# katehai/m-cedm

Measured on AMD Instinct MI355X. Metric: denoised_states_per_sec_18step_edm_heun, higher is better.
Workload: dtype f32; 1 GPU; SWE-periodic 128x128, EDM U-Net ch=128 ch_mult=[1,1,1,1] attn@16^2 (BASELINE config 3); states_per_gpu=32, global_batch=32, H=128, W=128, sampler=EDM Heun, 18 steps, 35 NFE/state, S_churn=0, w=0, fp64 state / fp32 net, parallelism=batch-sharded x1, no data-path collective, launch=one HIP graph per sampler call

## Files before the change

include/mcedm_hip.h:

```cpp
#ifndef MCEDM_HIP_H_
#define MCEDM_HIP_H_

#include <stddef.h>
#include <stdint.h>

#ifdef __cplusplus
extern "C" {
#endif

#define MCEDM_ABI_VERSION 4
#define MCEDM_REDUCE_SCRATCH_BYTES (4096 * 8 + 64)
#define MCEDM_MAX_LEVELS 8

typedef enum {
  MCEDM_OK = 0,
  MCEDM_ERR_INVALID = -1,
  MCEDM_ERR_UNSUPPORTED = -2,
  MCEDM_ERR_WORKSPACE = -3,
  MCEDM_ERR_HIP = -4
} mcedm_status;

#define MCEDM_DX_NONE 0
#define MCEDM_DX_CAT 1
#define MCEDM_DX_ENC 2
typedef struct {
  int32_t in_channels;
  int32_t cond_channels;
  int32_t out_channels;
  int32_t ch;
  int32_t n_levels;
  int32_t ch_mult[MCEDM_MAX_LEVELS];
  int32_t num_res_blocks;
  int32_t resolution;
  int32_t n_attn_resolutions;
  int32_t attn_resolutions[MCEDM_MAX_LEVELS];
  int32_t channels_per_head;
  float eps;
  int32_t dx_channels;
  int32_t dx_mode;
} mcedm_unet_desc;

typedef struct {
  int32_t timesteps;
  double sigma_min, sigma_max, rho;
  double S_churn, S_min, S_max, S_noise;
  double w;
  double sigma_data;
  double net_sigma_min, net_sigma_max;
} mcedm_sampler_desc;

typedef struct mcedm_plan mcedm_plan;

int mcedm_version(void);
const char* mcedm_last_error(void);

int mcedm_unet_plan_create(const mcedm_unet_desc* desc, mcedm_plan** out);
void mcedm_unet_plan_destroy(mcedm_plan* plan);

#define MCEDM_VARIANT_CONV_WINO 0
#define MCEDM_VARIANT_CONV_WINO1 1
#define MCEDM_VARIANT_CONV_RESIDENT 2
#define MCEDM_VARIANT_CONV8 3
#define MCEDM_VARIANT_ATTN_FUSED 4
#define MCEDM_VARIANT_WGRAD_WINO 5
#define MCEDM_VARIANT_CONV1X1_REG 6
#define MCEDM_VARIANT_CONV_WINO_FOLD 7
#define MCEDM_VARIANT_CONV_WINO_UPZ 8
int mcedm_unet_plan_set_variant(mcedm_plan* plan, int which, int value);

int mcedm_unet_param_count(const mcedm_plan* plan);
int mcedm_unet_param_info(const mcedm_plan* plan, int index, const char** name, int64_t* numel,
                          int32_t* ndim, int64_t shape[4]);

int mcedm_unet_packed_bytes(const mcedm_plan* plan, size_t* bytes);
int mcedm_unet_pack_weights(const mcedm_plan* plan, const float* const* params, void* packed, void* stream);

int mcedm_unet_workspace_bytes(const mcedm_plan* plan, int B, int H, int W, int training, size_t* bytes);

int mcedm_unet_forward(const mcedm_plan* plan, const void* packed, const float* x, const float* cond,
                       const float* x_scale, const float* noise_labels, int n_noise, float* out,
                       void* workspace, size_t workspace_bytes, int B, int H, int W, int training,
                       void* stream);

int mcedm_edm_denoise(const mcedm_plan* plan, const void* packed, const float* x, const float* sigma,
                      int n_sigma, const float* cond, float* D_out, float* F_out, void* workspace,
                      size_t workspace_bytes, int B, int H, int W, int training, double sigma_data,
                      void* stream);

int mcedm_sampler_workspace_bytes(const mcedm_plan* plan, int B, int H, int W, size_t* bytes);
int mcedm_heun_sample(const mcedm_plan* plan, const void* packed, const mcedm_sampler_desc* sp,
                      const float* cond, const float* mask, const float* init_noise,
                      const double* step_noise, double* out, int return_last, void* workspace,
                      size_t workspace_bytes, int B, int H, int W, void* stream);

int mcedm_heun_sample_rng(const mcedm_plan* plan, const void* packed, const mcedm_sampler_desc* sp, const float* cond,
                          const float* mask, const float* init_noise, const uint64_t* rng_seed, double* out, int return_last,
                          void* workspace, size_t workspace_bytes, int B, int H, int W, void* stream);
typedef struct {
  int32_t system;
  float half_dt, dx;
  float two_dx;
  float sub_h, div_h, sub_u, div_u;
  double weight;
} mcedm_guidance_desc;
int mcedm_heun_sample_guided(const mcedm_plan* plan, const void* packed, const mcedm_sampler_desc* sp,
                             const mcedm_guidance_desc* gd, const float* cond, const float* mask,
                             const float* init_noise, const double* step_noise, double* out, int return_last,
                             void* workspace, size_t workspace_bytes, int B, int H, int W, void* stream);
int mcedm_heun_sample_guided_rng(const mcedm_plan* plan, const void* packed, const mcedm_sampler_desc* sp,
                                 const mcedm_guidance_desc* gd, const float* cond, const float* mask, const float* init_noise,
                                 const uint64_t* rng_seed, double* out, int return_last, void* workspace, size_t workspace_bytes,
                                 int B, int H, int W, void* stream);
int mcedm_unet_forward_dx(const mcedm_plan* plan, const void* packed, const float* x, const float* dx, const float* cond,
                          const float* x_scale, const float* noise_labels, int n_noise, float* out, void* workspace,
                          size_t workspace_bytes, int B, int H, int W, int training, void* stream);
int mcedm_edm_denoise_dx(const mcedm_plan* plan, const void* packed, const float* x, const float* dx, const float* sigma,
                         int n_sigma, const float* cond, float* D_out, float* F_out, void* workspace,
                         size_t workspace_bytes, int B, int H, int W, int training, double sigma_data, void* stream);
int mcedm_edm_denoise_backward_dx(const mcedm_plan* plan, const void* packed, const float* const* params, const float* x,
                                  const float* dx, const float* sigma, int n_sigma, const float* cond, const float* dD,
// ... 56 lines not shown
                                 void* stream);

typedef struct {
  int32_t timesteps;
  int32_t cond_channels;
  const double* t_steps;
  const double* t_hat;
  const float* c_noise;
  double S_noise;
  double w;
} mcedm_vp_sampler_desc;
int mcedm_vp_sampler_workspace_bytes(const mcedm_plan* plan, int B, int H, int W, size_t* bytes);
int mcedm_vp_heun_sample(const mcedm_plan* plan, const void* packed, const mcedm_vp_sampler_desc* sp, const float* cond,
                         const float* init_noise, const double* step_noise, double* out, int return_last, void* workspace,
                         size_t workspace_bytes, int B, int H, int W, void* stream);
int mcedm_vp_heun_sample_rng(const mcedm_plan* plan, const void* packed, const mcedm_vp_sampler_desc* sp, const float* cond,
                             const float* init_noise, const uint64_t* rng_seed, double* out, int return_last, void* workspace,
                             size_t workspace_bytes, int B, int H, int W, void* stream);

typedef struct mcedm_cond_ddim_desc {
  int32_t timesteps, skip_type;
  double eta, w;
  int32_t cond_channels, self_cond, num_diffusion_timesteps;
  const float* alphas_cumprod_ext;
} mcedm_cond_ddim_desc;
int mcedm_cond_ddim_workspace_bytes(const mcedm_plan* plan, int B, int H, int W, size_t* bytes);
int mcedm_cond_ddim_sample(const mcedm_plan* plan, const void* packed, const mcedm_cond_ddim_desc* sp, const float* cond,
                           const float* init_noise, const float* eta_noise, float* xs_out, float* x0_out, int return_last,
                           void* workspace, size_t workspace_bytes, int B, int H, int W, void* stream);
int mcedm_cond_ddim_sample_rng(const mcedm_plan* plan, const void* packed, const mcedm_cond_ddim_desc* sp, const float* cond,
                               const float* init_noise, const uint64_t* rng_seed, float* xs_out, float* x0_out, int return_last,
                               void* workspace, size_t workspace_bytes, int B, int H, int W, void* stream);


typedef struct { float mean, scale, offset, pad; } mcedm_coef;

size_t mcedm_op_conv_packed_floats(int Cout, int Cin, int k);
int mcedm_op_pack_conv(const float* w, const float* b, int Cout, int Cin, int k, int qkv_heads, int dgrad,
                       float* wpk, float* bias_pk, void* stream);
int mcedm_op_gn_coef(const float* xa, const float* xb, int Ca, int Cb, int B, int HW, const float* gamma,
                     const float* beta, const float* film, int film_batch, int film_stride, float eps,
                     mcedm_coef* coef_out, float* stats_out, void* stream);
int mcedm_op_conv(const float* xa, const float* xb, int Ca, int Cb, const mcedm_coef* coef, int coef_batch, int act,
                  int resample, int Hs, int Ws, int H, int W, const float* wpk, const float* bias_pk,
                  const float* res, int res_mode, float* out, int Cout, int B, int k, void* stream);
size_t mcedm_op_conv_wino_packed_floats(int Cout, int Cin);
int mcedm_op_pack_conv_wino(const float* w, int Cout, int Cin, float* wino, void* stream);
int mcedm_op_conv_wino(const float* xa, const float* xb, int Ca, int Cb, const mcedm_coef* coef, int coef_batch, int act,
                       int resample, int H, int W, const float* wino, const float* bias, const float* res, int res_mode,
                       float* out, int Cout, int B, void* stream);
int mcedm_op_conv_wino_sums(const float* xa, const float* xb, int Ca, int Cb, const mcedm_coef* coef, int coef_batch, int act,
                            int resample, int H, int W, const float* wino, const float* bias, const float* res, int res_mode,
                            float* out, float* gsum, int Cout, int B, void* stream);
int mcedm_op_conv_bias_batch(const float* xa, const float* xb, int Ca, int Cb, const mcedm_coef* coef, int coef_batch, int act,
                             int resample, int Hs, int Ws, int H, int W, const float* wpk, const float* bias_pk, int bias_batch,
                             const float* res, int res_mode, float* out, int Cout, int B, int k, void* stream);
int mcedm_op_conv_wino_sums_bias_batch(const float* xa, const float* xb, int Ca, int Cb, const mcedm_coef* coef, int coef_batch,
                                       int act, int resample, int H, int W, const float* wino, const float* bias, int bias_batch,
                                       const float* res, int res_mode, float* out, float* gsum, int Cout, int B, void* stream);
int mcedm_op_pack_conv_wino_dgrad(const float* w, int Cout, int Cin, float* wino, void* stream);
int mcedm_op_embedding(const float* labels, int n, int ch, const float* w0, const float* b0, const float* w1,
                       const float* b1, const float* waff, const float* baff, int rows, float* freqs_scratch,
                       float* emb_out, float* film_out, void* stream);
int mcedm_op_attention(const float* qkv, float* out, int B, int heads, int T, void* stream);
int mcedm_op_attn_block64(const float* y, const float* gamma, const float* beta, float eps, const float* wq_pk,
                          const float* bq_pk, const float* wp_pk, const float* bp_pk, float* z, float* gsum, int B, void* stream);
size_t mcedm_op_wgrad_scratch_floats(int Cout, int Cin, int k, int B, int H, int W);
int mcedm_op_conv_wgrad(const float* dy, const float* xa, const float* xb, int Ca, int Cb, const mcedm_coef* coef,
                        int coef_batch, int act, int resample, int Hs, int Ws, int H, int W, int Cout, int B, int k,
                        int qkv_heads, float* scratch, float* dw, float* db, void* stream);
int mcedm_op_gn_bwd(const float* dact, int resample, const float* xa, const float* xb, int Ca, int Cb, int Hs, int Ws,
                    int B, const mcedm_coef* coef, const float* stats, const float* gamma, const float* beta,
                    const float* film, int film_batch, int film_stride, int act, float* dxa, float* dxb, int accumulate,
                    const float* add, int add_mode, float* ab, float* dgamma, float* dbeta, float* dfilm,
                    int dfilm_stride, void* stream);
#define MCEDM_GN_SYNC_WORDS 130
int mcedm_op_gn_bwd_sync(const float* dact, int resample, const float* xa, const float* xb, int Ca, int Cb, int Hs, int Ws,
                         int B, const mcedm_coef* coef, const float* stats, const float* gamma, const float* beta,
                         const float* film, int film_batch, int film_stride, int act, float* dxa, float* dxb, int accumulate,
                         const float* add, int add_mode, float* ab, float* dgamma, float* dbeta, float* dfilm,
                         int dfilm_stride, unsigned int* sync, void* stream);
int mcedm_op_attention_bwd(const float* qkv, const float* a, const float* da, float* dqkv, float* lse_scratch, int B,
                           int heads, int T, void* stream);
int mcedm_op_ddim_cond_step(const float* xt, const float* F, const float* Fu, const float* noise, double w, float s0, float s1,
                            float sa_next, float c1, float c2, float* xt_next, float* condp, float* condp_u, int cond_channels,
                            int plan_cond_channels, int B, int C, int H, int W, float* xs, int T_xs, int t_xs, float* x0s,
                            int T_x0, int t_x0, void* stream);
int mcedm_op_ddim_cond_step_rng(const float* xt, const float* F, const float* Fu, const uint64_t* rng_seed, uint64_t draw, double w,
                                float s0, float s1, float sa_next, float c1, float c2, float* xt_next, float* condp, float* condp_u,
                                int cond_channels, int plan_cond_channels, int B, int C, int H, int W, float* xs, int T_xs,
                                int t_xs, float* x0s, int T_x0, int t_x0, void* stream);
int mcedm_op_set_conv_tile(int mt, int ph, int pw);
int mcedm_op_set_conv8(int enable);
int mcedm_op_set_conv_resident(int enable);
int mcedm_op_set_conv_wino(int enable);
int mcedm_op_set_conv_wino1(int enable);
int mcedm_op_set_wgrad_wino(int enable);
int mcedm_op_set_conv1x1_reg(int enable);
int mcedm_op_set_conv_wino_fold(int enable);
int mcedm_op_set_conv_wino_upz(int enable);
int mcedm_op_pack_conv_frag(const float* w, int Cout, int Cin, float* wfrag, void* stream);
int mcedm_op_conv_skip(const float* x, int Cin, const mcedm_coef* coef, int act, int H, int W, const float* wpk, const float* wino,
                       const float* bias, const float* res, const float* sk_xa, const float* sk_xb, int sk_Ca, int sk_Cb,
                       const float* sk_wpk, const float* sk_wfrag, const float* sk_bias, float* out, float* gsum, int Cout, int B,
                       void* stream);
int mcedm_op_conv_sums(const float* xa, const float* xb, int Ca, int Cb, const mcedm_coef* coef, int coef_batch, int act, int resample,
                       int Hs, int Ws, int H, int W, const float* wpk, const float* wino, const float* bias_pk, int bias_batch,
                       const float* res, int res_mode, float* out, int Cout, int B, int k, float* gsum, int gsum_rc, int* tiling_out,
                       void* stream);
int mcedm_op_gn_coef_from_sums(const float* suma, const float* sumb, const int* tiling_a, const int* tiling_b, int Ca, int Cb, int B, int H,
                               int W, int groups, const float* gamma, const float* beta, const float* film, int film_batch,
                               int film_stride, float eps, mcedm_coef* coef_out, float* stats_out, void* stream);
int mcedm_op_conv_gn(const float* xa, const float* xb, int Ca, int Cb, const float* suma, const float* sumb, const int* tiling_a,
                     const int* tiling_b, int groups, const float* gamma, const float* beta, const float* film, int film_batch,
                     int film_stride, float eps, int act, int resample, int Hs, int Ws, int H, int W, const float* wpk, const float* wino,
                     const float* bias_pk, const float* res, int res_mode, float* out, int Cout, int B, int k, void* stream);
int mcedm_op_set_attn_fused(int enable);
int mcedm_op_set_conv_debug(unsigned long long* buf);

typedef struct {
  int32_t in_channels;
  int32_t out_channels;
  int32_t ch;
  int32_t n_levels;
  int32_t ch_mult[MCEDM_MAX_LEVELS];
  int32_t num_res_blocks;
  int32_t resolution;
  int32_t n_attn_resolutions;
  int32_t attn_resolutions[MCEDM_MAX_LEVELS];
  int32_t self_cond;
  float eps;
} mcedm_ddpm_desc;

typedef struct {
  int32_t timesteps;
  double sigma_min, sigma_max, rho;
  double S_churn, S_min, S_max, S_noise;
  double w;
  int32_t n_repeat;
  int32_t n_time_h, n_time_u;
  int32_t h_ch, u_ch;
  int32_t num_diffusion_timesteps;
  const float* edm_steps;
  const float* alphas_cumprod_ext;
} mcedm_repaint_desc;

typedef struct mcedm_ddpm_plan mcedm_ddpm_plan;
int mcedm_ddpm_plan_create(const mcedm_ddpm_desc* desc, mcedm_ddpm_plan** out);
void mcedm_ddpm_plan_destroy(mcedm_ddpm_plan* plan);
int mcedm_ddpm_plan_set_variant(mcedm_ddpm_plan* plan, int which, int value);
int mcedm_ddpm_param_count(const mcedm_ddpm_plan* plan);
int mcedm_ddpm_param_info(const mcedm_ddpm_plan* plan, int index, const char** name, int64_t* numel, int32_t* ndim,
                          int64_t shape[4]);
// ... 100 lines not shown
```

m-cedm_amd/csrc/backward.hip:

```cpp
#include <algorithm>
#include <cmath>
#include <vector>

#include "bwd.hpp"
#include "plan.hpp"

namespace mcedm {

static inline int grid_for(size_t n) {
  size_t b = (n + 255) / 256;
  return (int)(b < 2048 ? (b ? b : 1) : 2048);
}

__global__ void scale_by_cout_kernel(const float* __restrict__ dD, const float* __restrict__ coefs4, int n_sigma,
                                     size_t per_sample, size_t total, float* __restrict__ dF) {
  for (size_t i = blockIdx.x * (size_t)blockDim.x + threadIdx.x; i < total; i += (size_t)gridDim.x * blockDim.x)
    dF[i] = dD[i] * coefs4[4 * (n_sigma == 1 ? 0 : i / per_sample) + 1];
}

__device__ __forceinline__ float silu_b(float v) { return v / (1.0f + expf(-v)); }
__device__ __forceinline__ float dsilu_b(float v) { const float s = 1.0f / (1.0f + expf(-v)); return s * (1.0f + v * (1.0f - s)); }

__global__ __launch_bounds__(256) void emb_save_kernel(const float* __restrict__ labels, const float* __restrict__ freqs,
                                                       const float* __restrict__ w0, const float* __restrict__ b0,
// ... 89 lines not shown
  S.xact = take(max_dact * 4);
  S.ab = take((size_t)B * max_c * 2 * 4);
  S.wg = take(max_wg * 4);
  S.dfilm = take((size_t)B * P.film_rows * 4);
  S.lse = take(max_lse * 4);
  S.gF = take((size_t)B * P.desc.out_channels * H * W * 4);
  S.pe = take((size_t)B * ch * 4); S.u1 = take((size_t)B * ch * 4); S.u2 = take((size_t)B * ch * 4);
  S.t1 = take((size_t)B * ch * 4); S.t2 = take((size_t)B * ch * 4); S.t3 = take((size_t)B * ch * 4);
  S.emb = take((size_t)B * ch * 4);
  S.sync_bytes = gn_bwd_sync_words(B, 32) * sizeof(unsigned);
  S.sync = take(S.sync_bytes);
  S.total = cur;
  return S;
}

size_t backward_scratch_bytes(const mcedm_plan& P, const Layout& L, int B, int H, int W) {
  return make_scratch(P, L, B, H, W).total;
}

struct Ctx;
static GnBwdArgs with_sync(const Ctx& c, GnBwdArgs g);

struct Ctx {
  const AdmNet& net;
  const mcedm_plan& P;
  const Layout& L;
  const BwdScratch& S;
  char* scr;
  const float* pk;
  float* const* grads;
  int B, n_noise;
  hipStream_t s;
  std::vector<char> have;
  const float* emb = nullptr;
  int n_buckets = 0;
  const int32_t* bucket_first = nullptr;
  void* const* bucket_events = nullptr;

  Ctx(const AdmNet& n, const BwdScratch& scratch, float* const* g)
      : net(n), P(*n.plan), L(n.L), S(scratch), scr(n.act + n.L.total_bytes), pk(n.pk), grads(g), B(n.B), n_noise(n.n_noise),
        s(n.s), have(n.L.t.size(), 0) {}
  float* T(int id) const { return net.T(id); }
  Coef* CF(int id) const { return net.CF(id); }
  float* G(int id) const { return id < 0 ? nullptr : reinterpret_cast<float*>(scr + S.g[id]); }
  float* X(size_t off) const { return reinterpret_cast<float*>(scr + off); }
};
static GnBwdArgs with_sync(const Ctx& c, GnBwdArgs g) { g.sync = reinterpret_cast<unsigned*>(c.X(c.S.sync)); return g; }

static int dgrad(const Ctx& c, const ConvP& cv, const float* dy, int H, int W, float* out) {
  ConvArgs a{};
  a.xa = dy; a.Ca = cv.cout;
  a.Hs = H; a.Ws = W; a.H = H; a.W = W;
  a.wpk = c.pk + cv.wpk_dgrad;
  a.wino = cv.wino_dgrad != NONE ? c.pk + cv.wino_dgrad : nullptr;
  a.out = out; a.Cout = cv.cin; a.B = c.B;
  return launch_conv(a, cv.taps, c.s);
}

static int norm_param_grads(const Ctx& c, const NormP& nm, const float* film, int film_stride, float* dfilm) {
  return launch_gn_param_grads(c.X(c.S.ab), c.pk + nm.gamma, c.pk + nm.beta, film, c.net.coef_batch(), film_stride,
                               c.B, nm.C, c.grads[nm.w], c.grads[nm.b], dfilm, c.P.film_rows, c.s);
}

static int block_backward(Ctx& c, const BlockP& b, const BlockLayout& bl) {
  int rc;
  const int B = c.B, H = bl.H, W = bl.W;
  const float* xa = c.T(bl.xa);
  const float* xb = c.T(bl.xb);
  const int Ca = c.L.t[bl.xa].C, Cb = bl.xb >= 0 ? c.L.t[bl.xb].C : 0;
  const int rs = b.up ? RS_UP : (b.down ? RS_DOWN : RS_NONE);
  float* dact = c.X(c.S.dact);
  float* wg = c.X(c.S.wg);
  const float* dy = c.G(bl.out);
  if (b.attn) {
    const float* dz = c.G(bl.z);
    WgradArgs wp{dz, c.T(bl.a), nullptr, b.cout, 0, nullptr, 0, 0, RS_NONE, H, W, H, W, b.cout, B, wg, nullptr};
    if ((rc = launch_wgrad(wp, 1, c.grads[b.proj.w], c.grads[b.proj.b], 0, c.X(c.S.xact), c.s))) return rc;
    if ((rc = dgrad(c, b.proj, dz, H, W, c.G(bl.a)))) return rc;
    if ((rc = launch_attention_bwd(c.T(bl.qkv), c.T(bl.a), c.G(bl.a), c.G(bl.qkv), c.X(c.S.lse), B, b.heads, H * W, c.s))) return rc;
    if ((rc = dgrad(c, b.qkv, c.G(bl.qkv), H, W, dact))) return rc;
    GnBwdArgs g2{dact, RS_NONE, c.T(bl.y), nullptr, b.cout, 0, H, W, B, b.norm2.groups, c.CF(bl.coef2), c.T(bl.stats2),
                 c.pk + b.norm2.gamma, nullptr, 0, 0, 0, c.G(bl.y), nullptr, 0, dz, 1, b.cout, c.X(c.S.ab), c.X(c.S.xact)};
    if ((rc = launch_gn_bwd(with_sync(c, g2), c.s))) return rc;
    if ((rc = norm_param_grads(c, b.norm2, nullptr, 0, nullptr))) return rc;
    WgradArgs wq{c.G(bl.qkv), c.T(bl.y), nullptr, b.cout, 0, c.CF(bl.coef2), 1, 0, RS_NONE, H, W, H, W, 3 * b.cout, B, wg, nullptr};
    if ((rc = launch_wgrad(wq, 1, c.grads[b.qkv.w], c.grads[b.qkv.b], b.heads, c.X(c.S.xact), c.s, true))) return rc;
    dy = c.G(bl.y);
  }
  if ((rc = dgrad(c, b.conv1, dy, H, W, dact))) return rc;
  const float* film = c.net.film() + b.film_row0;
  GnBwdArgs g1{dact, RS_NONE, c.T(bl.h), nullptr, b.cout, 0, H, W, B, b.norm1.groups, c.CF(bl.coef1), c.T(bl.stats1),
               c.pk + b.norm1.gamma, film, c.net.coef_batch(), c.P.film_rows, 1, c.G(bl.h), nullptr, 0, nullptr, 0, 0,
               c.X(c.S.ab), c.X(c.S.xact)};
  if ((rc = launch_gn_bwd(with_sync(c, g1), c.s))) return rc;
  if ((rc = norm_param_grads(c, b.norm1, film, c.P.film_rows, c.X(c.S.dfilm) + b.film_row0))) return rc;
  WgradArgs w1{dy, c.T(bl.h), nullptr, b.cout, 0, c.CF(bl.coef1), 1, 1, RS_NONE, H, W, H, W, b.cout, B, wg, nullptr};
  if ((rc = launch_wgrad(w1, 9, c.grads[b.conv1.w], c.grads[b.conv1.b], 0, c.X(c.S.xact), c.s, true))) return rc;
  const float* add = dy;
  int add_mode = 1;
  if (b.skip_kernel == 1) {
    if (rs != RS_NONE) { set_error("backward: resampling 1x1 skip conv is outside the hot path (%s)", b.key.c_str()); return MCEDM_ERR_UNSUPPORTED; }
    WgradArgs wsk{dy, xa, xb, Ca, Cb, nullptr, 0, 0, RS_NONE, H, W, H, W, b.cout, B, wg, nullptr};
    if ((rc = launch_wgrad(wsk, 1, c.grads[b.skip.w], c.grads[b.skip.b], 0, c.X(c.S.xact), c.s))) return rc;
    if ((rc = dgrad(c, b.skip, dy, H, W, c.X(c.S.dskip)))) return rc;
    add = c.X(c.S.dskip);
  } else if (b.skip_kernel == 0) {
    add_mode = 2;
// ... 248 lines not shown
```

m-cedm_amd/csrc/common.hpp:

```cpp
#pragma once
#include <hip/hip_runtime.h>
#include <cstdarg>
#include <cstddef>
#include <cstdint>
#include <cstdio>

#include "mcedm_hip.h"

namespace mcedm {

void set_error(const char* fmt, ...);

#define MCEDM_HIP_TRY(expr)                                                                   \
  do {                                                                                        \
    hipError_t e__ = (expr);                                                                  \
    if (e__ != hipSuccess) {                                                                  \
      ::mcedm::set_error("%s failed: %s (%s:%d)", #expr, hipGetErrorString(e__), __FILE__, __LINE__); \
      return MCEDM_ERR_HIP;                                                                   \
    }                                                                                         \
  } while (0)

#define MCEDM_LAUNCH_CHECK(what)                                                               \
  do {                                                                                        \
    hipError_t e__ = hipGetLastError();                                                       \
    if (e__ != hipSuccess) {                                                                  \
      ::mcedm::set_error("launch of %s failed: %s", what, hipGetErrorString(e__));            \
      return MCEDM_ERR_HIP;                                                                   \
    }                                                                                         \
  } while (0)

#define MCEDM_REQUIRE(cond, ...)                                                              \
  do {                                                                                        \
    if (!(cond)) {                                                                            \
      ::mcedm::set_error(__VA_ARGS__);                                                        \
      return MCEDM_ERR_INVALID;                                                               \
    }                                                                                         \
  } while (0)

enum KernelVariant { KV_CONV_WINO = 0, KV_CONV_WINO1 = 1, KV_CONV_RESIDENT = 2, KV_CONV8 = 3, KV_ATTN_FUSED = 4, KV_WGRAD_WINO = 5,
                     KV_CONV1X1_REG = 6, KV_CONV_WINO_FOLD = 7, KV_CONV_WINO_UPZ = 8, KV_COUNT = 9 };
struct KernelVariants { int v[KV_COUNT] = {-1, -1, -1, -1, -1, -1, -1, -1, -1}; };
const KernelVariants* current_variants();
struct VariantScope {
  const KernelVariants* prev;
  explicit VariantScope(const KernelVariants* kv);
  ~VariantScope();
};
static inline int variant_choice(int which, int global, int env_default) {
  const KernelVariants* kv = current_variants();
  if (kv && kv->v[which] >= 0) return kv->v[which];
  return global >= 0 ? global : env_default;
}

typedef float f32x16 __attribute__((ext_vector_type(16)));
typedef float f32x4 __attribute__((ext_vector_type(4)));
typedef float f32x2 __attribute__((ext_vector_type(2)));

static inline int ceil_div(int a, int b) { return (a + b - 1) / b; }
#ifdef __HIPCC__
__device__ __forceinline__ void xcd_group_map(int map, int& bx, int& by) {
  const int nx = gridDim.x, ny = gridDim.y;
  bx = blockIdx.x; by = blockIdx.y;
  if (!map || (ny & 7) != 0) return;
  const int lin = bx + by * nx;
  const int c = lin & 7, i = lin >> 3;
  by = (i / nx) * 8 + c;
  bx = i - (i / nx) * nx;
}
#endif

static inline size_t align_up(size_t v, size_t a) { return (v + a - 1) / a * a; }

struct __attribute__((aligned(16))) Coef {
  float mean, scale, offset, pad;
};

enum Resample { RS_NONE = 0, RS_UP = 1, RS_DOWN = 2, RS_S2 = 3 };

struct SumTiles {
  int tiles = 0;
  int tiles_x = 0;
  int ph = 0, pw = 0;
  int rc = 4;
};
__host__ __device__ static inline int sum_tile_count(const SumTiles& g, int t, int H, int W) {
  const int ty = t / g.tiles_x, tx = t - ty * g.tiles_x;
  const int h = H - ty * g.ph < g.ph ? H - ty * g.ph : g.ph;
  const int w = W - tx * g.pw < g.pw ? W - tx * g.pw : g.pw;
  return g.rc * h * w;
}

struct GnArgs {
  const float* xa; const float* xb; int Ca, Cb;
  int HW, B, groups;
// ... 7 lines not shown
  const float* suma; const float* sumb;
  SumTiles ta, tb;
  int W;
};
int launch_gn_coef_from_sums(const GnArgs& a, hipStream_t stream);
int launch_gn_coef(const GnArgs& a, hipStream_t stream);
bool gn_sums_usable(const GnArgs& a);

struct ConvArgs {
  const float* xa;
  const float* xb;
  int Ca, Cb;
  const Coef* coef;
  int coef_batch;
  int act;
  int resample;
  int Hs, Ws;
  int H, W;
  const float* wpk;
  const float* wino;
  const float* bias;
  const float* res;
  int res_mode;
  int bias_batch;
  float* out;
  int Cout;
  int B;
  float* gsum;
  int gsum_rc;
  SumTiles* gsum_tiles;
  const float* sk_xa; const float* sk_xb; int sk_Ca, sk_Cb;
  const float* sk_wpk; const float* sk_bias;
  GnArgs gn; int gn_on;
  int coef_rows;
  unsigned long long* dbg;
  const float* sk_wfrag;
};
static_assert(sizeof(ConvArgs) % 8 == 0 && offsetof(ConvArgs, bias_batch) + sizeof(int) == offsetof(ConvArgs, out),
              "bias_batch fills the padding in front of `out`: no member moves and the struct does not grow");

int launch_conv(const ConvArgs& a, int taps, hipStream_t stream);
size_t conv_wino_packed_floats(int Cout, int Cin);
int launch_pack_conv_wino(const float* w, float* dst, int Cout, int Cin, int transpose_flip, hipStream_t stream);
bool conv_wino_applicable(const ConvArgs& a, int taps);
bool conv_wino_shape_ok(int Cout, int Cin, int H, int W);
bool conv_wino_fold_shape_ok(int Cout, int sk_Ca, int sk_Cb, int H, int W);
void set_conv_wino_fold(int enable);
void set_conv_wino_upz(int enable);
size_t conv_frag_packed_floats(int Cout, int Cin);
int launch_pack_conv_frag(const float* w, float* dst, int Cout, int Cin, hipStream_t stream);
void set_conv_wino(int enable);
bool conv_wino_preferred(const ConvArgs& a);
int launch_conv_wino(const ConvArgs& a, hipStream_t stream);
static inline int cout_padded(int Cout) { return (Cout + 31) / 32 * 32; }
int conv_resolve_identity(ConvArgs& a);
unsigned long long* conv_debug_buffer();
int try_launch_conv_resident(const ConvArgs& a, int taps, hipStream_t stream);
int try_launch_conv1x1_reg(const ConvArgs& a, int taps, hipStream_t stream);
void set_conv1x1_reg(int enable);
void set_conv_resident(int enable);
static inline int conv_max_tiles(int H, int W) { return ((H + 3) / 4) * ((W + 7) / 8); }
void set_conv_tile_override(int mt, int ph, int pw);
void set_conv8(int enable);
void set_conv_debug(unsigned long long* buf);
int conv_mt_for(int Cout);
int conv_kc_for(int taps);
size_t conv_packed_floats(int Cout, int Cin, int taps);
int launch_pack_conv(const float* w, float* dst, int Cout, int Cin, int taps, int qkv_heads, int transpose_flip,
                     hipStream_t stream);
int launch_pack_bias(const float* b, float* dst, int Cout, int qkv_heads, hipStream_t stream);



struct EmbArgs {
  const float* labels; int n;
  int ch;
  const float* freqs;
  const float* w0; const float* b0; const float* w1; const float* b1;
  const float* waff; const float* baff; int rows;
  float* emb;
  float* film;
};
int launch_embedding(const EmbArgs& a, hipStream_t stream);

int launch_attention(const float* qkv, float* out, int B, int heads, int T, hipStream_t stream);
bool attn_block_fused_applicable(int C, int heads, int H, int W, int groups);
int launch_attn_block64(const float* y, float* z, const float* gamma, const float* beta, float eps, int groups, const float* wq,
                        const float* bq, const float* wp, const float* bp, float* gsum, SumTiles* gsum_tiles, int B,
                        hipStream_t stream);
void set_attn_fused(int enable);

}
```

m-cedm_amd/csrc/conv_mfma.hip:

```cpp
#include <atomic>
#include <cstdlib>

#include "common.hpp"
#include "conv_tile.hpp"
#include "pack.hpp"
#include "prof.hpp"

namespace mcedm {

__device__ Coef k_identity_coef = {0.f, 1.f, 0.f, 0.f};


template <class C>
__device__ __forceinline__ void conv_skip_phase(const ConvArgs& p, const TileGeom<C, RS_NONE>& G, float* xl, float* wl,
                                                f32x16 (&acc)[C::TM][C::TN], int n, int m0, int coutp, int aoff,
                                                const int (&boff)[C::TN], int tid, int wave) {
  static_assert(C::TAPS == 9, "the folded projection rides on a 3x3 conv");
  constexpr int SUB = TileGeom<C, RS_NONE>::SUB;
  constexpr int KS = 8;
  constexpr int V4 = C::MT / 4;
  constexpr int NV4 = KS * V4;
  static_assert(NV4 <= C::NT && C::KC == KS, "one float4 of the skip slab per thread");
  const int Cin = p.sk_Ca + p.sk_Cb;
  const int iters = (Cin + KS - 1) / KS;
// ... 734 lines not shown
  const long long want = 512;
  if ((long long)a.H * a.W <= 256 || a.W < 12) {
    if (coutp % 64 == 0) return launch_cfg<ConvCfg<64, 8, 8, 2, 2, TAPS, KC, 256, SMALL_CPI>>(a, stream);
    return launch_cfg<ConvCfg<32, 8, 8, 1, 2, TAPS, KC, 256, SMALL_CPI>>(a, stream);
  }
  if (TAPS == 9 && a.W >= 24 && (long long)a.H * a.W <= 1024) {
    if (coutp % 128 == 0 && blocks_for(128, 8, 16) >= want) return launch_cfg<ConvCfg<128, 8, 16, 1, 4, TAPS, KC>>(a, stream);
    if (coutp % 64 == 0) return launch_cfg<ConvCfg<64, 8, 16, 1, 4, TAPS, KC, 256, MID_CPI>>(a, stream);
    return launch_cfg<ConvCfg<32, 8, 32, 1, 4, TAPS, KC>>(a, stream);
  }
  if (a.W >= 24) {
    static int conv8_env = -1;
    if (conv8_env < 0) { const char* e = getenv("MCEDM_CONV8"); conv8_env = e ? atoi(e) : 0; }
    if (variant_choice(KV_CONV8, g_conv8, conv8_env) && !a.sk_wpk && a.gsum_rc != 2 && TAPS == 9 && a.resample == RS_NONE && coutp % 128 == 0 && a.Ca + a.Cb <= 2048 &&
        blocks_for(128, 16, 32) >= 224)
      return launch_conv8(a, stream);
    if (coutp % 128 == 0 && blocks_for(128, 8, 32) >= want) return launch_cfg<ConvCfg<128, 8, 32, 1, 4, TAPS, KC>>(a, stream);
    if (coutp % 64 == 0 && blocks_for(64, 8, 32) >= want) return launch_cfg<ConvCfg<64, 8, 32, 1, 4, TAPS, KC>>(a, stream);
    return launch_cfg<ConvCfg<32, 8, 32, 1, 4, TAPS, KC>>(a, stream);
  }
  if (coutp % 128 == 0 && blocks_for(128, 16, 16) >= want) return launch_cfg<ConvCfg<128, 16, 16, 1, 4, TAPS, KC>>(a, stream);
  if (coutp % 64 == 0 && blocks_for(64, 16, 16) >= want) return launch_cfg<ConvCfg<64, 16, 16, 1, 4, TAPS, KC>>(a, stream);
  return launch_cfg<ConvCfg<32, 16, 16, 1, 4, TAPS, KC>>(a, stream);
#endif
}

int launch_conv(const ConvArgs& a, int taps, hipStream_t stream) {
  MCEDM_REQUIRE(taps == 9 || taps == 1, "conv: taps must be 9 or 1 (got %d)", taps);
  MCEDM_REQUIRE(a.B > 0 && a.H > 0 && a.W > 0 && a.Cout > 0 && a.Ca + a.Cb > 0, "conv: empty shape");
  MCEDM_REQUIRE(a.out && a.wpk, "conv: null output / weights");
  if (a.resample == RS_UP) MCEDM_REQUIRE(a.Hs * 2 == a.H && a.Ws * 2 == a.W, "conv: up-resample needs H = 2*Hs");
  else if (a.resample == RS_DOWN) MCEDM_REQUIRE(a.Hs == a.H * 2 && a.Ws == a.W * 2, "conv: down-resample needs Hs = 2*H");
  else if (a.resample == RS_S2) MCEDM_REQUIRE(taps == 9 && a.Hs == a.H * 2 && a.Ws == a.W * 2 && !a.res,
                                              "conv: the stride-2 conv is 3x3 on an even-sized source, without residual");
  else MCEDM_REQUIRE(a.Hs == a.H && a.Ws == a.W, "conv: source size mismatch");
  if (a.res && a.res_mode == RS_UP) MCEDM_REQUIRE(a.H % 2 == 0 && a.W % 2 == 0, "conv: up residual needs even size");
  if (a.sk_wpk) MCEDM_REQUIRE(taps == 9 && a.resample == RS_NONE && a.sk_Ca + a.sk_Cb > 0 && (a.sk_xa || a.sk_xb) && a.Cout > 4,
                              "conv: a folded 1x1 projection rides on an un-resampled 3x3 conv with more than 4 output channels");
  MCEDM_REQUIRE(a.bias_batch == 0 || (a.bias && a.bias_batch >= a.Cout && (long long)a.B * a.bias_batch < (1ll << 31) && taps == 9 &&
                                      a.resample == RS_NONE && a.Cout > 4),
                "conv: a bias row per sample (bias_batch=%d) goes with an un-resampled 3x3 conv of more than 4 output channels", a.bias_batch);
  MCEDM_REQUIRE((unsigned long long)a.Hs * a.Ws * 4ull < (1ull << 32) &&
                (unsigned long long)cout_padded(a.Cout) * (a.Ca + a.Cb + 16) * taps * 4ull < (1ull << 32),
                "conv: plane or weight table exceeds the 4 GiB buffer range");
  if (a.res) {
    const unsigned long long rpix = a.res_mode == RS_DOWN ? 4ull * a.H * a.W : a.res_mode == RS_UP ? (a.H / 2ull) * (a.W / 2ull)
                                                                                                    : 1ull * a.H * a.W;
    MCEDM_REQUIRE(rpix * a.Cout * 4ull < (1ull << 32), "conv: one sample of the residual exceeds the 4 GiB buffer range");
  }
  if (taps == 9 && a.Cout <= 4 && a.resample == RS_NONE && !a.res && !a.gsum && !g_force_mt && (long long)a.H * a.W >= 4096)
    return launch_small_cout(a, stream);
  if (a.resample == RS_S2) return dispatch_s2(a, stream);
  if (!g_force_mt && taps == 9 && a.wino && (a.bias_batch == 0 || a.act) && conv_wino_preferred(a) && conv_wino_applicable(a, taps)) return launch_conv_wino(a, stream);
  if (!g_force_mt && taps == 1) {
    const int rc = try_launch_conv1x1_reg(a, taps, stream);
    if (rc != -1) return rc;
  }
  if (!g_force_mt) {
    const int rc = try_launch_conv_resident(a, taps, stream);
    if (rc != -1) return rc;
  }
  return taps == 9 ? dispatch<9, 8>(a, stream) : dispatch<1, 16>(a, stream);
}

}
```

m-cedm_amd/csrc/conv_resident.hip:

```cpp
#include <atomic>
#include <algorithm>
#include <cstdint>
#include <cstdlib>
#include <type_traits>

#include "common.hpp"
#include "conv_tile.hpp"
#include "prof.hpp"

namespace mcedm {

__device__ __forceinline__ int opaque(int v) { asm volatile("" : "+v"(v)); return v; }

static constexpr int SKC = 16;

template <int MT_, int PH_, int PW_, int WM_, int WN_, int TAPS_, int KC_, int KS_ = 1, int DB_ = 0>
struct ResCfg {
  static constexpr int MT = MT_, PH = PH_, PW = PW_, WM = WM_, WN = WN_, TAPS = TAPS_, KC = KC_, KS = KS_;
  static constexpr bool DB = DB_ != 0;
  static constexpr int CPI = 1, KCI = KC_, NT = 256;
  static constexpr int HALO = (TAPS == 9) ? 1 : 0;
  static constexpr int XL0 = HALO ? 3 : 0;
  static constexpr int XM = HALO ? 4 : 0;
  static constexpr int PITCH = HALO ? PW + 8 : PW;
// ... 405 lines not shown
      }
    }
  }

  if (p.dbg && tid == 0) { p.dbg[blockIdx.x * 16 + 2] = __builtin_amdgcn_s_memrealtime(); p.dbg[blockIdx.x * 16 + 6] = __builtin_amdgcn_s_memtime(); }
  float* red = wl;
  if constexpr (C::KS > 1) {
    float* part = xl;
    constexpr int PER_WAVE = C::TM * C::TN * 16 * 64;
    if (ks > 0) {
      float* dst = part + ((ks - 1) * (C::WM * C::WN) + wm * C::WN + wn) * PER_WAVE + lane;
#pragma unroll
      for (int i = 0; i < C::TM; ++i)
#pragma unroll
        for (int j = 0; j < C::TN; ++j)
#pragma unroll
          for (int r = 0; r < 16; ++r) dst[((i * C::TN + j) * 16 + r) * 64] = acc[i][j][r];
    }
    __syncthreads();
    if (ks == 0) {
      for (int g = 1; g < C::KS; ++g) {
        const float* src = part + ((g - 1) * (C::WM * C::WN) + wm * C::WN + wn) * PER_WAVE + lane;
#pragma unroll
        for (int i = 0; i < C::TM; ++i)
#pragma unroll
          for (int j = 0; j < C::TN; ++j)
#pragma unroll
            for (int r = 0; r < 16; ++r) acc[i][j][r] += src[((i * C::TN + j) * 16 + r) * 64];
      }
    }
  }
  if (ks == 0) conv_epilogue_any<C>(p, acc, n, m0, y0, x0, wm, wn, lane, red);
  if (p.dbg && tid == 0) {
    asm volatile("s_waitcnt vmcnt(0)" ::: "memory");
    p.dbg[blockIdx.x * 16 + 3] = __builtin_amdgcn_s_memrealtime();
    unsigned hwid, xcc;
    asm volatile("s_getreg_b32 %0, hwreg(HW_REG_HW_ID)" : "=s"(hwid));
    asm volatile("s_getreg_b32 %0, hwreg(HW_REG_XCC_ID)" : "=s"(xcc));
    p.dbg[blockIdx.x * 16 + 4] = ((unsigned long long)xcc << 32) | hwid;
  }
  if (p.gsum) {
    __syncthreads();
    conv_stats_store<C, C::WN>(p, red, n, m0, ty * tiles_x + tx, tiles_x * tiles_y, tid);
  }
}

static int g_resident = -1;
void set_conv_resident(int enable) { g_resident = enable; }
static int resident_level() {
  static int env = -1;
  if (env < 0) { const char* e = getenv("MCEDM_CONV_RESIDENT"); env = e ? atoi(e) : 1; }
  return variant_choice(KV_CONV_RESIDENT, g_resident, env);
}

static constexpr int LDS_MAX = 160 * 1024;
static int big_level() {
  static int env = -1;
  if (env < 0) { const char* e = getenv("MCEDM_RES_BIG"); env = e ? atoi(e) : 1; }
  return env;
}
static int db_level() {
  static int env = -1;
  if (env < 0) { const char* e = getenv("MCEDM_RES_DB"); env = e ? atoi(e) : 0; }
  return env;
}
static int big128_level() {
  static int env = -1;
  if (env < 0) { const char* e = getenv("MCEDM_RES_BIG128"); env = e ? atoi(e) : 0; }
  return env;
}
static int big_pass() {
  static int env = -1;
  if (env < 0) { const char* e = getenv("MCEDM_RES_BIG_PASS"); env = (e && atoi(e) >= 8) ? atoi(e) / 8 * 8 : 1 << 20; }
  return env;
}

struct ResidentPlan { int pass_c = 0, nslab = 0, wide = 0; size_t lds = 0; };

template <class C, bool SPLIT>
static size_t resident_lds_bytes(const ConvArgs& a, int pass_c, int nslab) {
  return sizeof(float) * ((size_t)nslab * SlabGeom<C, SPLIT>::SL + (size_t)((C::BIG || C::DB) ? 2 : 1) * pass_c * C::PLANE) + sizeof(Coef) * (size_t)(a.Ca + a.Cb);
}

template <class C, bool SPLIT>
static ResidentPlan resident_plan(const ConvArgs& a, size_t budget, int min_pass) {
  constexpr int LPQ = C::PH * (C::PW / 4);
  constexpr int CPS = C::BIG ? 1 : C::NT / C::PLANE, CPD = C::BIG ? 1 : C::NT / C::NPIX, CPQ = LPQ > 64 ? 1 : 64 / LPQ;
  ResidentPlan r;
  const int Cin = a.Ca + a.Cb, Csk = a.sk_wpk ? a.sk_Ca + a.sk_Cb : 0;
  if (!a.xa || a.Ca <= 0 || (a.Cb > 0 && !a.xb)) return r;
  if (Csk && (!a.sk_xa || a.sk_Ca <= 0 || (a.sk_Cb > 0 && !a.sk_xb) || Csk % SKC)) return r;
  auto al16 = [](const void* q) { return (reinterpret_cast<uintptr_t>(q) & 15u) == 0; };
  r.wide = a.resample == RS_NONE && a.Ws % 4 == 0 && a.W % 4 == 0 && al16(a.xa) && al16(a.xb) && a.Ca % C::CPW == 0 && Cin % C::CPW == 0 &&
           (!Csk || (al16(a.sk_xa) && al16(a.sk_xb) && a.sk_Ca % CPQ == 0));
  if (!r.wide && (C::BIG || a.Ca % CPS || Cin % CPS || (Csk && a.sk_Ca % CPD))) { r.wide = 0; return r; }
  const int need = std::max(ceil_div(Cin, C::KC) * C::KC, Csk);
  constexpr int G = C::BIG ? C::KC : (C::KS * C::KC > 16 ? C::KS * C::KC : 16);
  static_assert(!C::BIG || 2 * C::KC * C::PLANE >= SKC * C::NPIX, "projection chunk fits the two pass buffers");
  const int all = ceil_div(need, G) * G;
  for (int nslab = 3; nslab >= 2; --nslab) {
    const size_t fixed = resident_lds_bytes<C, SPLIT>(a, 0, nslab);
    if (fixed >= budget) continue;
    int pc = (int)((budget - fixed) / (sizeof(float) * C::PLANE * ((C::BIG || C::DB) ? 2 : 1))) / G * G;
    if (pc > all) pc = all;
    if (pc >= std::min(min_pass, all)) { r.pass_c = pc; r.nslab = nslab; r.lds = resident_lds_bytes<C, SPLIT>(a, pc, nslab); return r; }
  }
// ... 127 lines not shown
```

m-cedm_amd/csrc/conv_wino.hip:

```cpp
#include <atomic>
#include <cstdlib>

#include "conv_wino.hpp"
#include "pack.hpp"
#include "prof.hpp"

namespace mcedm {

__global__ void wino_pack_kernel(const float* __restrict__ w, float* __restrict__ dst, int Cout, int Cin, int coutp, int nch,
                                 int tflip) {
  const int idx = blockIdx.x * blockDim.x + threadIdx.x;
  if (idx >= coutp * nch * WKC) return;
  wino_pack_elem(w, dst, idx, Cout, Cin, coutp, tflip);
}

__global__ void conv_frag_pack_kernel(const float* __restrict__ w, float* __restrict__ dst, int Cout, int Cin, int coutp, int cinp) {
  const int idx = blockIdx.x * blockDim.x + threadIdx.x;
  if (idx >= coutp * cinp) return;
  dst[idx] = frag_pack_value(w, idx, Cout, Cin, coutp);
}

template <class C, bool = C::SKIP>
struct SkipFold {};
template <class C>
// ... 60 lines not shown
#pragma unroll
    for (int r = 0; r < 16; ++r) v0[r] = keep[0][r] + xch[(pw * 16 + r) * 64 + lane];
    f32x4 bq[4];
#pragma unroll
    for (int jj = 0; jj < 4; ++jj) bq[jj] = *reinterpret_cast<const f32x4*>(rd + 4 * jj);
    for (int s = 0; s < nsk; ++s) {
      f32x4 bqn[4], san[2];
      wreq(s + 1 < nsk ? s + 1 : s, san);
      commit((s + 1) & 1);
      sld = req(s + 2 < nsk ? s + 2 : nsk - 1);
#pragma unroll
      for (int j = 0; j < 4; ++j)
#pragma unroll
        for (int e = 0; e < 2; ++e) rv[e] = __builtin_amdgcn_mfma_f32_32x32x2f32(sa[j >> 2][j & 3], bq[j >> 1][2 * (j & 1) + e], rv[e], 0, 0, 0);
      __syncthreads();
      const float* b = rd + ((s + 1) & 1) * SKBUF;
#pragma unroll
      for (int jj = 0; jj < 4; ++jj) bqn[jj] = *reinterpret_cast<const f32x4*>(b + 4 * jj);
      if (s == 0) {
#pragma unroll
        for (int r = 0; r < 16; ++r) xch[(wave * 16 + r) * 64 + lane] = send[1][r];
      }
      if (s == 1) {
#pragma unroll
        for (int r = 0; r < 16; ++r) v1[r] = keep[1][r] + xch[(pw * 16 + r) * 64 + lane];
      }
#pragma unroll
      for (int j = 4; j < 8; ++j)
#pragma unroll
        for (int e = 0; e < 2; ++e) rv[e] = __builtin_amdgcn_mfma_f32_32x32x2f32(sa[j >> 2][j & 3], bq[j >> 1][2 * (j & 1) + e], rv[e], 0, 0, 0);
#pragma unroll
      for (int jj = 0; jj < 4; ++jj) bq[jj] = bqn[jj];
      sa[0] = san[0];
      sa[1] = san[1];
    }
#pragma unroll
    for (int r = 0; r < 16; ++r) {
      const float bs = skb[(r & 3) + 8 * (r >> 2)];
      v0[r] = v0[r] + (rv[0][r] + bs);
      v1[r] = v1[r] + (rv[1][r] + bs);
    }
  }
};

template <class C, bool UP, bool ACT = true, class... Tag>
__global__ __launch_bounds__(C::NT, C::MB == 4 ? 1 : 2) void conv_wino_kernel(const ConvArgs p, int tiles_x, int tiles_img, int nch, int mblocks,
                                                                          int per, int mode) {
  constexpr int WSC = C::SC, VBUF = C::VBUF, RBUF = C::RBUF, MB = C::MB;
  constexpr bool SKIP = C::SKIP;
  constexpr bool UPZ = WinoUpTraits<Tag...>::UPZ;
  constexpr bool UPS = WinoUpTraits<Tag...>::UPS;
  static_assert(!UPS || UPZ, "source-resolution staging is part of the zero-position variant");
  static_assert(!UPZ || (UP && !SKIP), "the zero positions belong to the up-sampled input");
  extern __shared__ float lds[];
  const int Cin = p.Ca + p.Cb;
  float* const vbuf = lds;
  float* const rbuf = lds + 2 * VBUF;
  Coef* const cfl = reinterpret_cast<Coef*>(lds + C::LDS_ROWS_OFF);
  float* const xch = lds + C::LDS_ROWS_OFF + 4 * Cin;
  float* const red = xch + C::XCH_FLOATS;
  float* const bias_l = red + 2 * (C::MT / 2) * 3;
  float* const skb_l = bias_l + C::MT;
  float* const skbuf = skb_l + C::MT;
  const int tid = threadIdx.x, lane = tid & 63;
  const int wave = __builtin_amdgcn_readfirstlane(tid >> 6);
  const int mb = wave % MB, hf = wave / MB;
  if (p.dbg && tid == 0) { p.dbg[blockIdx.x * 16 + 0] = __builtin_amdgcn_s_memrealtime(); p.dbg[blockIdx.x * 16 + 4] = per; }
  int gt0 = blockIdx.x * per, tstep = 1;
  int n = gt0 / tiles_img, tile0 = gt0 % tiles_img;
  if (mode & 256) {
    const int nwg = gridDim.x, wps = tiles_img / per;
    const int lid = (nwg % 8 == 0) ? (int)(blockIdx.x % 8) * (nwg / 8) + (int)(blockIdx.x / 8) : (int)blockIdx.x;
    n = lid / wps; tile0 = lid % wps; tstep = wps;
  }
  const int m0 = blockIdx.y * C::MT;
  const size_t HW = (size_t)p.H * p.W, HWs = (size_t)p.Hs * p.Ws;
  const int nst = (nch + WSC - 1) / WSC;
  const int G = per * nst;

  constexpr int NR = UPS ? 1 : UP ? RSUB : 4, NG = UPS ? 1 : UP ? RSUB : 1;
  unsigned roff[NG], rkeepL[NG], rkeepC[NG];
  int lofs[4];
  if (!UP) {
    const int r = lane / 6, qd = lane % 6;
#pragma unroll
    for (int e = 0; e < 4; ++e) {
      const int col = 4 * qd + e - 3;
      lofs[e] = (lane < 60 && col >= 0 && col < RPITCH) ? r * RPITCH + col : RROWS * RPITCH + lane % (RPLANE - RROWS * RPITCH);
    }
  }
  auto set_geom = [&](int tile) {
    const int y0 = (tile / tiles_x) * WPH, x0 = (tile % tiles_x) * WPW;
    if (UPS) {
      const int r = lane / UCOLS, c = lane - r * UCOLS;
      const int y = (y0 >> 1) - 1 + r, x = (x0 >> 1) - 1 + c;
      const bool inb = lane < UROWS * UCOLS && (unsigned)y < (unsigned)p.Hs && (unsigned)x < (unsigned)p.Ws;
      rkeepL[0] = inb ? 0xffffffffu : 0u;
      roff[0] = !inb ? 0u : 4u * (unsigned)(y * p.Ws + x);
    } else if (UP) {
#pragma unroll
      for (int i = 0; i < NG; ++i) {
        const int e = lane + 64 * i;
        const int r = e / RPITCH, c = e - r * RPITCH;
        const int y = y0 - 1 + r, x = x0 - 1 + c;
        const bool inb = e < RROWS * RPITCH && (unsigned)y < (unsigned)p.H && (unsigned)x < (unsigned)p.W;
        rkeepL[i] = inb ? 0xffffffffu : 0u;
        roff[i] = !inb ? 0u : 4u * (unsigned)((y >> 1) * p.Ws + (x >> 1));
      }
    } else {
      const int y = y0 - 1 + lane / 6, x = x0 - 4 + 4 * (lane % 6);
      const bool inb = lane < 60 && (unsigned)y < (unsigned)p.H && x >= 0 && x < p.W;
      rkeepL[0] = inb ? 0xffffffffu : 0u;
      roff[0] = inb ? 4u * (unsigned)(y * p.W + x) : 0u;
    }
  };
  float raw[WSC][C::CPW][NR];
  int ld_st = 0, ld_tile = tile0, cm_st = 0;
  set_geom(tile0);
  auto raw_load1 = [&](int sc) {
#pragma unroll
    for (int cw = 0; cw < C::CPW; ++cw) {
      const int ci = (ld_st * WSC + sc) * WKC + wave * C::CPW + cw;
      const bool in_a = ci < p.Ca;
      const float* src = in_a ? p.xa : p.xb;
      const int cc = in_a ? ci : ci - p.Ca, CC = in_a ? p.Ca : p.Cb;
      const bool ok = ci < Cin && src != nullptr;
      const float* plane = ok ? src + ((size_t)n * CC + cc) * HWs : (p.xa ? p.xa : p.xb);
      if (UP) {
// ... 92 lines not shown
      for (int ti = 0; ti < C::TI; ++ti) {
        float t[2][3];
#pragma unroll
        for (int c = 0; c < 3; ++c) {
          t[0][c] = tu[sc][ti][0][c] - tu[sc][ti][2][c];
          t[1][c] = tu[sc][ti][2][c] + tsgn * tu[sc][ti][1][c];
        }
#pragma unroll
        for (int x = 0; x < 2; ++x) {
          if (x == 0 && hf != 0) continue;
          float* o = vb + sc * 16 * VPOS + tr_dst + MB * ti * WTX * 4 + 4 * x * VPOS;
          o[0 * VPOS] = t[x][0] - t[x][1];
          o[1 * VPOS] = t[x][1] + 1.f * t[x][1];
          o[3 * VPOS] = t[x][1] - t[x][2];
        }
      }
      return;
    }
#pragma unroll
    for (int ti = 0; ti < C::TI; ++ti) {
      f32x2 t[2][2];
#pragma unroll
      for (int j = 0; j < 2; ++j) {
        t[0][j] = td[sc][ti][0][j] - td[sc][ti][2][j];
        t[1][j] = td[sc][ti][2][j] + tsgn * td[sc][ti][1][j];
      }
#pragma unroll
      for (int x = 0; x < 2; ++x) {
        const f32x2 o03 = t[x][0] - t[x][1];
        const f32x2 c11 = {t[x][0].y, t[x][0].y}, c22 = {t[x][1].x, t[x][1].x};
        const f32x2 o12 = c11 + tpm * c22;
        float* o = vb + sc * 16 * VPOS + tr_dst + MB * ti * WTX * 4 + 4 * x * VPOS;
        o[0 * VPOS] = o03.x;
        o[1 * VPOS] = o12.x;
        if constexpr (!UPZ) o[2 * VPOS] = o12.y;
        o[3 * VPOS] = o03.y;
      }
    }
  };
  auto transform_read = [&](const float* rb) { for (int sc = 0; sc < WSC; ++sc) transform_read1(sc, rb); };
  auto transform_finish = [&](float* vb) { for (int sc = 0; sc < WSC; ++sc) transform_finish1(sc, vb); };

  stage_coef_rows<C::NT>(p, n, cfl, tid);
  if (tid < C::MT) bias_l[tid] = p.bias ? p.bias[(WinoUpTraits<Tag...>::BROWS ? n * p.bias_batch : 0) + m0 + tid] : 0.f;
  if constexpr (SKIP) { if (tid < C::MT) skb_l[tid] = p.sk_bias ? p.sk_bias[m0 + tid] : 0.f; }
  raw_load();
  __syncthreads();
  for (int sc = 0; sc < WSC; ++sc) raw_commit1(sc, rbuf);
  commit_done();
  if (G > 1) { raw_load(); for (int sc = 0; sc < WSC; ++sc) raw_commit1(sc, rbuf + RBUF); commit_done(); }
  if (G > 2) raw_load();
  const size_t ustride = (size_t)mblocks * 16 * 64;
  constexpr int PHF = UPZ ? 12 : 8;
  const f32x4* up = reinterpret_cast<const f32x4*>(p.wino) + ((size_t)(m0 / 32 + mb) * 16 + PHF * hf) * 64 + lane;
  f32x4 ua[8];
  if constexpr (UPZ) {
    const f32x4 zero4 = {0.f, 0.f, 0.f, 0.f};
    ua[0] = up[0 * 64]; ua[1] = up[1 * 64]; ua[3] = up[3 * 64];
    ua[4] = zero4; ua[5] = zero4; ua[7] = zero4;
    if (hf == 0) { ua[4] = up[4 * 64]; ua[5] = up[5 * 64]; ua[7] = up[7 * 64]; }
  } else {
#pragma unroll
    for (int q = 0; q < 8; ++q) ua[q] = up[q * 64];
  }
  __syncthreads();
  transform_read(rbuf);
  transform_finish(vbuf);
  f32x16 acc[8];
  auto init_acc = [&]() {
    const f32x16 zero16 = {0.f, 0.f, 0.f, 0.f, 0.f, 0.f, 0.f, 0.f, 0.f, 0.f, 0.f, 0.f, 0.f, 0.f, 0.f, 0.f};
    float z = 0.f;
#pragma unroll
    for (int q = 0; q < 8; ++q) {
      asm volatile("" : "+v"(z));
      acc[q] = __builtin_amdgcn_mfma_f32_32x32x2f32(z, z, zero16, 0, 0, 0);
    }
    if (hf == 0) {
#pragma unroll
      for (int r = 0; r < 16; ++r) acc[5][r] = bias_l[32 * mb + 4 * (lane >> 5) + (r & 3) + 8 * (r >> 2)];
    }
  };
  __syncthreads();
  init_acc();

  const int vrd = (PHF * hf) * VPOS + (lane >> 5) * VH1 + (lane & 31) * 4;
  if (p.dbg && tid == 0) { p.dbg[blockIdx.x * 16 + 1] = __builtin_amdgcn_s_memrealtime(); p.dbg[blockIdx.x * 16 + 5] = __builtin_amdgcn_s_memtime(); }
#ifdef MCEDM_WINO_TIMELINE
  unsigned long long ph[5] = {0, 0, 0, 0, 0}, tlast = __builtin_amdgcn_s_memtime();
#define WINO_STAMP(i) { const unsigned long long t_ = __builtin_amdgcn_s_memtime(); ph[i] += t_ - tlast; tlast = t_; }
  unsigned long long sl[8] = {0, 0, 0, 0, 0, 0, 0, 0}, slast = 0;
#define WINO_SLOT(i) { const unsigned long long t_ = __builtin_amdgcn_s_memtime(); sl[(i) & 7] += t_ - slast; slast = t_; }
#define WINO_SLOT0 { slast = __builtin_amdgcn_s_memtime(); }
  unsigned long long ep[6] = {0, 0, 0, 0, 0, 0}, elast = 0;
#define WINO_EP(i) { __builtin_amdgcn_sched_barrier(0); const unsigned long long t_ = __builtin_amdgcn_s_memtime(); if (i) ep[(i) - 1] += t_ - elast; elast = t_; __builtin_amdgcn_sched_barrier(0); }
  const bool no_u = mode & 2;
#else
#define WINO_STAMP(i)
#define WINO_SLOT(i)
#define WINO_SLOT0
#define WINO_EP(i)
  constexpr bool no_u = false;
#endif
  auto side_slice_upz = [&](int slot, int cur) {
    if (WSC == 2) {
      if (slot == 0) transform_read1(0, rbuf + (cur ^ 1) * RBUF);
      if (slot == 1) raw_commit1(0, rbuf + cur * RBUF);
      if (slot == 2) { transform_finish1(0, vbuf + (cur ^ 1) * VBUF); raw_load1(0); }
      if (slot == 3) transform_read1(WSC - 1, rbuf + (cur ^ 1) * RBUF);
      if (slot == 4) { raw_commit1(WSC - 1, rbuf + cur * RBUF); commit_done(); }
      if (slot == 5) { transform_finish1(WSC - 1, vbuf + (cur ^ 1) * VBUF); raw_load1(WSC - 1); raw_load_done(); }
    } else {
      if (slot == 0) transform_read(rbuf + (cur ^ 1) * RBUF);
      if (slot == 1) { raw_commit1(0, rbuf + cur * RBUF); commit_done(); }
      if (slot == 2) { transform_finish1(0, vbuf + (cur ^ 1) * VBUF); raw_load1(0); raw_load_done(); }
    }
  };
  auto side_slice = [&](int slot, int g, int cur) {
    if (WSC == 2) {
      if (slot == 0) transform_read1(0, rbuf + (cur ^ 1) * RBUF);
      if (slot == 1) raw_commit1(0, rbuf + cur * RBUF);
      if (slot == 2) { transform_finish1(0, vbuf + (cur ^ 1) * VBUF); raw_load1(0); }
      if (slot == 3) transform_read1(WSC - 1, rbuf + (cur ^ 1) * RBUF);
      if (slot == 4) { raw_commit1(WSC - 1, rbuf + cur * RBUF); commit_done(); }
      if (slot == 5) { transform_finish1(WSC - 1, vbuf + (cur ^ 1) * VBUF); raw_load1(WSC - 1); raw_load_done(); }
    } else {
      if (slot == 0) transform_read(rbuf + (cur ^ 1) * RBUF);
      if (slot == 1) { raw_commit1(0, rbuf + cur * RBUF); commit_done(); }
      if (slot == 2) { raw_load1(0); raw_load_done(); }
      if (slot == 3) transform_finish1(0, vbuf + (cur ^ 1) * VBUF);
    }
  };
  (void)mode;
  int st = 0, tile = tile0;
  for (int g = 0; g < G; ++g) {
    const int cur = g & 1;
    WINO_STAMP(0)
    WINO_SLOT0
#pragma unroll
    for (int sc = 0; sc < WSC; ++sc) {
      const int c = st * WSC + sc;
      const f32x4* un = up + (size_t)(c + 1 < nch ? c + 1 : 0) * ustride;
      const float* vb = vbuf + cur * VBUF + sc * 16 * VPOS + vrd;
      if constexpr (UPZ) {
        constexpr int CQ[3] = {0, 1, 3};
        f32x4 bq[3];
        bq[0] = *reinterpret_cast<const f32x4*>(vb);
        bq[1] = *reinterpret_cast<const f32x4*>(vb + VPOS);
        __builtin_amdgcn_sched_group_barrier(0x100, 2, 0);
#pragma unroll
        for (int i = 0; i < 3; ++i) {
          if (i == 0) bq[2] = *reinterpret_cast<const f32x4*>(vb + 3 * VPOS);
#pragma unroll
          for (int s = 0; s < 4; ++s) acc[CQ[i]] = __builtin_amdgcn_mfma_f32_32x32x2f32(ua[CQ[i]][s], bq[i][s], acc[CQ[i]], 0, 0, 0);
          if (!no_u) ua[CQ[i]] = un[CQ[i] * 64];
          side_slice_upz(sc * 3 + i, cur);
          if (i == 0) __builtin_amdgcn_sched_group_barrier(0x100, 1, 0);
#pragma unroll
          for (int k = 0; k < 4; ++k) {
            __builtin_amdgcn_sched_group_barrier(0x008, 1, 0);
            __builtin_amdgcn_sched_group_barrier(0x486, 2 * WINO_IL_K, 0);
          }
          __builtin_amdgcn_sched_group_barrier(0x020, 4, 0);
          __builtin_amdgcn_sched_barrier(0);
          if (sc * 3 + i == (WSC == 2 ? 5 : 2)) raw_load_next();
          __builtin_amdgcn_sched_barrier(0);
        }
        if (hf == 0) {
          constexpr int HQ[3] = {4, 5, 7};
          f32x4 bh[3];
#pragma unroll
          for (int i = 0; i < 3; ++i) bh[i] = *reinterpret_cast<const f32x4*>(vb + HQ[i] * VPOS);
#pragma unroll
          for (int i = 0; i < 3; ++i) {
#pragma unroll
            for (int s = 0; s < 4; ++s) acc[HQ[i]] = __builtin_amdgcn_mfma_f32_32x32x2f32(ua[HQ[i]][s], bh[i][s], acc[HQ[i]], 0, 0, 0);
            if (!no_u) ua[HQ[i]] = un[HQ[i] * 64];
          }
        }
        __builtin_amdgcn_sched_barrier(0);
      } else {
      f32x4 b4[2][2];
      b4[0][0] = *reinterpret_cast<const f32x4*>(vb);
      b4[0][1] = *reinterpret_cast<const f32x4*>(vb + VPOS);
      __builtin_amdgcn_sched_group_barrier(0x100, 2, 0);
#pragma unroll
      for (int qp = 0; qp < 4; ++qp) {
        const int cb = qp & 1;
        if (qp < 3) {
          b4[cb ^ 1][0] = *reinterpret_cast<const f32x4*>(vb + (2 * qp + 2) * VPOS);
          b4[cb ^ 1][1] = *reinterpret_cast<const f32x4*>(vb + (2 * qp + 3) * VPOS);
        }
#pragma unroll
        for (int s = 0; s < 4; ++s) {
          acc[2 * qp] = __builtin_amdgcn_mfma_f32_32x32x2f32(ua[2 * qp][s], b4[cb][0][s], acc[2 * qp], 0, 0, 0);
          acc[2 * qp + 1] = __builtin_amdgcn_mfma_f32_32x32x2f32(ua[2 * qp + 1][s], b4[cb][1][s], acc[2 * qp + 1], 0, 0, 0);
        }
        if (!no_u) {
          ua[2 * qp] = un[(2 * qp) * 64];
          ua[2 * qp + 1] = un[(2 * qp + 1) * 64];
        }
        side_slice(sc * 4 + qp, g, cur);
        if (qp < 3) __builtin_amdgcn_sched_group_barrier(0x100, 2, 0);
#pragma unroll
        for (int i = 0; i < 8; ++i) {
          __builtin_amdgcn_sched_group_barrier(0x008, 1, 0);
          __builtin_amdgcn_sched_group_barrier(0x486, WINO_IL_K, 0);
        }
        __builtin_amdgcn_sched_group_barrier(0x020, 4, 0);
        __builtin_amdgcn_sched_barrier(0);
        if (sc * 4 + qp == (WSC == 2 ? 5 : 2)) raw_load_next();
        __builtin_amdgcn_sched_barrier(0);
        WINO_SLOT(sc * 4 + qp + (WSC == 1 ? 0 : 0))
      }
      }
    }
    WINO_STAMP(1)
    __syncthreads();
    WINO_STAMP(2)
    if (++st < nst) continue;
    st = 0;

    WINO_EP(0)
    const int y0 = (tile / tiles_x) * WPH, x0 = (tile % tiles_x) * WPW;
    const int pt = lane & 31;
    const int oy = y0 + 2 * (pt >> 3) + hf, ox = x0 + 2 * (pt & 7);
    const int cbase = m0 + 32 * mb + 4 * (lane >> 5);
    const size_t splane = (size_t)p.Cout * HW;
    const __amdgpu_buffer_rsrc_t rs_out = make_rsrc(p.out + (size_t)n * splane, 4u * (unsigned)splane);
    const size_t rplane = p.res_mode == RS_UP ? splane >> 2 : p.res_mode == RS_DOWN ? splane << 2 : splane;
    const __amdgpu_buffer_rsrc_t rs_res = make_rsrc(p.res ? p.res + (size_t)n * rplane : nullptr, p.res ? 4u * (unsigned)rplane : 0u);
    const unsigned HWu = (unsigned)HW;
    const unsigned voff = 4u * ((unsigned)cbase * HWu + (unsigned)oy * p.W + ox);
    const unsigned rvoff = 4u * ((unsigned)cbase * (HWu >> 2) + (unsigned)(oy >> 1) * (p.W >> 1) + (ox >> 1));
    f32x16 keep[2], send[2];
    float v0[16], v1[16];
    SkipFold<C> sk;
    if constexpr (SKIP) sk.begin(p, skbuf, n, m0 / 32 + mb, mblocks, y0, x0, tid, lane, hf);
#pragma unroll
    for (int j = 0; j < 2; ++j) {
      const f32x16 t0 = j == 0 ? acc[0] + acc[1] + acc[2] : acc[1] - acc[2] - acc[3];
      const f32x16 t1 = j == 0 ? acc[4] + acc[5] + acc[6] : acc[5] - acc[6] - acc[7];
      if (hf == 0)  { keep[j] = t0 + t1; send[j] = t1; }
      else if (UPZ) { keep[j] = -t1 - t0; send[j] = t1; }
      else          { keep[j] = -t0 - t1; send[j] = t0; }
      __builtin_amdgcn_sched_barrier(0);
    }
    __builtin_amdgcn_sched_barrier(0);
    if constexpr (SKIP) {
      WINO_EP(1)
      sk.run(xch, skb_l + 32 * mb + 4 * (lane >> 5), wave, wave ^ MB, lane, keep, send, v0, v1);
      WINO_EP(2)
    } else {
    float2 rv[16];
    if (p.res && p.res_mode == RS_DOWN) {
      const unsigned dvoff = 4u * ((unsigned)cbase * (HWu << 2) + (unsigned)(2 * oy) * (unsigned)(2 * p.W) + (unsigned)(2 * ox));
#pragma unroll
      for (int r0 = 0; r0 < 16; r0 += 4) {
        f32x4 ta[4], tb[4];
#pragma unroll
        for (int k = 0; k < 4; ++k) {
          const unsigned so = 4u * (unsigned)(((r0 + k) & 3) + 8 * ((r0 + k) >> 2)) * (HWu << 2);
          ta[k] = __builtin_bit_cast(f32x4, __builtin_amdgcn_raw_buffer_load_b128(rs_res, dvoff, so, 0));
          tb[k] = __builtin_bit_cast(f32x4, __builtin_amdgcn_raw_buffer_load_b128(rs_res, dvoff + 8u * (unsigned)p.W, so, 0));
        }
#pragma unroll
        for (int k = 0; k < 4; ++k)
          rv[r0 + k] = make_float2(0.25f * ((ta[k][0] + ta[k][1]) + (tb[k][0] + tb[k][1])), 0.25f * ((ta[k][2] + ta[k][3]) + (tb[k][2] + tb[k][3])));
      }
    } else {
#pragma unroll
      for (int r = 0; r < 16; ++r) {
        const int dr = (r & 3) + 8 * (r >> 2);
        if (p.res && p.res_mode == RS_UP) {
          const float q = __builtin_bit_cast(float, __builtin_amdgcn_raw_buffer_load_b32(rs_res, rvoff, 4u * (unsigned)dr * (HWu >> 2), 0));
// ... 52 lines not shown
            for (int e = 0; e < 2; ++e) {
              float* slot = red + (hf * (C::MT / 2) + 2 * quad + e) * 3;
              slot[0] = cnt; slot[1] = a[e]; slot[2] = b[e];
            }
          } else {
            float* slot = red + (hf * (C::MT / 4) + quad) * 3;
            slot[0] = cnt; slot[1] = a[0] + a[1]; slot[2] = b[0] + b[1];
          }
        }
      }
      __syncthreads();
      conv_stats_store<C, 2>(p, red, n, m0, tile, tiles_img, tid);
    }
    WINO_EP(4)
    __builtin_amdgcn_sched_barrier(0);
    init_acc();
    tile += tstep;
    WINO_EP(5)
    WINO_STAMP(3)
  }
  if (p.dbg && tid == 0) {
    asm volatile("s_waitcnt vmcnt(0)" ::: "memory");
    p.dbg[blockIdx.x * 16 + 2] = __builtin_amdgcn_s_memrealtime(); p.dbg[blockIdx.x * 16 + 6] = __builtin_amdgcn_s_memtime();
    p.dbg[blockIdx.x * 16 + 3] = __builtin_amdgcn_s_memrealtime();
  }
#ifdef MCEDM_WINO_TIMELINE
  if (p.dbg && tid == 0) for (int i = 0; i < 5; ++i) p.dbg[blockIdx.x * 16 + 8 + i] = ph[i];
  if (p.dbg && tid == 0 && (mode & 16)) for (int i = 0; i < 8; ++i) p.dbg[blockIdx.x * 16 + 8 + i] = sl[i];
  if (p.dbg && tid == 0 && (mode & 32)) for (int i = 0; i < 6; ++i) p.dbg[blockIdx.x * 16 + 8 + i] = ep[i];
  if (p.dbg && tid == 64 * MB && !(mode & 48)) { p.dbg[blockIdx.x * 16 + 13] = ph[1]; p.dbg[blockIdx.x * 16 + 14] = ph[2]; p.dbg[blockIdx.x * 16 + 15] = ph[3]; p.dbg[blockIdx.x * 16 + 7] = ph[0]; }
#endif
}

static int g_wino = -1;
void set_conv_wino(int enable) { g_wino = enable; }
static int wino_env() {
  static int env = -1;
  if (env < 0) { const char* e = getenv("MCEDM_WINOGRAD"); env = e ? atoi(e) : 1; }
  return variant_choice(KV_CONV_WINO, g_wino, env);
}
static int g_wino_fold = -1;
void set_conv_wino_fold(int enable) { g_wino_fold = enable; }
static int wino_fold_env() {
  static int env = -1;
  if (env < 0) { const char* e = getenv("MCEDM_WINO_FOLD"); env = e ? atoi(e) : 1; }
  return variant_choice(KV_CONV_WINO_FOLD, g_wino_fold, env);
}
static int g_wino_upz = -1;
void set_conv_wino_upz(int enable) { g_wino_upz = enable; }
static int wino_upz_env() {
  static int env = -1;
  if (env < 0) { const char* e = getenv("MCEDM_WINO_UPZ"); env = e ? atoi(e) : 1; }
  return variant_choice(KV_CONV_WINO_UPZ, g_wino_upz, env);
}
static int wino_mode_env() {
  static int env = -1;
  if (env < 0) {
    const char* e = getenv("MCEDM_WINO_MODE");
    const char* m = getenv("MCEDM_WINO_MAP");
    env = ((e ? atoi(e) : 0) & ~256) | ((m ? atoi(m) : 1) ? 256 : 0);
  }
  return env;
}

static int wino_min_hw_env() {
  static int env = -1;
  if (env < 0) { const char* e = getenv("MCEDM_WINO_MIN_HW"); env = e ? atoi(e) : 1024; }
  return env;
}

size_t conv_frag_packed_floats(int Cout, int Cin) { return (size_t)cout_padded(Cout) * (size_t)ceil_div(Cin, 8) * 8; }

int launch_pack_conv_frag(const float* w, float* dst, int Cout, int Cin, hipStream_t stream) {
  MCEDM_REQUIRE(w && dst && Cout > 0 && Cin > 0, "pack_conv_frag: bad arguments");
  const int coutp = cout_padded(Cout), cinp = ceil_div(Cin, 8) * 8;
  hipLaunchKernelGGL(conv_frag_pack_kernel, dim3(ceil_div(coutp * cinp, 256)), dim3(256), 0, stream, w, dst, Cout, Cin, coutp, cinp);
  MCEDM_LAUNCH_CHECK("conv_frag_pack_kernel");
  return MCEDM_OK;
}

size_t conv_wino_packed_floats(int Cout, int Cin) { return (size_t)16 * cout_padded(Cout) * (size_t)ceil_div(Cin, WKC) * WKC; }

int launch_pack_conv_wino(const float* w, float* dst, int Cout, int Cin, int transpose_flip, hipStream_t stream) {
  MCEDM_REQUIRE(w && dst && Cout > 0 && Cin > 0, "pack_conv_wino: bad arguments");
  const int coutp = cout_padded(Cout), nch = ceil_div(Cin, WKC);
  hipLaunchKernelGGL(wino_pack_kernel, dim3(ceil_div(coutp * nch * WKC, 256)), dim3(256), 0, stream, w, dst, Cout, Cin, coutp, nch,
                     transpose_flip);
  MCEDM_LAUNCH_CHECK("wino_pack_kernel");
  return MCEDM_OK;
}

static bool conv_wino_fold_ok(const ConvArgs& a) {
  const int Csk = a.sk_Ca + a.sk_Cb;
  const unsigned long long HW = (unsigned long long)a.H * a.W;
  return wino_fold_env() != 0 && a.sk_wfrag && a.resample == RS_NONE && !a.res && a.act && a.Cout % 128 == 0 && a.sk_xa && a.sk_Ca > 0 &&
         a.sk_Cb >= 0 && (a.sk_Cb > 0) == (a.sk_xb != nullptr) && a.sk_Ca % 16 == 0 && a.sk_Cb % 16 == 0 && Csk >= 32 && Csk <= 256 &&
         (((size_t)a.sk_xa | (size_t)a.sk_xb | (size_t)a.sk_wfrag) & 15) == 0 && HW * 4ull * (unsigned long long)a.sk_Ca < (1ull << 32) &&
         HW * 4ull * (unsigned long long)a.sk_Cb < (1ull << 32);
}
bool conv_wino_fold_shape_ok(int Cout, int sk_Ca, int sk_Cb, int H, int W) {
  const int Csk = sk_Ca + sk_Cb;
  return wino_fold_env() != 0 && conv_wino_shape_ok(Cout, Cout, H, W) && Cout % 128 == 0 && sk_Ca > 0 && sk_Ca % 16 == 0 && sk_Cb % 16 == 0 &&
         Csk >= 32 && Csk <= 256 && (unsigned long long)H * W * 4ull * (unsigned long long)(sk_Ca > sk_Cb ? sk_Ca : sk_Cb) < (1ull << 32);
}

bool conv_wino_applicable(const ConvArgs& a, int taps) {
// ... 57 lines not shown
                               noact ? "false" : "true", a.bias_batch ? ", WinoBiasRows" : upz == 2 ? ", WinoUp<false>" : upz ? ", WinoUp<true>" : "");
  const double px = (double)a.B * a.H * a.W;
  const double skc = C::SKIP ? (double)(a.sk_Ca + a.sk_Cb) : 0.0;
  ProfScope ps(name, 2.0 * px * a.Cout * ((double)Cin * 9 + skc),
               4.0 * ((double)a.B * Cin * a.Hs * a.Ws + px * (a.Cout * (a.res ? 2 : 1) + skc) + (double)a.Cout * (Cin * 9 + skc)), stream);
  if constexpr (C::SKIP)
    hipLaunchKernelGGL((conv_wino_kernel<C, false>), dim3((unsigned)(total / per), a.Cout / C::MT), dim3(C::NT), lds_bytes, stream, a, tiles_x,
                       tiles_img, nch, cout_padded(a.Cout) / 32, per, wino_mode_env());
  else if (a.bias_batch)
    hipLaunchKernelGGL((conv_wino_kernel<C, false, true, WinoBiasRows>), dim3((unsigned)(total / per), a.Cout / C::MT), dim3(C::NT), lds_bytes, stream, a, tiles_x,
                       tiles_img, nch, cout_padded(a.Cout) / 32, per, wino_mode_env());
  else if (upz == 2)
    hipLaunchKernelGGL((conv_wino_kernel<C, true, true, WinoUp<false>>), dim3((unsigned)(total / per), a.Cout / C::MT), dim3(C::NT), lds_bytes, stream, a, tiles_x,
                       tiles_img, nch, cout_padded(a.Cout) / 32, per, wino_mode_env());
  else if (upz)
    hipLaunchKernelGGL((conv_wino_kernel<C, true, true, WinoUp<true>>), dim3((unsigned)(total / per), a.Cout / C::MT), dim3(C::NT), lds_bytes, stream, a, tiles_x,
                       tiles_img, nch, cout_padded(a.Cout) / 32, per, wino_mode_env());
  else if (a.resample == RS_UP)
    hipLaunchKernelGGL((conv_wino_kernel<C, true>), dim3((unsigned)(total / per), a.Cout / C::MT), dim3(C::NT), lds_bytes, stream, a, tiles_x,
                       tiles_img, nch, cout_padded(a.Cout) / 32, per, wino_mode_env());
  else if (noact)
    hipLaunchKernelGGL((conv_wino_kernel<C, false, false>), dim3((unsigned)(total / per), a.Cout / C::MT), dim3(C::NT), lds_bytes, stream, a, tiles_x,
                       tiles_img, nch, cout_padded(a.Cout) / 32, per, wino_mode_env());
  else
    hipLaunchKernelGGL((conv_wino_kernel<C, false>), dim3((unsigned)(total / per), a.Cout / C::MT), dim3(C::NT), lds_bytes, stream, a, tiles_x,
                       tiles_img, nch, cout_padded(a.Cout) / 32, per, wino_mode_env());
  MCEDM_LAUNCH_CHECK("conv_wino_kernel");
  if (a.gsum_tiles) *a.gsum_tiles = SumTiles{tiles_img, tiles_x, WPH, WPW, a.gsum_rc == 2 ? 2 : 4};
  return MCEDM_OK;
}

int launch_conv_wino(const ConvArgs& a_in, hipStream_t stream) {
  ConvArgs a = a_in;
  a.dbg = conv_debug_buffer();
  MCEDM_REQUIRE(conv_wino_applicable(a, 9), "conv_wino: shape not served by the Winograd kernel");
  MCEDM_REQUIRE(a.out && a.B > 0 && (a.resample == RS_UP ? (a.Hs * 2 == a.H && a.Ws * 2 == a.W) : (a.Hs == a.H && a.Ws == a.W)),
                "conv_wino: bad arguments");
  MCEDM_REQUIRE((unsigned long long)a.H * a.W * 4ull * a.Cout * (a.res && a.res_mode == RS_DOWN ? 4 : 1) < (1ull << 32),
                "conv_wino: one sample of the output / residual exceeds the 4 GiB buffer range");
  { const int rc = conv_resolve_identity(a); if (rc != MCEDM_OK) return rc; }
  if (a.sk_wpk) return launch_wino_cfg<WinoSkipCfg<4>>(a, stream);
  if (a.Cout % 128 == 0 && !a.bias_batch) {
    const int rc = try_launch_conv_wino1(a, stream);
    if (rc != -1) return rc;
  }
  return a.Cout % 128 == 0 ? launch_wino_cfg<WinoCfg<4>>(a, stream) : launch_wino_cfg<WinoCfg<2>>(a, stream);
}

bool conv_wino_shape_ok(int Cout, int Cin, int H, int W) {
  return wino_env() != 0 && Cout % 64 == 0 && Cin % WKC == 0 && H % WPH == 0 && W % WPW == 0 && (long long)H * W >= wino_min_hw_env();
}
bool conv_wino_preferred(const ConvArgs& a) { return wino_env() != 0 && (long long)a.H * a.W >= wino_min_hw_env(); }

}
```

m-cedm_amd/csrc/conv_wino.hpp:

```cpp
#pragma once
#include "conv_tile.hpp"

namespace mcedm {

constexpr int WPH = 8, WPW = 16;
constexpr int WTX = WPW / 2, WTY = WPH / 2;
constexpr int WKC = 8;
static_assert(WTX * WTY == 32, "one MFMA N block of patches per workgroup");
template <int MB_>
struct WinoCfg {
  static constexpr int MB = MB_, NT = 128 * MB_, NW = 2 * MB_, MT = 32 * MB_;
  static constexpr int SC = MB_ == 4 ? 2 : 1;
  static constexpr int CPW = WKC / NW;
  static constexpr int TI = 4 / MB_;
  static constexpr int VBUF = SC * 16 * 288, RBUF = SC * WKC * 196;
  static constexpr int LDS_ROWS_OFF = 2 * VBUF + 2 * RBUF;
  static constexpr int XCH_FLOATS = NW * 16 * 64;
  static constexpr int RED_FLOATS = 2 * (MT / 2) * 3 + MT;
  static constexpr bool SKIP = false;
  static_assert(MB_ == 4 || MB_ == 2, "128 or 64 output channels per workgroup");
  static_assert(LDS_ROWS_OFF % 4 == 0, "LDS layout");
};
template <int MB_>
struct WinoSkipCfg : WinoCfg<MB_> {
  static constexpr bool SKIP = true;
  static constexpr int SKS = 16, SKPITCH = 36, SKBUF = 64 * SKPITCH;
  static constexpr int SK_FLOATS = WinoCfg<MB_>::MT + 2 * SKBUF;
  static_assert(MB_ == 4, "the fold is built for the 128-channel workgroup (512 threads = 16 channels x 32 quads per stage)");
};
template <bool SRC>
struct WinoUp {};
template <class... Tag>
struct WinoUpTraits { static constexpr bool UPZ = false, UPS = false, BROWS = false; static_assert(sizeof...(Tag) == 0, "one tag at most: WinoUp<SRC> or WinoBiasRows"); };
template <bool SRC>
struct WinoUpTraits<WinoUp<SRC>> { static constexpr bool UPZ = true, UPS = SRC, BROWS = false; };
struct WinoBiasRows {};
template <>
struct WinoUpTraits<WinoBiasRows> { static constexpr bool UPZ = false, UPS = false, BROWS = true; };
constexpr int UROWS = WPH / 2 + 2, UCOLS = WPW / 2 + 2;
constexpr int UPLANE = 68;
static_assert(UPLANE >= 64 && UPLANE % 32 == 4 && UPLANE <= 196, "LDS layout");
constexpr int RROWS = WPH + 2, RPITCH = WPW + 2;
constexpr int RPLANE = 196;
constexpr int RSUB = (RROWS * RPITCH + 63) / 64;
constexpr int WINO_IL_K = 5;
constexpr int VH1 = 144, VPOS = 288;
static_assert(RPLANE % 32 == 4 && VH1 % 32 == 16 && VH1 >= 128 && VPOS >= VH1 + 128 && RPLANE >= RROWS * RPITCH && RPLANE % 2 == 0 && VPOS % 4 == 0 && VH1 % 4 == 0, "LDS layout");



int try_launch_conv_wino1(const ConvArgs& a, hipStream_t stream);
void set_conv_wino1(int enable);
int wino_tiles_per_wg(long long total, int tiles_img, int slots);

}
```

m-cedm_amd/csrc/ddpm.hip:

```cpp
#include <cmath>
#include <cstring>
#include <string>
#include <vector>

#include "heun.hpp"
#include "prof.hpp"

namespace mcedm {

struct DConv { int w = -1, b = -1; int cin = 0, cout = 0, taps = 0; size_t wpk = NONE, bias = NONE, wino = NONE; };
struct DNorm { int w = -1, b = -1; int C = 0; size_t gamma = NONE, beta = NONE; };
struct DRes {
  std::string key;
  int cin = 0, cout = 0;
  DNorm n1, n2;
  DConv c1, c2, sc;
  bool has_sc = false;
  int tw = -1, tb = -1;
  int brow = 0;
};
struct DAttn {
  std::string key;
  int C = 0;
  DNorm n;
// ... 505 lines not shown
  Pool pool;
  std::vector<DT> t;
  int bias_batch = 0;

  int act(int C, int H, int W, bool with_sums) {
    DT d; d.C = C; d.H = H; d.W = W;
    d.bytes = (size_t)B * C * H * W * sizeof(float);
    d.off = pool.alloc(d.bytes);
    d.rc = with_sums ? record_width(C) : 0;
    if (d.rc) {
      d.sums_bytes = (size_t)B * conv_max_tiles(H, W) * ceil_div(C, d.rc) * 2 * sizeof(float);
      d.sums = pool.alloc(d.sums_bytes);
    }
    t.push_back(d);
    return (int)t.size() - 1;
  }
  int raw(size_t bytes) { DT d; d.bytes = bytes; d.off = pool.alloc(bytes); t.push_back(d); return (int)t.size() - 1; }
  void release(int id) {
    if (id < 0) return;
    pool.release(t[id].off, t[id].bytes);
    if (t[id].sums != NONE) pool.release(t[id].sums, t[id].sums_bytes);
  }
  float* ptr(int id) const { return id < 0 ? nullptr : reinterpret_cast<float*>(base + t[id].off); }
  float* sums(int id) const { return (id < 0 || t[id].sums == NONE) ? nullptr : reinterpret_cast<float*>(base + t[id].sums); }
};

static int gn_into(DExec& E, const DNorm& n, int xa, int xb, ConvArgs& c, int* table_id) {
  const DT& A = E.t[xa];
  const int Ca = A.C, Cb = xb >= 0 ? E.t[xb].C : 0;
  GnArgs g{E.ptr(xa), E.ptr(xb), Ca, Cb, A.H * A.W, E.B, 32, E.pk + n.gamma, E.pk + n.beta, nullptr, 0, 0, E.P.desc.eps,
           nullptr, nullptr, E.sums(xa), E.sums(xb), A.st, xb >= 0 ? E.t[xb].st : SumTiles{}, A.W};
  *table_id = -1;
  c.act = 1; c.coef_batch = 1;
  const int cpg = (Ca + Cb) / 32, ra = A.rc, rb = xb >= 0 ? E.t[xb].rc : A.rc;
  const bool usable = (Ca + Cb) % 32 == 0 && ra > 0 && rb > 0 && cpg % ra == 0 && cpg % rb == 0 && Ca % ra == 0 && Ca % rb == 0;
  if (usable) {
    if (!E.dry && !gn_sums_usable(g)) { set_error("ddpm forward: statistics table of a %d-channel input is unusable", Ca + Cb); return MCEDM_ERR_INVALID; }
    c.gn = g; c.gn_on = 1; c.coef = nullptr;
    return MCEDM_OK;
  }
  *table_id = E.raw((size_t)E.B * (Ca + Cb) * sizeof(Coef));
  g.coef = reinterpret_cast<Coef*>(E.ptr(*table_id));
  c.coef = g.coef;
  return E.dry ? MCEDM_OK : launch_gn_coef(g, E.s);
}

static void src_of(const DExec& E, ConvArgs& c, int xa, int xb) {
  c.xa = E.ptr(xa); c.Ca = E.t[xa].C;
  c.xb = E.ptr(xb); c.Cb = xb >= 0 ? E.t[xb].C : 0;
  c.Hs = E.t[xa].H; c.Ws = E.t[xa].W; c.H = c.Hs; c.W = c.Ws;
}
static void dst_of(DExec& E, ConvArgs& c, int out, const DConv& cv, const float* bias, bool stats) {
  c.wpk = E.pk + cv.wpk; c.bias = bias ? bias : E.pk + cv.bias;
  c.wino = cv.wino != NONE ? E.pk + cv.wino : nullptr;
  c.out = E.ptr(out); c.Cout = cv.cout; c.B = E.B;
  if (stats && E.t[out].rc) { c.gsum = E.sums(out); c.gsum_rc = E.t[out].rc; c.gsum_tiles = &E.t[out].st; }
}
static int run_conv(DExec& E, ConvArgs& c, int taps, int out) {
  if (E.dry) { if (c.gsum_tiles) *c.gsum_tiles = SumTiles{1, 1, 8, 8, c.gsum_rc == 2 ? 2 : 4}; (void)out; return MCEDM_OK; }
  return launch_conv(c, taps, E.s);
}

static int res_block(DExec& E, const DRes& r, int xa, int xb, const float* bias_table, int* out_id) {
  const int bias_batch = E.bias_batch;
  int rc, tab;
  const int H = E.t[xa].H, W = E.t[xa].W;
  const int h = E.act(r.cout, H, W, true);
  ConvArgs c1{};
  src_of(E, c1, xa, xb);
  if ((rc = gn_into(E, r.n1, xa, xb, c1, &tab))) return rc;
  dst_of(E, c1, h, r.c1, bias_table + r.brow, true);
  c1.bias_batch = bias_batch;
  if ((rc = run_conv(E, c1, 9, h))) return rc;
  E.release(tab);
  const int y = E.act(r.cout, H, W, true);
  ConvArgs c2{};
  src_of(E, c2, h, -1);
  if ((rc = gn_into(E, r.n2, h, -1, c2, &tab))) return rc;
  dst_of(E, c2, y, r.c2, nullptr, true);
  int scid = -1;
  if (r.has_sc && r.c2.wino != NONE && conv_wino_shape_ok(r.cout, r.cout, H, W)) {
    scid = E.act(r.cout, H, W, false);
    ConvArgs cs{};
    src_of(E, cs, xa, xb);
    dst_of(E, cs, scid, r.sc, nullptr, false);
    if ((rc = run_conv(E, cs, 1, scid))) return rc;
    c2.res = E.ptr(scid); c2.res_mode = RS_NONE;
  } else if (r.has_sc) {
    c2.sk_xa = E.ptr(xa); c2.sk_Ca = E.t[xa].C;
    c2.sk_xb = E.ptr(xb); c2.sk_Cb = xb >= 0 ? E.t[xb].C : 0;
    c2.sk_wpk = E.pk + r.sc.wpk; c2.sk_bias = E.pk + r.sc.bias;
  } else {
    c2.res = E.ptr(xa); c2.res_mode = RS_NONE;
  }
  if ((rc = run_conv(E, c2, 9, y))) return rc;
  E.release(tab);
  E.release(h);
  if (scid >= 0) E.release(scid);
  *out_id = y;
  return MCEDM_OK;
}

static int attn_block(DExec& E, const DAttn& a, int x, int* out_id) {
  int rc, tab;
  const int H = E.t[x].H, W = E.t[x].W;
  const int qkv = E.act(3 * a.C, H, W, false);
  ConvArgs cq{};
// ... 851 lines not shown
```

m-cedm_amd/csrc/ops_api.hip:

```cpp
#include "common.hpp"
#include "conv_wino.hpp"
#include "bwd.hpp"
#include "edm.hpp"

using namespace mcedm;

static_assert(sizeof(mcedm_coef) == sizeof(Coef), "mcedm_coef must mirror Coef");

extern "C" size_t mcedm_op_conv_packed_floats(int Cout, int Cin, int k) {
  if (Cout <= 0 || Cin <= 0 || (k != 1 && k != 3)) return 0;
  return conv_packed_floats(Cout, Cin, k * k);
}

extern "C" int mcedm_op_pack_conv(const float* w, const float* b, int Cout, int Cin, int k, int qkv_heads, int dgrad,
                                  float* wpk, float* bias_pk, void* stream) {
  MCEDM_REQUIRE(w && wpk, "op_pack_conv: null pointer");
  MCEDM_REQUIRE(Cout > 0 && Cin > 0 && (k == 1 || k == 3), "op_pack_conv: bad shape");
  MCEDM_REQUIRE(qkv_heads == 0 || (Cout % (3 * qkv_heads) == 0 && !dgrad), "op_pack_conv: bad qkv_heads");
  int rc = dgrad ? launch_pack_conv(w, wpk, Cin, Cout, k * k, 0, 1, (hipStream_t)stream)
                 : launch_pack_conv(w, wpk, Cout, Cin, k * k, qkv_heads, 0, (hipStream_t)stream);
  if (rc) return rc;
  if (b && bias_pk) rc = launch_pack_bias(b, bias_pk, Cout, qkv_heads, (hipStream_t)stream);
  return rc;
}
// ... 44 lines not shown
  return launch_pack_conv_wino(w, wino, Cout, Cin, 0, (hipStream_t)stream);
}

extern "C" int mcedm_op_pack_conv_wino_dgrad(const float* w, int Cout, int Cin, float* wino, void* stream) {
  return launch_pack_conv_wino(w, wino, Cin, Cout, 1, (hipStream_t)stream);
}

extern "C" int mcedm_op_conv_wino(const float* xa, const float* xb, int Ca, int Cb, const mcedm_coef* coef, int coef_batch,
                                  int act, int resample, int H, int W, const float* wino, const float* bias, const float* res,
                                  int res_mode, float* out, int Cout, int B, void* stream) {
  MCEDM_REQUIRE((resample == RS_NONE || resample == RS_UP) && (res_mode == RS_NONE || res_mode == RS_UP || res_mode == RS_DOWN),
                "op_conv_wino: resample must be 0 (none) or 1 (nearest-2x up), res_mode 0, 1 or 2 (2x2-mean down)");
  ConvArgs a{};
  a.xa = xa; a.xb = xb; a.Ca = Ca; a.Cb = Cb;
  a.coef = reinterpret_cast<const Coef*>(coef); a.coef_batch = coef_batch; a.act = act;
  a.resample = resample; a.H = H; a.W = W;
  a.Hs = resample == RS_UP ? H / 2 : H; a.Ws = resample == RS_UP ? W / 2 : W;
  a.wino = wino; a.bias = bias; a.res = res; a.res_mode = res_mode;
  a.out = out; a.Cout = Cout; a.B = B;
  MCEDM_REQUIRE(conv_wino_applicable(a, 9), "op_conv_wino: needs Cout %% 64 == 0, H %% 8 == 0, W %% 16 == 0, Cin %% 8 == 0 and 16-byte aligned inputs / weight table");
  return launch_conv_wino(a, (hipStream_t)stream);
}

static int op_conv_wino_sums(const float* xa, const float* xb, int Ca, int Cb, const mcedm_coef* coef, int coef_batch, int act,
                             int resample, int H, int W, const float* wino, const float* bias, int bias_batch, const float* res,
                             int res_mode, float* out, float* gsum, int Cout, int B, void* stream) {
  MCEDM_REQUIRE((resample == RS_NONE || resample == RS_UP) && (res_mode == RS_NONE || res_mode == RS_UP || res_mode == RS_DOWN),
                "op_conv_wino_sums: resample must be 0 (none) or 1 (nearest-2x up), res_mode 0, 1 or 2 (2x2-mean down)");
  MCEDM_REQUIRE(gsum, "op_conv_wino_sums: gsum is null");
  ConvArgs a{};
  a.xa = xa; a.xb = xb; a.Ca = Ca; a.Cb = Cb;
  a.coef = reinterpret_cast<const Coef*>(coef); a.coef_batch = coef_batch; a.act = act;
  a.resample = resample; a.H = H; a.W = W;
  a.Hs = resample == RS_UP ? H / 2 : H; a.Ws = resample == RS_UP ? W / 2 : W;
  a.wino = wino; a.bias = bias; a.res = res; a.res_mode = res_mode;
  SumTiles st;
  a.out = out; a.Cout = Cout; a.B = B; a.gsum = gsum; a.gsum_tiles = &st;
  MCEDM_REQUIRE(bias_batch == 0 || (bias && bias_batch >= Cout), "op_conv_wino_sums: bias_batch %d needs a bias of B rows of at least Cout floats", bias_batch);
  a.bias_batch = bias_batch;
  MCEDM_REQUIRE(conv_wino_applicable(a, 9), "op_conv_wino_sums: needs Cout %% 64 == 0, H %% 8 == 0, W %% 16 == 0, Cin %% 8 == 0 and 16-byte aligned inputs / weight table");
  return launch_conv_wino(a, (hipStream_t)stream);
}
extern "C" int mcedm_op_conv_wino_sums(const float* xa, const float* xb, int Ca, int Cb, const mcedm_coef* coef, int coef_batch,
                                       int act, int resample, int H, int W, const float* wino, const float* bias, const float* res,
                                       int res_mode, float* out, float* gsum, int Cout, int B, void* stream) {
  return op_conv_wino_sums(xa, xb, Ca, Cb, coef, coef_batch, act, resample, H, W, wino, bias, 0, res, res_mode, out, gsum, Cout, B, stream);
}
extern "C" int mcedm_op_conv_wino_sums_bias_batch(const float* xa, const float* xb, int Ca, int Cb, const mcedm_coef* coef,
                                                  int coef_batch, int act, int resample, int H, int W, const float* wino,
                                                  const float* bias, int bias_batch, const float* res, int res_mode, float* out,
                                                  float* gsum, int Cout, int B, void* stream) {
  return op_conv_wino_sums(xa, xb, Ca, Cb, coef, coef_batch, act, resample, H, W, wino, bias, bias_batch, res, res_mode, out, gsum, Cout, B,
                           stream);
}

extern "C" int mcedm_op_pack_conv_frag(const float* w, int Cout, int Cin, float* wfrag, void* stream) {
  return launch_pack_conv_frag(w, wfrag, Cout, Cin, (hipStream_t)stream);
}

extern "C" int mcedm_op_conv_skip(const float* x, int Cin, const mcedm_coef* coef, int act, int H, int W, const float* wpk, const float* wino,
                                  const float* bias, const float* res, const float* sk_xa, const float* sk_xb, int sk_Ca, int sk_Cb,
                                  const float* sk_wpk, const float* sk_wfrag, const float* sk_bias, float* out, float* gsum, int Cout,
                                  int B, void* stream) {
  MCEDM_REQUIRE(x && out && wpk && Cin > 0 && Cout > 0 && B > 0 && H > 0 && W > 0, "op_conv_skip: bad arguments");
  MCEDM_REQUIRE(!(res && sk_wpk), "op_conv_skip: a residual or a folded projection, not both");
  ConvArgs a{};
  a.xa = x; a.Ca = Cin;
  a.coef = reinterpret_cast<const Coef*>(coef); a.coef_batch = 1; a.act = act;
  a.resample = RS_NONE; a.Hs = H; a.Ws = W; a.H = H; a.W = W;
  a.wpk = wpk; a.wino = wino; a.bias = bias; a.res = res; a.res_mode = RS_NONE;
  a.sk_xa = sk_xa; a.sk_xb = sk_xb; a.sk_Ca = sk_Ca; a.sk_Cb = sk_Cb; a.sk_wpk = sk_wpk; a.sk_wfrag = sk_wfrag; a.sk_bias = sk_bias;
  SumTiles st;
  a.out = out; a.Cout = Cout; a.B = B; a.gsum = gsum; a.gsum_tiles = gsum ? &st : nullptr;
  return launch_conv(a, 9, (hipStream_t)stream);
}

static void tiling_to_ints(const SumTiles& t, int* o) { o[0] = t.tiles; o[1] = t.tiles_x; o[2] = t.ph; o[3] = t.pw; o[4] = t.rc; }
static SumTiles tiling_from_ints(const int* t) { return t ? SumTiles{t[0], t[1], t[2], t[3], t[4]} : SumTiles{}; }

static int op_conv_chain(const char* who, const float* xa, const float* xb, int Ca, int Cb, const mcedm_coef* coef, int coef_batch,
                         const GnArgs* gn, int act, int resample, int Hs, int Ws, int H, int W, const float* wpk, const float* wino,
                         const float* bias_pk, int bias_batch, const float* res, int res_mode, float* out, int Cout, int B, int k,
                         float* gsum, int gsum_rc, int* tiling_out, void* stream) {
  MCEDM_REQUIRE(k == 1 || k == 3, "%s: k must be 1 or 3", who);
  MCEDM_REQUIRE(resample >= 0 && resample <= 3 && res_mode >= 0 && res_mode <= 2, "%s: bad resample mode", who);
  MCEDM_REQUIRE(bias_batch >= 0, "%s: bias_batch %d < 0", who, bias_batch);
  ConvArgs a{};
  a.xa = xa; a.xb = xb; a.Ca = Ca; a.Cb = Cb;
  a.coef = reinterpret_cast<const Coef*>(coef); a.coef_batch = coef_batch; a.act = act;
  a.resample = resample; a.Hs = Hs; a.Ws = Ws; a.H = H; a.W = W;
  a.wpk = wpk; a.wino = wino; a.bias = bias_pk; a.res = res; a.res_mode = res_mode;
  a.out = out; a.Cout = Cout; a.B = B; a.bias_batch = bias_batch;
  SumTiles st;
  if (gsum) { a.gsum = gsum; a.gsum_rc = gsum_rc; a.gsum_tiles = &st; }
  if (gn) { a.gn = *gn; a.gn_on = 1; a.coef = nullptr; a.coef_batch = 1; }
  const int rc = launch_conv(a, k * k, (hipStream_t)stream);
  if (rc) return rc;
  if (gsum) {
    MCEDM_REQUIRE(st.tiles > 0 && st.rc == (gsum_rc == 2 ? 2 : 4), "%s: the launcher wrote no tiling, or records of %d channels where %d were asked for",
                  who, st.rc, gsum_rc == 2 ? 2 : 4);
    tiling_to_ints(st, tiling_out);
  }
  return MCEDM_OK;
}

extern "C" int mcedm_op_conv_sums(const float* xa, const float* xb, int Ca, int Cb, const mcedm_coef* coef, int coef_batch, int act,
// ... 117 lines not shown
              stats, gamma, film, film_batch, film_stride, act, dxa, dxb, accumulate, add, add_mode, C, ab};
  a.sync = sync;
  int rc = launch_gn_bwd(a, (hipStream_t)stream);
  if (rc) return rc;
  return launch_gn_param_grads(ab, gamma, beta, film, film_batch, film_stride, B, C, dgamma, dbeta, dfilm, dfilm_stride,
                               (hipStream_t)stream);
}

extern "C" int mcedm_op_gn_bwd(const float* dact, int resample, const float* xa, const float* xb, int Ca, int Cb, int Hs,
                               int Ws, int B, const mcedm_coef* coef, const float* stats, const float* gamma,
                               const float* beta, const float* film, int film_batch, int film_stride, int act,
                               float* dxa, float* dxb, int accumulate, const float* add, int add_mode, float* ab,
                               float* dgamma, float* dbeta, float* dfilm, int dfilm_stride, void* stream) {
  return op_gn_bwd_impl(dact, resample, xa, xb, Ca, Cb, Hs, Ws, B, coef, stats, gamma, beta, film, film_batch, film_stride, act, dxa, dxb,
                        accumulate, add, add_mode, ab, dgamma, dbeta, dfilm, dfilm_stride, nullptr, stream);
}

extern "C" int mcedm_op_gn_bwd_sync(const float* dact, int resample, const float* xa, const float* xb, int Ca, int Cb, int Hs,
                                    int Ws, int B, const mcedm_coef* coef, const float* stats, const float* gamma,
                                    const float* beta, const float* film, int film_batch, int film_stride, int act,
                                    float* dxa, float* dxb, int accumulate, const float* add, int add_mode, float* ab,
                                    float* dgamma, float* dbeta, float* dfilm, int dfilm_stride, unsigned int* sync, void* stream) {
  return op_gn_bwd_impl(dact, resample, xa, xb, Ca, Cb, Hs, Ws, B, coef, stats, gamma, beta, film, film_batch, film_stride, act, dxa, dxb,
                        accumulate, add, add_mode, ab, dgamma, dbeta, dfilm, dfilm_stride, sync, stream);
}

extern "C" int mcedm_op_attention_bwd(const float* qkv, const float* a, const float* da, float* dqkv, float* lse_scratch,
                                      int B, int heads, int T, void* stream) {
  return launch_attention_bwd(qkv, a, da, dqkv, lse_scratch, B, heads, T, (hipStream_t)stream);
}

extern "C" int mcedm_op_set_conv8(int enable) {
  set_conv8(enable);
  return MCEDM_OK;
}

extern "C" int mcedm_op_set_conv_wino(int enable) {
  set_conv_wino(enable);
  return MCEDM_OK;
}

extern "C" int mcedm_op_set_conv_wino1(int enable) {
  set_conv_wino1(enable);
  return MCEDM_OK;
}

extern "C" int mcedm_op_set_conv_wino_fold(int enable) {
  set_conv_wino_fold(enable);
  return MCEDM_OK;
}

extern "C" int mcedm_op_set_conv_wino_upz(int enable) {
  set_conv_wino_upz(enable);
  return MCEDM_OK;
}

extern "C" int mcedm_op_set_conv1x1_reg(int enable) {
  set_conv1x1_reg(enable);
  return MCEDM_OK;
}

extern "C" int mcedm_op_set_wgrad_wino(int enable) {
  set_wgrad_wino(enable);
  return MCEDM_OK;
}

extern "C" int mcedm_op_set_conv_resident(int enable) {
  set_conv_resident(enable);
  return MCEDM_OK;
}

extern "C" int mcedm_op_set_attn_fused(int enable) {
  set_attn_fused(enable);
  return MCEDM_OK;
}

extern "C" int mcedm_op_set_conv_debug(unsigned long long* buf) {
  set_conv_debug(buf);
  return MCEDM_OK;
}

static int op_ddim_cond_step(const float* xt, const float* F, const float* Fu, const float* noise, const uint64_t* rng_seed,
                             uint64_t draw, double w, float s0, float s1, float sa_next, float c1, float c2, float* xt_next,
                             float* condp, float* condp_u, int cond_channels, int plan_cond_channels, int B, int C, int H, int W,
                             float* xs, int T_xs, int t_xs, float* x0s, int T_x0, int t_x0, void* stream) {
  MCEDM_REQUIRE(xt && F && xt_next, "op_ddim_cond_step: null pointer");
  MCEDM_REQUIRE(B > 0 && C > 0 && H > 0 && W > 0, "op_ddim_cond_step: empty shape");
  MCEDM_REQUIRE(!condp_u || condp, "op_ddim_cond_step: the twin goes with cond'");
  MCEDM_REQUIRE(!condp || (cond_channels >= 0 && cond_channels + C <= plan_cond_channels),
                "op_ddim_cond_step: channels [%d, %d) outside cond' (%d channels)", cond_channels, cond_channels + C, plan_cond_channels);
  MCEDM_REQUIRE((!xs || (t_xs >= 0 && t_xs < T_xs)) && (!x0s || (t_x0 >= 0 && t_x0 < T_x0)), "op_ddim_cond_step: slot outside the trajectory");
  DdimCondStep k{};
  k.xt = xt; k.F = F; k.Fu = Fu; k.noise = noise;
  k.seed = reinterpret_cast<const unsigned long long*>(rng_seed); k.draw = draw;
  k.w1 = (float)(w + 1.0); k.w = (float)w; k.s0 = s0; k.s1 = s1; k.sa = sa_next; k.c1 = c1; k.c2 = c2;
  k.xt_next = xt_next; k.sc = condp; k.sc_u = condp_u;
  k.C = C; k.Cp = plan_cond_channels; k.sc_off = cond_channels; k.hw = (size_t)H * W; k.n = (size_t)B * C * k.hw;
  k.xs = xs; k.x0s = x0s; k.T_xs = T_xs; k.t_xs = t_xs; k.T_x0 = T_x0; k.t_x0 = t_x0;
  return launch_ddim_cond_step(k, (hipStream_t)stream);
}
extern "C" int mcedm_op_ddim_cond_step(const float* xt, const float* F, const float* Fu, const float* noise, double w, float s0,
                                       float s1, float sa_next, float c1, float c2, float* xt_next, float* condp, float* condp_u,
                                       int cond_channels, int plan_cond_channels, int B, int C, int H, int W, float* xs,
                                       int T_xs, int t_xs, float* x0s, int T_x0, int t_x0, void* stream) {
  return op_ddim_cond_step(xt, F, Fu, noise, nullptr, 0, w, s0, s1, sa_next, c1, c2, xt_next, condp, condp_u, cond_channels,
                           plan_cond_channels, B, C, H, W, xs, T_xs, t_xs, x0s, T_x0, t_x0, stream);
// ... 11 lines not shown
```

m-cedm_amd/csrc/plan.hip:

```cpp
#include <algorithm>
#include <cmath>
#include <cstring>

#include "edm.hpp"
#include "pack.hpp"
#include "plan.hpp"
#include "prof.hpp"
#include "bwd.hpp"

namespace mcedm {

static thread_local char g_err[1024] = "";

void set_error(const char* fmt, ...) {
  va_list ap;
  va_start(ap, fmt);
  vsnprintf(g_err, sizeof(g_err), fmt, ap);
  va_end(ap);
}

static NormP make_norm(mcedm_plan& P, const std::string& key, int C) {
  NormP n;
  n.C = C;
  n.groups = std::min(32, C / 4);
  n.w = add_param(P.params, key + ".weight", {C});
  n.b = add_param(P.params, key + ".bias", {C});
  return n;
}

static ConvP make_conv(mcedm_plan& P, const std::string& key, int cin, int cout, int k, int qkv_heads = 0) {
  ConvP c;
  c.cin = cin; c.cout = cout; c.taps = k * k; c.qkv_heads = qkv_heads;
  c.w = add_param(P.params, key + ".weight", {cout, cin, k, k});
  c.b = add_param(P.params, key + ".bias", {cout});
  return c;
}

static BlockP make_block(mcedm_plan& P, const std::string& key, int cin, int cout, bool up, bool down, bool attn) {
  const int emb = P.desc.ch;
  BlockP b;
  b.key = key; b.cin = cin; b.cout = cout; b.up = up; b.down = down;
  b.heads = attn ? cout / P.desc.channels_per_head : 0;
  b.attn = b.heads > 0;
  b.norm0 = make_norm(P, key + ".norm0", cin);
  b.conv0 = make_conv(P, key + ".conv0", cin, cout, 3);
  b.aff_w = add_param(P.params, key + ".affine.weight", {2 * cout, emb});
  b.aff_b = add_param(P.params, key + ".affine.bias", {2 * cout});
  b.norm1 = make_norm(P, key + ".norm1", cout);
  b.conv1 = make_conv(P, key + ".conv1", cout, cout, 3);
  b.skip_kernel = -1;
  if (cout != cin || up || down) {
    b.skip_kernel = (cout != cin) ? 1 : 0;
    if (b.skip_kernel == 1) b.skip = make_conv(P, key + ".skip", cin, cout, 1);
  }
  if (b.attn) {
    b.norm2 = make_norm(P, key + ".norm2", cout);
    b.qkv = make_conv(P, key + ".qkv", cout, 3 * cout, 1, b.heads);
    b.proj = make_conv(P, key + ".proj", cout, cout, 1);
  }
  return b;
}

static void place_conv(Taker& t, ConvP& c, bool dgrad) {
  c.wpk = t.take(conv_packed_floats(c.cout, c.cin, c.taps));
  c.bias = t.take((size_t)(c.cout + 31) / 32 * 32);
  if (dgrad) c.wpk_dgrad = t.take(conv_packed_floats(c.cin, c.cout, c.taps));
  if (c.taps == 9 && c.qkv_heads == 0) {
    if (c.cout % 64 == 0 && c.cin % 8 == 0) c.wino = t.take(conv_wino_packed_floats(c.cout, c.cin));
    if (dgrad && c.cin % 64 == 0 && c.cout % 8 == 0) c.wino_dgrad = t.take(conv_wino_packed_floats(c.cin, c.cout));
  }
}
static void place_skip_frag(Taker& t, ConvP& c) {
  if (c.taps == 1 && c.cout % 128 == 0 && c.cin % 16 == 0 && c.cin >= 32 && c.cin <= 256) c.wfrag = t.take(conv_frag_packed_floats(c.cout, c.cin));
}
static void place_norm(Taker& t, NormP& n) { n.gamma = t.take(n.C); n.beta = t.take(n.C); }

}

using namespace mcedm;

extern "C" int mcedm_version(void) { return MCEDM_ABI_VERSION; }

extern "C" int mcedm_unet_plan_set_variant(mcedm_plan* plan, int which, int value) {
  return plan_set_variant(plan, "plan_set_variant", which, value);
}
extern "C" const char* mcedm_last_error(void) { return g_err; }

extern "C" int mcedm_unet_plan_create(const mcedm_unet_desc* d, mcedm_plan** out) {
  MCEDM_REQUIRE(d && out, "plan_create: null argument");
  MCEDM_REQUIRE(d->n_levels >= 1 && d->n_levels <= MCEDM_MAX_LEVELS, "plan_create: n_levels=%d out of range", d->n_levels);
  MCEDM_REQUIRE(d->n_attn_resolutions >= 0 && d->n_attn_resolutions <= MCEDM_MAX_LEVELS, "plan_create: bad n_attn_resolutions");
  MCEDM_REQUIRE(d->in_channels > 0 && d->out_channels > 0 && d->cond_channels >= 0, "plan_create: bad channel counts");
  MCEDM_REQUIRE(d->ch > 0 && d->ch % 8 == 0, "plan_create: ch=%d must be a positive multiple of 8", d->ch);
  MCEDM_REQUIRE(d->num_res_blocks >= 1, "plan_create: num_res_blocks must be >= 1");
  if (d->channels_per_head != 64) {
    set_error("plan_create: channels_per_head=%d unsupported (the hot path uses 64, adm_blocks.py:223)", d->channels_per_head);
    return MCEDM_ERR_UNSUPPORTED;
  }
  for (int l = 0; l < d->n_levels; ++l) {
    const int c = d->ch * d->ch_mult[l];
    MCEDM_REQUIRE(d->ch_mult[l] >= 1 && c % 8 == 0, "plan_create: level %d width %d must be a multiple of 8", l, c);
  }
  MCEDM_REQUIRE(d->dx_mode == MCEDM_DX_NONE || d->dx_mode == MCEDM_DX_CAT || d->dx_mode == MCEDM_DX_ENC, "plan_create: dx_mode=%d", d->dx_mode);
  MCEDM_REQUIRE((d->dx_mode == MCEDM_DX_NONE) == (d->dx_channels == 0) && d->dx_channels >= 0,
                "plan_create: dx_channels=%d does not go with dx_mode=%d", d->dx_channels, d->dx_mode);
  mcedm_plan* Pp = new mcedm_plan();
  mcedm_plan& P = *Pp;
  P.desc = *d;
  P.levels_div = 1 << (d->n_levels - 1);
  const int ch = d->ch;
  auto key = [&](const char* side, int res, const std::string& tail) {
    return std::string(side) + "." + std::to_string(res) + "x" + std::to_string(res) + "_" + tail;
  };
  P.map0_w = add_param(P.params, "map_layer0.weight", {ch, ch});
  P.map0_b = add_param(P.params, "map_layer0.bias", {ch});
  P.map1_w = add_param(P.params, "map_layer1.weight", {ch, ch});
  P.map1_b = add_param(P.params, "map_layer1.bias", {ch});
  if (d->dx_mode == MCEDM_DX_ENC) {
    const int c0 = ch * d->ch_mult[0];
    P.dx_enc0 = make_conv(P, "dx_enc.0", d->dx_channels, c0, 3);
    P.dx_enc2 = make_conv(P, "dx_enc.2", c0, c0, 3);
// ... 224 lines not shown
  for (auto* v : {&P.enc, &P.dec})
    for (const BlockP& b : *v) {
      cp.add(params[b.aff_w], pk + P.waff + (size_t)b.film_row0 * ch, (size_t)2 * b.cout * ch);
      cp.add(params[b.aff_b], pk + P.baff + b.film_row0, (size_t)2 * b.cout);
      pack_norm(b.norm0, params, pk, cp);
      pack_norm(b.norm1, params, pk, cp);
      if ((rc = pack_conv(b.conv0, params, pk, cp, pp, s))) return rc;
      if ((rc = pack_conv(b.conv1, params, pk, cp, pp, s))) return rc;
      if (b.skip_kernel == 1 && (rc = pack_conv(b.skip, params, pk, cp, pp, s))) return rc;
      if (b.attn) {
        pack_norm(b.norm2, params, pk, cp);
        if ((rc = pack_conv(b.qkv, params, pk, cp, pp, s))) return rc;
        if ((rc = pack_conv(b.proj, params, pk, cp, pp, s))) return rc;
      }
    }
  pack_norm(P.out_norm, params, pk, cp);
  if ((rc = pack_conv(P.conv_out, params, pk, cp, pp, s))) return rc;
  cp.flush();
  pp.flush();
  return cp.status != MCEDM_OK ? cp.status : pp.status;
}

namespace mcedm {

struct LayoutBuilder {
  Layout& L;
  Pool pool;
  int B;
  int make(int C, int H, int W, size_t bytes) {
    TRef t;
    t.C = C; t.H = H; t.W = W; t.bytes = bytes;
    t.off = pool.alloc(bytes);
    L.t.push_back(t);
    return (int)L.t.size() - 1;
  }
  int act(int C, int H, int W) { return make(C, H, W, (size_t)B * C * H * W * sizeof(float)); }
  int coef(int C) { return make(C, 1, 1, (size_t)B * C * sizeof(Coef)); }
  int stats(int groups) { return make(groups, 1, 1, (size_t)B * groups * 2 * sizeof(float)); }
  void retain(int id) { if (id >= 0) L.t[id].ref++; }
  void release(int id) {
    if (id < 0) return;
    if (--L.t[id].ref == 0) pool.release(L.t[id].off, L.t[id].bytes);
  }
  void drop(int id) { if (id >= 0) pool.release(L.t[id].off, L.t[id].bytes); }
};

int build_layout(const mcedm_plan& P, int B, int H, int W, int training, int n_noise, Layout* out) {
  MCEDM_REQUIRE(B > 0 && H > 0 && W > 0, "layout: empty shape B=%d H=%d W=%d", B, H, W);
  MCEDM_REQUIRE(H % P.levels_div == 0 && W % P.levels_div == 0,
                "layout: H=%d W=%d must be multiples of %d (2^(levels-1))", H, W, P.levels_div);
  MCEDM_REQUIRE(n_noise == 1 || n_noise == B, "layout: n_noise=%d must be 1 or B=%d", n_noise, B);
  Layout& L = *out;
  L = Layout();
  LayoutBuilder lb{L, Pool(), B};
  lb.pool.keep_all = training != 0;
  L.film = lb.make(P.film_rows, 1, 1, (size_t)n_noise * P.film_rows * sizeof(float));
  auto sums_sz = [&](int C, int h, int w) { return align_up((size_t)B * conv_max_tiles(h, w) * ceil_div(C, 4) * 2 * sizeof(float), 256); };
  {
    size_t need = sums_sz(P.conv_in.cout, H, W);
    int h = H, w = W;
    for (auto* v : {&P.enc, &P.dec})
      for (const BlockP& b : *v) {
        if (b.up) { h *= 2; w *= 2; } else if (b.down) { h /= 2; w /= 2; }
        need += (size_t)(b.attn ? 3 : 2) * sums_sz(b.cout, h, w);
      }
    L.sums_bytes = need;
    const int id = lb.make(1, 1, 1, need);
    L.sums_base = L.t[id].off;
  }
  size_t sums_cur = L.sums_base;
  auto give_sums = [&](int id) {
    L.t[id].sums = sums_cur;
    sums_cur += sums_sz(L.t[id].C, L.t[id].H, L.t[id].W);
  };
  if (P.desc.dx_mode == MCEDM_DX_CAT) L.xdx = lb.act(P.desc.in_channels + P.desc.dx_channels, H, W);
  if (P.desc.dx_mode == MCEDM_DX_ENC) {
    L.xf = lb.act(P.conv_in.cout, H, W);
    L.d1 = lb.act(P.conv_in.cout, H, W);
    L.g1 = lb.act(P.conv_in.cout, H, W);
    L.d2 = lb.act(P.conv_in.cout, H, W);
  }
  L.t0 = lb.act(P.conv_in.cout, H, W);
  give_sums(L.t0);
  lb.drop(L.xdx); lb.drop(L.xf); lb.drop(L.d1); lb.drop(L.g1); lb.drop(L.d2);
  std::vector<int> skips;
  int cur = L.t0;
  lb.retain(cur);
  lb.retain(cur); skips.push_back(cur);

  auto do_block = [&](const BlockP& b, int xa, int xb) {
    BlockLayout bl;
    bl.xa = xa; bl.xb = xb;
    bl.Hin = L.t[xa].H; bl.Win = L.t[xa].W;
    bl.H = b.up ? bl.Hin * 2 : (b.down ? bl.Hin / 2 : bl.Hin);
    bl.W = b.up ? bl.Win * 2 : (b.down ? bl.Win / 2 : bl.Win);
    bl.coef0 = lb.coef(b.cin);
    if (training) bl.stats0 = lb.stats(b.norm0.groups);
    if (b.down) bl.xd = lb.act(b.cin, bl.H, bl.W);
    bl.h = lb.act(b.cout, bl.H, bl.W);
    give_sums(bl.h);
    lb.drop(bl.coef0); lb.drop(bl.xd);
    bl.coef1 = lb.coef(b.cout);
    if (training) bl.stats1 = lb.stats(b.norm1.groups);
    const bool wino1 = b.conv1.wino != NONE && conv_wino_shape_ok(b.cout, b.cout, bl.H, bl.W);
    const bool wfold = wino1 && !training && !b.up && !b.down && b.skip_kernel == 1 && b.skip.wfrag != NONE &&
                       conv_wino_fold_shape_ok(b.cout, L.t[xa].C, xb >= 0 ? L.t[xb].C : 0, bl.H, bl.W);
// ... 44 lines not shown
  L.coef_out = lb.coef(P.out_norm.C);
  if (training) L.stats_out = lb.stats(P.out_norm.groups);
  L.total_bytes = lb.pool.peak;
  return MCEDM_OK;
}

Header header_for(const mcedm_plan& P, int B, int H, int W) {
  Header h;
  size_t cur = 0;
  auto take = [&](size_t bytes) { size_t o = cur; cur += align_up(bytes, 256); return o; };
  const int Ct = P.desc.in_channels + P.desc.cond_channels + P.desc.dx_channels;
  h.coefs4 = take((size_t)B * 4 * sizeof(float));
  h.c_noise = take((size_t)B * sizeof(float));
  h.coef_in = take((size_t)B * Ct * sizeof(Coef));
  h.F = take((size_t)B * P.desc.out_channels * H * W * sizeof(float));
  h.Fu = take((size_t)B * P.desc.out_channels * H * W * sizeof(float));
  h.total = cur;
  return h;
}

float* AdmNet::F() const { return at<float>(ws, hd.F); }
float* AdmNet::Fu() const { return at<float>(ws, hd.Fu); }
Coef* AdmNet::coef_in() const { return at<Coef>(ws, hd.coef_in); }
float* AdmNet::c_noise() const { return at<float>(ws, hd.c_noise); }
float* AdmNet::coefs4() const { return at<float>(ws, hd.coefs4); }

void AdmNet::place(const void* packed, void* region, void* stream) {
  pk = (const float*)packed; ws = (char*)region; act = ws + hd.total; s = (hipStream_t)stream;
}

int adm_sizes(const mcedm_plan& P, int B, int H, int W, int training, int n_noise, AdmNet* net, size_t* bytes) {
  const int rc = build_layout(P, B, H, W, training, n_noise, &net->L);
  if (rc) return rc;
  net->plan = &P; net->hd = header_for(P, B, H, W);
  net->B = B; net->H = H; net->W = W; net->n_noise = n_noise;
  *bytes = net->hd.total + net->L.total_bytes;
  return MCEDM_OK;
}

static int gn_for_conv(const GnArgs& g, ConvArgs& c, bool need_table, hipStream_t s) {
  if (!need_table && g.stats == nullptr && gn_sums_usable(g)) {
    c.gn = g; c.gn_on = 1; c.coef = nullptr;
    return MCEDM_OK;
  }
  return launch_gn_coef_from_sums(g, s);
}

ConvArgs AdmNet::conv(const ConvP& cv, const float* xa, int Ca, const float* xb, int Cb, int Hs, int Ws, int H, int W, int dst,
                      std::vector<SumTiles>& st) const {
  ConvArgs c{};
  c.xa = xa; c.Ca = Ca; c.xb = xb; c.Cb = Cb;
  c.Hs = Hs; c.Ws = Ws; c.H = H; c.W = W;
  c.wpk = pk + cv.wpk; c.bias = pk + cv.bias;
  c.wino = cv.wino != NONE ? pk + cv.wino : nullptr;
  c.out = T(dst); c.Cout = cv.cout; c.B = B;
  c.gsum = SUMS(dst); c.gsum_tiles = c.gsum ? &st[dst] : nullptr;
  return c;
}

int AdmNet::run_block(const BlockP& b, const BlockLayout& bl, std::vector<SumTiles>& st) const {
  const mcedm_plan& P = *plan;
  auto TL = [&](int id) -> SumTiles { return id < 0 ? SumTiles{} : st[id]; };
  const float* xa = T(bl.xa);
  const float* xb = T(bl.xb);
  const int Ca = L.t[bl.xa].C, Cb = bl.xb >= 0 ? L.t[bl.xb].C : 0;
  const float eps = P.desc.eps;
  int rc;
  GnArgs g0{xa, xb, Ca, Cb, bl.Hin * bl.Win, B, b.norm0.groups, pk + b.norm0.gamma, pk + b.norm0.beta,
            nullptr, 0, 0, eps, CF(bl.coef0), T(bl.stats0), SUMS(bl.xa), SUMS(bl.xb), TL(bl.xa), TL(bl.xb), bl.Win};
  const int rs = b.up ? RS_UP : (b.down ? RS_DOWN : RS_NONE);
  ConvArgs c0 = conv(b.conv0, xa, Ca, xb, Cb, bl.Hin, bl.Win, bl.H, bl.W, bl.h, st);
  c0.coef = CF(bl.coef0); c0.coef_batch = 1; c0.act = 1; c0.resample = rs;
  if ((rc = gn_for_conv(g0, c0, bl.xd >= 0, s))) return rc;
  if (bl.xd >= 0) {
    WgradArgs m{};
    m.xa = xa; m.xb = xb; m.Ca = Ca; m.Cb = Cb; m.coef = c0.coef; m.coef_batch = 1; m.act = 1; m.resample = RS_DOWN;
    m.Hs = bl.Hin; m.Ws = bl.Win; m.H = bl.H; m.W = bl.W; m.B = B;
    if ((rc = launch_act_materialize(m, T(bl.xd), s))) return rc;
    c0.xa = T(bl.xd); c0.xb = nullptr; c0.Ca = Ca + Cb; c0.Cb = 0;
    c0.coef = nullptr; c0.act = 0; c0.resample = RS_NONE; c0.Hs = bl.H; c0.Ws = bl.W;
  }
  if ((rc = launch_conv(c0, 9, s))) return rc;
  GnArgs g1{T(bl.h), nullptr, b.cout, 0, bl.H * bl.W, B, b.norm1.groups, pk + b.norm1.gamma, pk + b.norm1.beta,
            film() + b.film_row0, coef_batch(), P.film_rows, eps, CF(bl.coef1), T(bl.stats1), SUMS(bl.h), nullptr, TL(bl.h), SumTiles{}, bl.W};
  const float* res = xa;
  int res_mode = RS_NONE;
  const bool fold_skip = b.skip_kernel == 1 && (bl.sk < 0 || bl.wfold);
  if (b.skip_kernel == 1 && !fold_skip) {
    ConvArgs cs = conv(b.skip, xa, Ca, xb, Cb, bl.Hin, bl.Win, bl.H, bl.W, bl.sk, st);
    cs.resample = rs;
    if ((rc = launch_conv(cs, 1, s))) return rc;
    res = T(bl.sk);
  } else if (b.skip_kernel == 0) {
    res_mode = rs;
  }
  ConvArgs c1 = conv(b.conv1, T(bl.h), b.cout, nullptr, 0, bl.H, bl.W, bl.H, bl.W, bl.y, st);
  c1.coef = CF(bl.coef1); c1.coef_batch = 1; c1.act = 1;
  c1.res = res; c1.res_mode = res_mode;
  if (fold_skip) {
    c1.res = nullptr; c1.res_mode = RS_NONE;
    c1.sk_xa = xa; c1.sk_xb = xb; c1.sk_Ca = Ca; c1.sk_Cb = Cb;
    c1.sk_wpk = pk + b.skip.wpk; c1.sk_bias = pk + b.skip.bias;
    c1.sk_wfrag = b.skip.wfrag != NONE ? pk + b.skip.wfrag : nullptr;
  }
  if ((rc = gn_for_conv(g1, c1, false, s))) return rc;
  if ((rc = launch_conv(c1, 9, s))) return rc;
  if (!b.attn) return MCEDM_OK;
// ... 171 lines not shown
```

m-cedm_amd/csrc/plan.hpp:

```cpp
#pragma once
#include <algorithm>
#include <initializer_list>
#include <string>
#include <utility>
#include <vector>

#include "common.hpp"

namespace mcedm {

constexpr size_t NONE = (size_t)-1;

struct Pool {
  std::vector<std::pair<size_t, size_t>> free_;
  size_t top = 0, peak = 0;
  bool keep_all = false;
  size_t alloc(size_t bytes) {
    bytes = align_up(bytes ? bytes : 1, 256);
    for (size_t i = 0; i < free_.size(); ++i)
      if (free_[i].second >= bytes) {
        const size_t off = free_[i].first;
        if (free_[i].second == bytes) free_.erase(free_.begin() + i);
        else { free_[i].first += bytes; free_[i].second -= bytes; }
        return off;
// ... 78 lines not shown
  int w = -1, b = -1;
  int cin = 0, cout = 0, taps = 0;
  int qkv_heads = 0;
  size_t wpk = NONE, bias = NONE;
  size_t wpk_dgrad = NONE;
  size_t wino = NONE, wino_dgrad = NONE;
  size_t wfrag = NONE;
};

struct NormP {
  int w = -1, b = -1;
  int C = 0, groups = 0;
  size_t gamma = NONE, beta = NONE;
};

struct BlockP {
  std::string key;
  int cin = 0, cout = 0;
  bool up = false, down = false, attn = false;
  int heads = 0;
  int skip_kernel = -1;
  NormP norm0, norm1, norm2;
  ConvP conv0, conv1, skip, qkv, proj;
  int aff_w = -1, aff_b = -1;
  int film_row0 = 0;
};

struct TRef {
  size_t off = NONE;
  int C = 0, H = 0, W = 0;
  size_t bytes = 0;
  size_t sums = NONE;
  int sum_tiles = 0;
  int ref = 0;
};

struct BlockLayout {
  int xa = -1, xb = -1;
  int coef0 = -1, h = -1, coef1 = -1, sk = -1, y = -1, coef2 = -1, qkv = -1, a = -1, z = -1;
  int stats0 = -1, stats1 = -1, stats2 = -1;
  int xd = -1;
  int out = -1;
  int wfold = 0;
  int Hin = 0, Win = 0, H = 0, W = 0;
};

struct Layout {
  std::vector<TRef> t;
  std::vector<BlockLayout> blocks;
  int film = -1, t0 = -1, coef_out = -1, stats_out = -1, last = -1;
  int xdx = -1, xf = -1, d1 = -1, g1 = -1, d2 = -1;
  size_t sums_base = 0, sums_bytes = 0;
  size_t total_bytes = 0;
};

}

struct mcedm_plan {
  mcedm_unet_desc desc;
  std::vector<mcedm::ParamInfo> params;
  mcedm::ConvP conv_in, conv_out;
  mcedm::ConvP dx_enc0, dx_enc2, combine;
  mcedm::NormP out_norm;
  std::vector<mcedm::BlockP> enc, dec;
  int map0_w = -1, map0_b = -1, map1_w = -1, map1_b = -1;
  size_t freqs = mcedm::NONE, w0 = mcedm::NONE, b0 = mcedm::NONE, w1 = mcedm::NONE, b1 = mcedm::NONE;
  size_t waff = mcedm::NONE, baff = mcedm::NONE;
  int film_rows = 0;
  size_t packed_floats = 0;
  int levels_div = 1;
  mcedm::KernelVariants variants;
};

namespace mcedm {
int build_layout(const mcedm_plan& P, int B, int H, int W, int training, int n_noise, Layout* out);

struct Header {
  size_t coefs4, c_noise, coef_in, F, Fu, total;
};
Header header_for(const mcedm_plan& P, int B, int H, int W);

template <class T>
static inline T* at(void* ws, size_t off) { return reinterpret_cast<T*>(reinterpret_cast<char*>(ws) + off); }

static inline int heun_check_workspace(const char* who, size_t have, size_t need) {
  if (need > have) {
    set_error("%s: workspace too small (%zu < %zu bytes)", who, have, need);
    return MCEDM_ERR_WORKSPACE;
  }
  return MCEDM_OK;
}

struct AdmIn {
  const float* x = nullptr;
  const float* dx = nullptr;
  const float* cond = nullptr;
  const Coef* coef_in = nullptr;
  const float* noise_labels = nullptr;
};

struct AdmNet {
  const mcedm_plan* plan = nullptr;
  const float* pk = nullptr;
  Layout L;
  Header hd{};
  char* ws = nullptr;
// ... 49 lines not shown
```

m-cedm_amd/lib.py:

```python
from __future__ import annotations

import ctypes as C
import os
from typing import Dict, List, Optional, Sequence

import torch

_HERE = os.path.dirname(os.path.abspath(__file__))
LIB_PATH = os.environ.get("MCEDM_LIB") or os.path.join(_HERE, "libmcedm_hip.so")
MAX_LEVELS = 8

EXPORTS = [
    "mcedm_version", "mcedm_last_error", "mcedm_unet_plan_create", "mcedm_unet_plan_destroy",
    "mcedm_unet_param_count", "mcedm_unet_param_info", "mcedm_unet_packed_bytes", "mcedm_unet_pack_weights",
    "mcedm_unet_workspace_bytes", "mcedm_unet_forward", "mcedm_edm_denoise", "mcedm_sampler_workspace_bytes",
    "mcedm_heun_sample", "mcedm_edm_t_steps", "mcedm_edm_loss", "mcedm_edm_noise_inputs",
    "mcedm_edm_denoise_backward", "mcedm_edm_denoise_backward_bucketed", "mcedm_unet_grad_buckets", "mcedm_sqnorm",
    "mcedm_adam_ema_step",
    "mcedm_swe_fv_step", "mcedm_swe_fv_residual", "mcedm_darcy_residual", "mcedm_swe_fv_guidance", "mcedm_darcy_guidance",
    "mcedm_heun_sample_guided",
    "mcedm_ddpm_plan_create", "mcedm_ddpm_plan_destroy", "mcedm_ddpm_param_count", "mcedm_ddpm_param_info",
    "mcedm_ddpm_packed_bytes", "mcedm_ddpm_pack_weights", "mcedm_ddpm_workspace_bytes", "mcedm_ddpm_forward",
    "mcedm_ddpm_denoise", "mcedm_repaint_schedule", "mcedm_repaint_workspace_bytes", "mcedm_repaint_sample",
    "mcedm_repaint_sample_rng", "mcedm_normal_fill", "mcedm_ddpm_forward_sc", "mcedm_ddim_workspace_bytes",
    "mcedm_ddim_repaint_sample", "mcedm_ddim_timesteps",
    "mcedm_unet_forward_dx", "mcedm_edm_denoise_dx", "mcedm_edm_denoise_backward_dx", "mcedm_heun_sample_dxcond",
    "mcedm_unet_plan_set_variant", "mcedm_ddpm_plan_set_variant", "mcedm_heun_sample_rng",
    "mcedm_eps_noise_inputs", "mcedm_eps_self_cond", "mcedm_eps_loss", "mcedm_unet_backward", "mcedm_unet_backward_bucketed",
    "mcedm_vp_sampler_workspace_bytes", "mcedm_vp_heun_sample", "mcedm_vp_heun_sample_rng",
    "mcedm_cond_ddim_workspace_bytes", "mcedm_cond_ddim_sample",
    "mcedm_uniform_fill", "mcedm_cond_ddim_sample_rng", "mcedm_ddim_repaint_sample_rng", "mcedm_heun_sample_guided_rng",
    "mcedm_heun_sample_dxcond_rng",
    "mcedm_ddpm_plan_create_cond", "mcedm_ddpm_cond_map", "mcedm_ddpm_forward_cond", "mcedm_ddpm_vp_sampler_workspace_bytes",
    "mcedm_ddpm_vp_heun_sample", "mcedm_ddpm_vp_heun_sample_rng", "mcedm_ddpm_cond_ddim_workspace_bytes",
    "mcedm_ddpm_cond_ddim_sample", "mcedm_ddpm_cond_ddim_sample_rng",
    "mcedm_ddpm_forward_cat", "mcedm_ddpm_edm_denoise", "mcedm_ddpm_edm_sampler_workspace_bytes", "mcedm_ddpm_edm_heun_sample",
    "mcedm_ddpm_edm_heun_sample_rng",
    "mcedm_swe_fv_unroll",
    "mcedm_ddpm_temb_row_count", "mcedm_ddpm_temb_rows", "mcedm_ddpm_workspace_bytes_t", "mcedm_ddpm_forward_t",
    "mcedm_ddpm_edm_denoise_t",
]
SAMPLER_STEMS = {
    "mcedm_heun_sample": 1, "mcedm_heun_sample_guided": 1, "mcedm_heun_sample_dxcond": 1,
    "mcedm_vp_heun_sample": 1, "mcedm_ddpm_vp_heun_sample": 1, "mcedm_cond_ddim_sample": 1, "mcedm_ddpm_cond_ddim_sample": 1,
    "mcedm_ddim_repaint_sample": 1, "mcedm_repaint_sample": 2, "mcedm_ddpm_edm_heun_sample": 1,
}
GN_SYNC_WORDS = 130
VARIANTS = {"conv_wino": 0, "conv_wino1": 1, "conv_resident": 2, "conv8": 3, "attn_fused": 4, "wgrad_wino": 5, "conv1x1_reg": 6,
            "conv_wino_fold": 7, "conv_wino_upz": 8}


class UNetDesc(C.Structure):
    _fields_ = [("in_channels", C.c_int32), ("cond_channels", C.c_int32), ("out_channels", C.c_int32),
                ("ch", C.c_int32), ("n_levels", C.c_int32), ("ch_mult", C.c_int32 * MAX_LEVELS),
                ("num_res_blocks", C.c_int32), ("resolution", C.c_int32), ("n_attn_resolutions", C.c_int32),
                ("attn_resolutions", C.c_int32 * MAX_LEVELS), ("channels_per_head", C.c_int32), ("eps", C.c_float),
                ("dx_channels", C.c_int32), ("dx_mode", C.c_int32)]


DX_NONE, DX_CAT, DX_ENC = 0, 1, 2
ABI_VERSION = 4
REDUCE_SCRATCH_BYTES = 4096 * 8 + 64
SWE_UNROLL_MAX_X = 4096


class SamplerDesc(C.Structure):
    _fields_ = [("timesteps", C.c_int32), ("sigma_min", C.c_double), ("sigma_max", C.c_double), ("rho", C.c_double),
                ("S_churn", C.c_double), ("S_min", C.c_double), ("S_max", C.c_double), ("S_noise", C.c_double),
                ("w", C.c_double), ("sigma_data", C.c_double), ("net_sigma_min", C.c_double),
                ("net_sigma_max", C.c_double)]


class GuidanceDesc(C.Structure):
    _fields_ = [("system", C.c_int32), ("half_dt", C.c_float), ("dx", C.c_float), ("two_dx", C.c_float), ("sub_h", C.c_float),
                ("div_h", C.c_float), ("sub_u", C.c_float), ("div_u", C.c_float), ("weight", C.c_double)]


class DdpmDesc(C.Structure):
    _fields_ = [("in_channels", C.c_int32), ("out_channels", C.c_int32), ("ch", C.c_int32), ("n_levels", C.c_int32),
                ("ch_mult", C.c_int32 * MAX_LEVELS), ("num_res_blocks", C.c_int32), ("resolution", C.c_int32),
                ("n_attn_resolutions", C.c_int32), ("attn_resolutions", C.c_int32 * MAX_LEVELS), ("self_cond", C.c_int32),
                ("eps", C.c_float)]


class DdpmCondDesc(C.Structure):
    _fields_ = [("cond_channels", C.c_int32), ("cat_cond", C.c_int32)]


class RepaintDesc(C.Structure):
    _fields_ = [("timesteps", C.c_int32), ("sigma_min", C.c_double), ("sigma_max", C.c_double), ("rho", C.c_double),
                ("S_churn", C.c_double), ("S_min", C.c_double), ("S_max", C.c_double), ("S_noise", C.c_double),
                ("w", C.c_double), ("n_repeat", C.c_int32), ("n_time_h", C.c_int32), ("n_time_u", C.c_int32),
                ("h_ch", C.c_int32), ("u_ch", C.c_int32), ("num_diffusion_timesteps", C.c_int32),
                ("edm_steps", C.POINTER(C.c_float)), ("alphas_cumprod_ext", C.POINTER(C.c_float))]


class DdimDesc(C.Structure):
    _fields_ = [("timesteps", C.c_int32), ("skip_type", C.c_int32), ("eta", C.c_double), ("n_repeat", C.c_int32),
                ("n_time_h", C.c_int32), ("n_time_u", C.c_int32), ("h_ch", C.c_int32), ("u_ch", C.c_int32),
                ("num_diffusion_timesteps", C.c_int32), ("self_cond", C.c_int32), ("alphas_cumprod_ext", C.POINTER(C.c_float))]


# ... 1112 lines not shown
    check(load().mcedm_darcy_residual(_ptr(pred), _ptr(out), B, S, two_dx, denom, int(clamp), _stream()), "darcy_residual")
    return out


def sqnorm(g: torch.Tensor, out: Optional[torch.Tensor] = None, scratch: Optional[torch.Tensor] = None) -> torch.Tensor:
    if out is None:
        out = torch.empty(1, dtype=torch.float64, device=g.device)
    scratch = reduce_scratch(g.device) if scratch is None else scratch
    check(load().mcedm_sqnorm(_ptr(g), g.numel(), _ptr(out, torch.float64), scratch.data_ptr(),
                              scratch.numel() * scratch.element_size(), _stream()), "sqnorm")
    return out


def adam_ema_step(param, grad, exp_avg, exp_avg_sq, ema, step, lr=2e-4, beta1=0.9, beta2=0.999, eps=1e-8,
                  weight_decay=0.0, sqnorm_t=None, max_norm=1.0, grad_scale=1.0, ema_beta=0.999):
    check(load().mcedm_adam_ema_step(_ptr(param), _ptr(grad), _ptr(exp_avg), _ptr(exp_avg_sq), _ptr(ema), param.numel(),
                                     lr, beta1, beta2, eps, weight_decay, _ptr(sqnorm_t, torch.float64), max_norm,
                                     grad_scale, ema_beta, int(step), _stream()), "adam_ema_step")


_OPS_BOUND = False


def _bind_ops():
    global _OPS_BOUND
    lib = load()
    if _OPS_BOUND:
        return lib
    vp, i32, sz = C.c_void_p, C.c_int, C.c_size_t
    lib.mcedm_op_conv_packed_floats.argtypes = [i32, i32, i32]
    lib.mcedm_op_conv_packed_floats.restype = sz
    lib.mcedm_op_pack_conv.argtypes = [vp, vp, i32, i32, i32, i32, i32, vp, vp, vp]
    lib.mcedm_op_gn_coef.argtypes = [vp, vp, i32, i32, i32, i32, vp, vp, vp, i32, i32, C.c_float, vp, vp, vp]
    lib.mcedm_op_conv.argtypes = [vp, vp, i32, i32, vp, i32, i32, i32, i32, i32, i32, i32, vp, vp, vp, i32, vp, i32,
                                  i32, i32, vp]
    lib.mcedm_op_attention.argtypes = [vp, vp, i32, i32, i32, vp]
    lib.mcedm_op_attn_block64.argtypes = [vp, vp, vp, C.c_float, vp, vp, vp, vp, vp, vp, i32, vp]
    lib.mcedm_op_embedding.argtypes = [vp, i32, i32, vp, vp, vp, vp, vp, vp, i32, vp, vp, vp, vp]
    lib.mcedm_op_wgrad_scratch_floats.argtypes = [i32, i32, i32, i32, i32, i32]
    lib.mcedm_op_wgrad_scratch_floats.restype = sz
    lib.mcedm_op_conv_wgrad.argtypes = [vp, vp, vp, i32, i32, vp, i32, i32, i32, i32, i32, i32, i32, i32, i32, i32, i32,
                                        vp, vp, vp, vp]
    lib.mcedm_op_gn_bwd.argtypes = [vp, i32, vp, vp, i32, i32, i32, i32, i32, vp, vp, vp, vp, vp, i32, i32, i32, vp, vp,
                                    i32, vp, i32, vp, vp, vp, vp, i32, vp]
    lib.mcedm_op_gn_bwd_sync.argtypes = [vp, i32, vp, vp, i32, i32, i32, i32, i32, vp, vp, vp, vp, vp, i32, i32, i32, vp, vp,
                                         i32, vp, i32, vp, vp, vp, vp, i32, vp, vp]
    lib.mcedm_op_attention_bwd.argtypes = [vp, vp, vp, vp, vp, i32, i32, i32, vp]
    lib.mcedm_op_conv_wino_packed_floats.argtypes = [i32, i32]
    lib.mcedm_op_conv_wino_packed_floats.restype = sz
    lib.mcedm_op_pack_conv_wino.argtypes = [vp, i32, i32, vp, vp]
    lib.mcedm_op_pack_conv_wino_dgrad.argtypes = [vp, i32, i32, vp, vp]
    lib.mcedm_op_conv_wino.argtypes = [vp, vp, i32, i32, vp, i32, i32, i32, i32, i32, vp, vp, vp, i32, vp, i32, i32, vp]
    lib.mcedm_op_conv_wino_sums.argtypes = [vp, vp, i32, i32, vp, i32, i32, i32, i32, i32, vp, vp, vp, i32, vp, vp, i32, i32, vp]
    lib.mcedm_op_conv_bias_batch.argtypes = [vp, vp, i32, i32, vp, i32, i32, i32, i32, i32, i32, i32, vp, vp, i32, vp, i32, vp, i32,
                                             i32, i32, vp]
    lib.mcedm_op_conv_wino_sums_bias_batch.argtypes = [vp, vp, i32, i32, vp, i32, i32, i32, i32, i32, vp, vp, i32, vp, i32, vp, vp, i32,
                                                       i32, vp]
    lib.mcedm_op_pack_conv_frag.argtypes = [vp, i32, i32, vp, vp]
    lib.mcedm_op_conv_skip.argtypes = [vp, i32, vp, i32, i32, i32, vp, vp, vp, vp, vp, vp, i32, i32, vp, vp, vp, vp, vp, i32, i32, vp]
    f32 = C.c_float
    lib.mcedm_op_conv_sums.argtypes = [vp, vp, i32, i32, vp, i32, i32, i32, i32, i32, i32, i32, vp, vp, vp, i32, vp, i32, vp, i32, i32, i32,
                                       vp, i32, vp, vp]
    lib.mcedm_op_gn_coef_from_sums.argtypes = [vp, vp, vp, vp, i32, i32, i32, i32, i32, i32, vp, vp, vp, i32, i32, f32, vp, vp, vp]
    lib.mcedm_op_conv_gn.argtypes = [vp, vp, i32, i32, vp, vp, vp, vp, i32, vp, vp, vp, i32, i32, f32, i32, i32, i32, i32, i32, i32, vp, vp,
                                     vp, vp, i32, vp, i32, i32, i32, vp]
    lib.mcedm_op_ddim_cond_step.argtypes = [vp, vp, vp, vp, C.c_double, f32, f32, f32, f32, f32, vp, vp, vp, i32, i32, i32, i32, i32,
                                            i32, vp, i32, i32, vp, i32, i32, vp]
    lib.mcedm_op_ddim_cond_step_rng.argtypes = [vp, vp, vp, vp, C.c_uint64, C.c_double, f32, f32, f32, f32, f32, vp, vp, vp, i32, i32,
                                                i32, i32, i32, i32, vp, i32, i32, vp, i32, i32, vp]
    for n in ("mcedm_op_pack_conv", "mcedm_op_gn_coef", "mcedm_op_conv", "mcedm_op_attention", "mcedm_op_embedding", "mcedm_op_conv_wgrad",
              "mcedm_op_gn_bwd", "mcedm_op_gn_bwd_sync", "mcedm_op_attention_bwd", "mcedm_op_pack_conv_wino", "mcedm_op_conv_wino",
              "mcedm_op_conv_wino_sums", "mcedm_op_pack_conv_wino_dgrad", "mcedm_op_ddim_cond_step", "mcedm_op_ddim_cond_step_rng", "mcedm_op_pack_conv_frag", "mcedm_op_conv_skip",
              "mcedm_op_attn_block64", "mcedm_op_conv_bias_batch", "mcedm_op_conv_wino_sums_bias_batch", "mcedm_op_conv_sums",
              "mcedm_op_gn_coef_from_sums", "mcedm_op_conv_gn"):
        getattr(lib, n).restype = C.c_int
    _OPS_BOUND = True
    return lib


OP_EXPORTS = ["mcedm_op_conv_packed_floats", "mcedm_op_pack_conv", "mcedm_op_gn_coef", "mcedm_op_conv",
              "mcedm_op_attention", "mcedm_op_set_conv_tile", "mcedm_prof_enable", "mcedm_prof_report",
              "mcedm_op_wgrad_scratch_floats", "mcedm_op_conv_wgrad", "mcedm_op_gn_bwd", "mcedm_op_attention_bwd",
              "mcedm_op_set_conv_debug", "mcedm_op_set_conv8", "mcedm_op_set_conv_resident", "mcedm_op_set_attn_fused", "mcedm_op_embedding",
              "mcedm_op_conv_wino_packed_floats", "mcedm_op_pack_conv_wino", "mcedm_op_conv_wino", "mcedm_op_set_conv_wino", "mcedm_op_set_conv_wino1",
              "mcedm_op_set_wgrad_wino", "mcedm_op_set_conv1x1_reg", "mcedm_op_gn_bwd_sync", "mcedm_op_pack_conv_wino_dgrad",
              "mcedm_op_ddim_cond_step", "mcedm_op_ddim_cond_step_rng", "mcedm_op_set_conv_wino_fold", "mcedm_op_set_conv_wino_upz", "mcedm_op_conv_wino_sums", "mcedm_op_pack_conv_frag", "mcedm_op_conv_skip",
              "mcedm_op_attn_block64", "mcedm_op_conv_bias_batch", "mcedm_op_conv_wino_sums_bias_batch", "mcedm_op_conv_sums",
              "mcedm_op_gn_coef_from_sums", "mcedm_op_conv_gn"]


def prof_enable(on: bool) -> None:
    lib = load()
    lib.mcedm_prof_enable.argtypes = [C.c_int]
    check(lib.mcedm_prof_enable(int(on)), "prof_enable")


def prof_report() -> list:
    import json
    lib = load()
    lib.mcedm_prof_report.argtypes = [C.c_char_p, C.c_size_t]
    buf = C.create_string_buffer(1 << 16)
    check(lib.mcedm_prof_report(buf, len(buf)), "prof_report")
    return json.loads(buf.value.decode())


def set_conv_tile(mt: int = 0, ph: int = 0, pw: int = 0) -> None:
    lib = _bind_ops()
    lib.mcedm_op_set_conv_tile.argtypes = [C.c_int, C.c_int, C.c_int]
    check(lib.mcedm_op_set_conv_tile(mt, ph, pw), "set_conv_tile")
def set_conv8(enable: int = -1) -> None:
    lib = _bind_ops()
    lib.mcedm_op_set_conv8.argtypes = [C.c_int]
    check(lib.mcedm_op_set_conv8(int(enable)), "set_conv8")


def set_conv_wino(enable: int = -1) -> None:
    lib = _bind_ops()
    lib.mcedm_op_set_conv_wino.argtypes = [C.c_int]
    check(lib.mcedm_op_set_conv_wino(int(enable)), "set_conv_wino")


def set_conv_wino1(enable: int = -1) -> None:
    lib = _bind_ops()
    lib.mcedm_op_set_conv_wino1.argtypes = [C.c_int]
    check(lib.mcedm_op_set_conv_wino1(int(enable)), "set_conv_wino1")


def set_conv1x1_reg(enable: int = -1) -> None:
    lib = _bind_ops()
    lib.mcedm_op_set_conv1x1_reg.argtypes = [C.c_int]
    check(lib.mcedm_op_set_conv1x1_reg(int(enable)), "set_conv1x1_reg")


def set_conv_wino_fold(enable: int = -1) -> None:
    lib = _bind_ops()
    lib.mcedm_op_set_conv_wino_fold.argtypes = [C.c_int]
    check(lib.mcedm_op_set_conv_wino_fold(int(enable)), "set_conv_wino_fold")


def set_conv_wino_upz(enable: int = -1) -> None:
    lib = _bind_ops()
    lib.mcedm_op_set_conv_wino_upz.argtypes = [C.c_int]
    check(lib.mcedm_op_set_conv_wino_upz(int(enable)), "set_conv_wino_upz")


def set_wgrad_wino(enable: int = -1) -> None:
    lib = _bind_ops()
    lib.mcedm_op_set_wgrad_wino.argtypes = [C.c_int]
    check(lib.mcedm_op_set_wgrad_wino(int(enable)), "set_wgrad_wino")


def set_conv_resident(enable: int = -1) -> None:
    lib = _bind_ops()
    lib.mcedm_op_set_conv_resident.argtypes = [C.c_int]
    check(lib.mcedm_op_set_conv_resident(int(enable)), "set_conv_resident")


def set_attn_fused(enable: int = -1) -> None:
    lib = _bind_ops()
    lib.mcedm_op_set_attn_fused.argtypes = [C.c_int]
    check(lib.mcedm_op_set_attn_fused(int(enable)), "set_attn_fused")


def set_conv_debug(buf: Optional[torch.Tensor] = None) -> None:
    lib = _bind_ops()
    lib.mcedm_op_set_conv_debug.argtypes = [C.c_void_p]
    if buf is not None and (not buf.is_cuda or buf.element_size() != 8 or not buf.is_contiguous() or buf.numel() % 16):
        raise ValueError("set_conv_debug: buf must be a contiguous device tensor of 64-bit words, 16 per workgroup")
    check(lib.mcedm_op_set_conv_debug(buf.data_ptr() if buf is not None else None), "set_conv_debug")


RS_NONE, RS_UP, RS_DOWN, RS_S2 = 0, 1, 2, 3


def op_pack_conv(w: torch.Tensor, b: Optional[torch.Tensor], qkv_heads: int = 0, dgrad: bool = False):
    lib = _bind_ops()
    Cout, Cin, k, _ = w.shape
    rows, cols = (Cin, Cout) if dgrad else (Cout, Cin)
    n = lib.mcedm_op_conv_packed_floats(rows, cols, k)
    wpk = torch.empty(n, dtype=torch.float32, device=w.device)
    bpk = torch.zeros((Cout + 31) // 32 * 32, dtype=torch.float32, device=w.device) if b is not None else None
    check(lib.mcedm_op_pack_conv(_ptr(w), _ptr(b), Cout, Cin, k, qkv_heads, int(dgrad), _ptr(wpk), _ptr(bpk), _stream()),
          "op_pack_conv")
    return wpk, bpk


def op_gn_coef(xa, xb, gamma, beta, film=None, film_batch=0, film_stride=0, eps=1e-5, want_stats=False):
    lib = _bind_ops()
    B, Ca = xa.shape[:2]
    Cb = xb.shape[1] if xb is not None else 0
    HW = xa[0, 0].numel()
    Ct = Ca + Cb
    coef = torch.empty((B, Ct, 4), dtype=torch.float32, device=xa.device)
    stats = torch.empty((B, min(32, Ct // 4), 2), dtype=torch.float32, device=xa.device) if want_stats else None
    check(lib.mcedm_op_gn_coef(_ptr(xa), _ptr(xb), Ca, Cb, B, HW, _ptr(gamma), _ptr(beta), _ptr(film), film_batch,
                               film_stride, eps, _ptr(coef), _ptr(stats), _stream()), "op_gn_coef")
# ... 7 lines not shown
    Cb = xb.shape[1] if xb is not None else 0
    H, W = (Hs * 2, Ws * 2) if resample == RS_UP else ((Hs // 2, Ws // 2) if resample in (RS_DOWN, RS_S2) else (Hs, Ws))
    if out is None:
        out = torch.empty((B, Cout, H, W), dtype=torch.float32, device=xa.device)
    if bias_batch:
        if bias_pk is None or bias_pk.numel() < (B - 1) * bias_batch + Cout:
            raise RuntimeError(f"op_conv: bias_batch={bias_batch} needs a bias of {B} rows")
        check(lib.mcedm_op_conv_bias_batch(_ptr(xa), _ptr(xb), Ca, Cb, _ptr(coef), coef_batch, act, resample, Hs, Ws, H, W, _ptr(wpk),
                                           _ptr(bias_pk), int(bias_batch), _ptr(res), res_mode, _ptr(out), Cout, B, k, _stream()),
              "op_conv_bias_batch")
        return out
    check(lib.mcedm_op_conv(_ptr(xa), _ptr(xb), Ca, Cb, _ptr(coef), coef_batch, act, resample, Hs, Ws, H, W, _ptr(wpk),
                            _ptr(bias_pk), _ptr(res), res_mode, _ptr(out), Cout, B, k, _stream()), "op_conv")
    return out


def op_pack_conv_wino(w: torch.Tensor, dgrad: bool = False) -> torch.Tensor:
    lib = _bind_ops()
    Cout, Cin = w.shape[:2]
    if dgrad:
        wino = torch.empty(lib.mcedm_op_conv_wino_packed_floats(Cin, Cout), dtype=torch.float32, device=w.device)
        check(lib.mcedm_op_pack_conv_wino_dgrad(_ptr(w), Cout, Cin, _ptr(wino), _stream()), "op_pack_conv_wino_dgrad")
        return wino
    wino = torch.empty(lib.mcedm_op_conv_wino_packed_floats(Cout, Cin), dtype=torch.float32, device=w.device)
    check(lib.mcedm_op_pack_conv_wino(_ptr(w), Cout, Cin, _ptr(wino), _stream()), "op_pack_conv_wino")
    return wino


def op_conv_wino(xa, xb, wino, bias, Cout, coef=None, coef_batch=1, act=0, resample=RS_NONE, res=None, res_mode=RS_NONE,
                 out=None, want_sums=False, bias_batch=0):
    lib = _bind_ops()
    B, Ca, Hs, Ws = xa.shape
    Cb = xb.shape[1] if xb is not None else 0
    H, W = (Hs * 2, Ws * 2) if resample == RS_UP else (Hs, Ws)
    if out is None:
        out = torch.empty((B, Cout, H, W), dtype=torch.float32, device=xa.device)
    if bias_batch and (not want_sums or bias is None or bias.numel() < (B - 1) * bias_batch + Cout):
        raise RuntimeError(f"op_conv_wino: bias_batch={bias_batch} goes with want_sums and a bias of {B} rows")
    if want_sums:
        gsum = torch.zeros(B * ((H + 3) // 4) * ((W + 7) // 8) * ((Cout + 3) // 4) * 2, dtype=torch.float32, device=xa.device)
        if bias_batch:
            check(lib.mcedm_op_conv_wino_sums_bias_batch(_ptr(xa), _ptr(xb), Ca, Cb, _ptr(coef), coef_batch, act, resample, H, W,
                                                         _ptr(wino), _ptr(bias), int(bias_batch), _ptr(res), res_mode, _ptr(out),
                                                         _ptr(gsum), Cout, B, _stream()), "op_conv_wino_sums_bias_batch")
            return out, gsum
        check(lib.mcedm_op_conv_wino_sums(_ptr(xa), _ptr(xb), Ca, Cb, _ptr(coef), coef_batch, act, resample, H, W, _ptr(wino),
                                          _ptr(bias), _ptr(res), res_mode, _ptr(out), _ptr(gsum), Cout, B, _stream()), "op_conv_wino_sums")
        return out, gsum
    check(lib.mcedm_op_conv_wino(_ptr(xa), _ptr(xb), Ca, Cb, _ptr(coef), coef_batch, act, resample, H, W, _ptr(wino),
                                 _ptr(bias), _ptr(res), res_mode, _ptr(out), Cout, B, _stream()), "op_conv_wino")
    return out


def op_pack_conv_frag(w: torch.Tensor) -> torch.Tensor:
    lib = _bind_ops()
    Cout, Cin = w.shape[:2]
    wfrag = torch.empty((Cout + 31) // 32 * 32 * ((Cin + 7) // 8 * 8), dtype=torch.float32, device=w.device)
    check(lib.mcedm_op_pack_conv_frag(_ptr(w), Cout, Cin, _ptr(wfrag), _stream()), "op_pack_conv_frag")
    return wfrag


def op_conv_skip(x, wpk, wino, bias, Cout, coef=None, act=1, res=None, sk_xa=None, sk_xb=None, sk_wpk=None, sk_wfrag=None,
                 sk_bias=None, want_sums=False):
    lib = _bind_ops()
    B, Cin, H, W = x.shape
    out = torch.empty((B, Cout, H, W), dtype=torch.float32, device=x.device)
    gsum = torch.zeros(B * ((H + 3) // 4) * ((W + 7) // 8) * ((Cout + 3) // 4) * 2, dtype=torch.float32, device=x.device) if want_sums else None
    check(lib.mcedm_op_conv_skip(_ptr(x), Cin, _ptr(coef), act, H, W, _ptr(wpk), _ptr(wino), _ptr(bias), _ptr(res), _ptr(sk_xa), _ptr(sk_xb),
                                 sk_xa.shape[1] if sk_xa is not None else 0, sk_xb.shape[1] if sk_xb is not None else 0, _ptr(sk_wpk),
                                 _ptr(sk_wfrag), _ptr(sk_bias), _ptr(out), _ptr(gsum), Cout, B, _stream()), "op_conv_skip")
    return (out, gsum) if want_sums else out


def _conv_hw(xa, resample):
    Hs, Ws = xa.shape[2:]
    H, W = (Hs * 2, Ws * 2) if resample == RS_UP else ((Hs // 2, Ws // 2) if resample in (RS_DOWN, RS_S2) else (Hs, Ws))
    return Hs, Ws, H, W


def _tiling_arg(t):
    return None if t is None else (C.c_int * 5)(*[int(v) for v in t])


def op_conv_sums(xa, xb, wpk, bias_pk, Cout, k, rc=4, wino=None, coef=None, coef_batch=1, act=0, resample=RS_NONE, res=None,
                 res_mode=RS_NONE, bias_batch=0):
    lib = _bind_ops()
    B, Ca = xa.shape[:2]
    Cb = xb.shape[1] if xb is not None else 0
    Hs, Ws, H, W = _conv_hw(xa, resample)
    out = torch.empty((B, Cout, H, W), dtype=torch.float32, device=xa.device)
    nrec = -(-Cout // (2 if rc == 2 else 4))
    gsum = torch.full((B * ((H + 3) // 4) * ((W + 7) // 8) * nrec * 2,), float("nan"), dtype=torch.float32, device=xa.device)
    tiling = (C.c_int * 5)()
    check(lib.mcedm_op_conv_sums(_ptr(xa), _ptr(xb), Ca, Cb, _ptr(coef), coef_batch, act, resample, Hs, Ws, H, W, _ptr(wpk), _ptr(wino),
                                 _ptr(bias_pk), int(bias_batch), _ptr(res), res_mode, _ptr(out), Cout, B, k, _ptr(gsum), int(rc), tiling,
                                 _stream()), "op_conv_sums")
    tiling = tuple(tiling)
    if tiling[0] > ((H + 3) // 4) * ((W + 7) // 8):
        raise RuntimeError(f"op_conv_sums: the launcher reports {tiling[0]} tiles, beyond the table")
    return out, gsum[:B * tiling[0] * nrec * 2].view(B, tiling[0], nrec, 2), tiling


def op_gn_coef_from_sums(suma, tiling_a, Ca, H, W, groups, gamma, beta, sumb=None, tiling_b=None, Cb=0, film=None, film_batch=0,
                         film_stride=0, eps=1e-5):
    lib = _bind_ops()
    B = suma.shape[0]
# ... 116 lines not shown
```

Baseline: 82.35 states/s.

## Add split-Cout Winograd conv variant for small low-resolution feature maps

Adds a Winograd 3x3 conv kernel variant for images below the Winograd minimum size. It splits the Winograd transform positions across waves, with each wave handling two positions for a 32-channel output block, and spreads output blocks over the grid so small images still fill the GPU. The output transform goes through an LDS dump and also does the residual add, 2x2-mean downsampled residual and group-norm partial sums. Winograd weights are now packed for Cout%32, training and dgrad paths keep the old routing, and the variant is on by default unless resident conv is chosen explicitly.

Result: faster. 83.41 states/s, median of 6 (+1.3%).

```diff
diff --git a/include/mcedm_hip.h b/include/mcedm_hip.h
--- a/include/mcedm_hip.h
+++ b/include/mcedm_hip.h
@@ -66,6 +66,7 @@
 #define MCEDM_VARIANT_CONV1X1_REG 6
 #define MCEDM_VARIANT_CONV_WINO_FOLD 7
 #define MCEDM_VARIANT_CONV_WINO_UPZ 8
+#define MCEDM_VARIANT_CONV_WINO_SPLIT 9
 int mcedm_unet_plan_set_variant(mcedm_plan* plan, int which, int value);
 
 int mcedm_unet_param_count(const mcedm_plan* plan);
@@ -228,6 +229,12 @@
 int mcedm_op_conv_wino_sums(const float* xa, const float* xb, int Ca, int Cb, const mcedm_coef* coef, int coef_batch, int act,
                             int resample, int H, int W, const float* wino, const float* bias, const float* res, int res_mode,
                             float* out, float* gsum, int Cout, int B, void* stream);
+int mcedm_op_conv_wino_split(const float* xa, const float* xb, int Ca, int Cb, const mcedm_coef* coef, int coef_batch, int act,
+                             int H, int W, const float* wino, const float* bias, const float* res, int res_mode, float* out, int Cout,
+                             int B, void* stream);
+int mcedm_op_conv_wino_split_sums(const float* xa, const float* xb, int Ca, int Cb, const mcedm_coef* coef, int coef_batch, int act,
+                                  int H, int W, const float* wino, const float* bias, const float* res, int res_mode, float* out,
+                                  float* gsum, int Cout, int B, void* stream);
 int mcedm_op_conv_bias_batch(const float* xa, const float* xb, int Ca, int Cb, const mcedm_coef* coef, int coef_batch, int act,
                              int resample, int Hs, int Ws, int H, int W, const float* wpk, const float* bias_pk, int bias_batch,
                              const float* res, int res_mode, float* out, int Cout, int B, int k, void* stream);
@@ -275,6 +282,7 @@
 int mcedm_op_set_conv1x1_reg(int enable);
 int mcedm_op_set_conv_wino_fold(int enable);
 int mcedm_op_set_conv_wino_upz(int enable);
+int mcedm_op_set_conv_wino_split(int enable);
 int mcedm_op_pack_conv_frag(const float* w, int Cout, int Cin, float* wfrag, void* stream);
 int mcedm_op_conv_skip(const float* x, int Cin, const mcedm_coef* coef, int act, int H, int W, const float* wpk, const float* wino,
                        const float* bias, const float* res, const float* sk_xa, const float* sk_xb, int sk_Ca, int sk_Cb,
diff --git a/m-cedm_amd/csrc/backward.hip b/m-cedm_amd/csrc/backward.hip
--- a/m-cedm_amd/csrc/backward.hip
+++ b/m-cedm_amd/csrc/backward.hip
@@ -165,7 +165,7 @@
   a.xa = dy; a.Ca = cv.cout;
   a.Hs = H; a.Ws = W; a.H = H; a.W = W;
   a.wpk = c.pk + cv.wpk_dgrad;
-  a.wino = cv.wino_dgrad != NONE ? c.pk + cv.wino_dgrad : nullptr;
+  a.wino = cv.wino_dgrad != NONE && !conv_wino_small(H, W) ? c.pk + cv.wino_dgrad : nullptr;
   a.out = out; a.Cout = cv.cin; a.B = c.B;
   return launch_conv(a, cv.taps, c.s);
 }
diff --git a/m-cedm_amd/csrc/common.hpp b/m-cedm_amd/csrc/common.hpp
--- a/m-cedm_amd/csrc/common.hpp
+++ b/m-cedm_amd/csrc/common.hpp
@@ -38,8 +38,8 @@
   } while (0)
 
 enum KernelVariant { KV_CONV_WINO = 0, KV_CONV_WINO1 = 1, KV_CONV_RESIDENT = 2, KV_CONV8 = 3, KV_ATTN_FUSED = 4, KV_WGRAD_WINO = 5,
-                     KV_CONV1X1_REG = 6, KV_CONV_WINO_FOLD = 7, KV_CONV_WINO_UPZ = 8, KV_COUNT = 9 };
-struct KernelVariants { int v[KV_COUNT] = {-1, -1, -1, -1, -1, -1, -1, -1, -1}; };
+                     KV_CONV1X1_REG = 6, KV_CONV_WINO_FOLD = 7, KV_CONV_WINO_UPZ = 8, KV_CONV_WINO_SPLIT = 9, KV_COUNT = 10 };
+struct KernelVariants { int v[KV_COUNT] = {-1, -1, -1, -1, -1, -1, -1, -1, -1, -1}; };
 const KernelVariants* current_variants();
 struct VariantScope {
   const KernelVariants* prev;
@@ -153,6 +153,12 @@
 void set_conv_wino(int enable);
 bool conv_wino_preferred(const ConvArgs& a);
 int launch_conv_wino(const ConvArgs& a, hipStream_t stream);
+bool conv_wino_split_applicable(const ConvArgs& a, int taps);
+bool conv_wino_split_preferred();
+bool conv_wino_small(int H, int W);
+int launch_conv_wino_split(const ConvArgs& a, hipStream_t stream);
+void set_conv_wino_split(int enable);
+bool conv_resident_explicit();
 static inline int cout_padded(int Cout) { return (Cout + 31) / 32 * 32; }
 int conv_resolve_identity(ConvArgs& a);
 unsigned long long* conv_debug_buffer();
diff --git a/m-cedm_amd/csrc/conv_mfma.hip b/m-cedm_amd/csrc/conv_mfma.hip
--- a/m-cedm_amd/csrc/conv_mfma.hip
+++ b/m-cedm_amd/csrc/conv_mfma.hip
@@ -810,6 +810,7 @@
     return launch_small_cout(a, stream);
   if (a.resample == RS_S2) return dispatch_s2(a, stream);
   if (!g_force_mt && taps == 9 && a.wino && (a.bias_batch == 0 || a.act) && conv_wino_preferred(a) && conv_wino_applicable(a, taps)) return launch_conv_wino(a, stream);
+  if (!g_force_mt && !conv_resident_explicit() && conv_wino_split_preferred() && conv_wino_split_applicable(a, taps)) return launch_conv_wino_split(a, stream);
   if (!g_force_mt && taps == 1) {
     const int rc = try_launch_conv1x1_reg(a, taps, stream);
     if (rc != -1) return rc;
diff --git a/m-cedm_amd/csrc/conv_resident.hip b/m-cedm_amd/csrc/conv_resident.hip
--- a/m-cedm_amd/csrc/conv_resident.hip
+++ b/m-cedm_amd/csrc/conv_resident.hip
@@ -481,6 +481,7 @@
   if (env < 0) { const char* e = getenv("MCEDM_CONV_RESIDENT"); env = e ? atoi(e) : 1; }
   return variant_choice(KV_CONV_RESIDENT, g_resident, env);
 }
+bool conv_resident_explicit() { return variant_choice(KV_CONV_RESIDENT, g_resident, -1) >= 0; }
 
 static constexpr int LDS_MAX = 160 * 1024;
 static int big_level() {
diff --git a/m-cedm_amd/csrc/conv_wino.hip b/m-cedm_amd/csrc/conv_wino.hip
--- a/m-cedm_amd/csrc/conv_wino.hip
+++ b/m-cedm_amd/csrc/conv_wino.hip
@@ -136,6 +136,8 @@
   constexpr bool UPS = WinoUpTraits<Tag...>::UPS;
   static_assert(!UPS || UPZ, "source-resolution staging is part of the zero-position variant");
   static_assert(!UPZ || (UP && !SKIP), "the zero positions belong to the up-sampled input");
+  constexpr bool SPLIT = C::SPLIT;
+  static_assert(!SPLIT || (!UP && !SKIP && sizeof...(Tag) == 0 && MB == 4 && WSC == 2), "the split variant: plain input, WinoCfg<4>'s input path");
   extern __shared__ float lds[];
   const int Cin = p.Ca + p.Cb;
   float* const vbuf = lds;
@@ -152,12 +154,19 @@
   if (p.dbg && tid == 0) { p.dbg[blockIdx.x * 16 + 0] = __builtin_amdgcn_s_memrealtime(); p.dbg[blockIdx.x * 16 + 4] = per; }
   int gt0 = blockIdx.x * per, tstep = 1;
   int n = gt0 / tiles_img, tile0 = gt0 % tiles_img;
-  if (mode & 256) {
+  if (!SPLIT && (mode & 256)) {
     const int nwg = gridDim.x, wps = tiles_img / per;
     const int lid = (nwg % 8 == 0) ? (int)(blockIdx.x % 8) * (nwg / 8) + (int)(blockIdx.x / 8) : (int)blockIdx.x;
     n = lid / wps; tile0 = lid % wps; tstep = wps;
   }
-  const int m0 = blockIdx.y * C::MT;
+  int split_mb = 0;
+  if constexpr (SPLIT) {
+    const int nwg = gridDim.x, nmb = p.Cout / C::MT;
+    const int lid = (nwg % 8 == 0) ? (int)(blockIdx.x % 8) * (nwg / 8) + (int)(blockIdx.x / 8) : (int)blockIdx.x;
+    split_mb = lid % nmb;
+    n = (lid / nmb) / tiles_img; tile0 = (lid / nmb) % tiles_img;
+  }
+  const int m0 = SPLIT ? split_mb * C::MT : blockIdx.y * C::MT;
   const size_t HW = (size_t)p.H * p.W, HWs = (size_t)p.Hs * p.Ws;
   const int nst = (nch + WSC - 1) / WSC;
   const int G = per * nst;
@@ -356,9 +365,15 @@
   if (G > 2) raw_load();
   const size_t ustride = (size_t)mblocks * 16 * 64;
   constexpr int PHF = UPZ ? 12 : 8;
-  const f32x4* up = reinterpret_cast<const f32x4*>(p.wino) + ((size_t)(m0 / 32 + mb) * 16 + PHF * hf) * 64 + lane;
+  const f32x4* up = reinterpret_cast<const f32x4*>(p.wino) + (SPLIT ? ((size_t)(m0 / 32) * 16 + 2 * wave) : ((size_t)(m0 / 32 + mb) * 16 + PHF * hf)) * 64 + lane;
   f32x4 ua[8];
-  if constexpr (UPZ) {
+  f32x4 wa[WSC][2];
+  if constexpr (SPLIT) {
+#pragma unroll
+    for (int sc = 0; sc < WSC; ++sc)
+#pragma unroll
+      for (int q = 0; q < 2; ++q) wa[sc][q] = up[(size_t)(sc < nch ? sc : 0) * ustride + q * 64];
+  } else if constexpr (UPZ) {
     const f32x4 zero4 = {0.f, 0.f, 0.f, 0.f};
     ua[0] = up[0 * 64]; ua[1] = up[1 * 64]; ua[3] = up[3 * 64];
     ua[4] = zero4; ua[5] = zero4; ua[7] = zero4;
@@ -375,11 +390,16 @@
     const f32x16 zero16 = {0.f, 0.f, 0.f, 0.f, 0.f, 0.f, 0.f, 0.f, 0.f, 0.f, 0.f, 0.f, 0.f, 0.f, 0.f, 0.f};
     float z = 0.f;
 #pragma unroll
-    for (int q = 0; q < 8; ++q) {
+    for (int q = 0; q < (SPLIT ? 2 : 8); ++q) {
       asm volatile("" : "+v"(z));
       acc[q] = __builtin_amdgcn_mfma_f32_32x32x2f32(z, z, zero16, 0, 0, 0);
     }
-    if (hf == 0) {
+    if constexpr (SPLIT) {
+      if (wave == 2) {
+#pragma unroll
+        for (int r = 0; r < 16; ++r) acc[1][r] = bias_l[4 * (lane >> 5) + (r & 3) + 8 * (r >> 2)];
+      }
+    } else if (hf == 0) {
 #pragma unroll
       for (int r = 0; r < 16; ++r) acc[5][r] = bias_l[32 * mb + 4 * (lane >> 5) + (r & 3) + 8 * (r >> 2)];
     }
@@ -387,7 +407,7 @@
   __syncthreads();
   init_acc();
 
-  const int vrd = (PHF * hf) * VPOS + (lane >> 5) * VH1 + (lane & 31) * 4;
+  const int vrd = (SPLIT ? 2 * wave : PHF * hf) * VPOS + (lane >> 5) * VH1 + (lane & 31) * 4;
   if (p.dbg && tid == 0) { p.dbg[blockIdx.x * 16 + 1] = __builtin_amdgcn_s_memrealtime(); p.dbg[blockIdx.x * 16 + 5] = __builtin_amdgcn_s_memtime(); }
 #ifdef MCEDM_WINO_TIMELINE
   unsigned long long ph[5] = {0, 0, 0, 0, 0}, tlast = __builtin_amdgcn_s_memtime();
@@ -440,6 +460,43 @@
     const int cur = g & 1;
     WINO_STAMP(0)
     WINO_SLOT0
+    if constexpr (SPLIT) {
+      f32x4 bf[WSC][2], wn[WSC][2];
+#pragma unroll
+      for (int sc = 0; sc < WSC; ++sc) {
+        const float* vb = vbuf + cur * VBUF + sc * 16 * VPOS + vrd;
+        bf[sc][0] = *reinterpret_cast<const f32x4*>(vb);
+        bf[sc][1] = *reinterpret_cast<const f32x4*>(vb + VPOS);
+      }
+#pragma unroll
+      for (int sc = 0; sc < WSC; ++sc) {
+        const int cn = (st + 1) * WSC + sc;
+        const f32x4* un = up + (size_t)(cn < nch ? cn : 0) * ustride;
+        wn[sc][0] = un[0];
+        wn[sc][1] = un[64];
+      }
+      __builtin_amdgcn_sched_barrier(0);
+#pragma unroll
+      for (int sc = 0; sc < WSC; ++sc) {
+#pragma unroll
+        for (int s = 0; s < 4; ++s) {
+          acc[0] = __builtin_amdgcn_mfma_f32_32x32x2f32(wa[sc][0][s], bf[sc][0][s], acc[0], 0, 0, 0);
+          acc[1] = __builtin_amdgcn_mfma_f32_32x32x2f32(wa[sc][1][s], bf[sc][1][s], acc[1], 0, 0, 0);
+          side_slice(sc * 4 + s, g, cur);
+#pragma unroll
+          for (int i = 0; i < 2; ++i) {
+            __builtin_amdgcn_sched_group_barrier(0x008, 1, 0);
+            __builtin_amdgcn_sched_group_barrier(0x486, 4 * WINO_IL_K, 0);
+          }
+          __builtin_amdgcn_sched_group_barrier(0x020, 4, 0);
+          __builtin_amdgcn_sched_barrier(0);
+          if (sc * 4 + s == 5) raw_load_next();
+          __builtin_amdgcn_sched_barrier(0);
+        }
+      }
+#pragma unroll
+      for (int sc = 0; sc < WSC; ++sc) { wa[sc][0] = wn[sc][0]; wa[sc][1] = wn[sc][1]; }
+    } else {
 #pragma unroll
     for (int sc = 0; sc < WSC; ++sc) {
       const int c = st * WSC + sc;
@@ -518,12 +575,104 @@
       }
       }
     }
+    }
     WINO_STAMP(1)
     __syncthreads();
     WINO_STAMP(2)
     if (++st < nst) continue;
     st = 0;
 
+    if constexpr (SPLIT) {
+      const int y0 = (tile / tiles_x) * WPH, x0 = (tile % tiles_x) * WPW;
+      float* const dump = lds;
+#pragma unroll
+      for (int q = 0; q < 2; ++q)
+#pragma unroll
+        for (int r = 0; r < 16; ++r) dump[((2 * wave + q) * 16 + r) * 64 + lane] = acc[q][r];
+      const int ehf = wave >> 2, gq = wave & 3, pt = lane & 31;
+      const int oy = y0 + 2 * (pt >> 3) + ehf, ox = x0 + 2 * (pt & 7);
+      const int cbase = m0 + 8 * gq + 4 * (lane >> 5);
+      const size_t splane = (size_t)p.Cout * HW;
+      const __amdgpu_buffer_rsrc_t rs_out = make_rsrc(p.out + (size_t)n * splane, 4u * (unsigned)splane);
+      const size_t rplane = p.res_mode == RS_DOWN ? splane << 2 : splane;
+      const __amdgpu_buffer_rsrc_t rs_res = make_rsrc(p.res ? p.res + (size_t)n * rplane : nullptr, p.res ? 4u * (unsigned)rplane : 0u);
+      const unsigned HWu = (unsigned)HW;
+      const unsigned voff = 4u * ((unsigned)cbase * HWu + (unsigned)oy * p.W + ox);
+      float2 rv[4];
+      if (p.res && p.res_mode == RS_DOWN) {
+        const unsigned dvoff = 4u * ((unsigned)cbase * (HWu << 2) + (unsigned)(2 * oy) * (unsigned)(2 * p.W) + (unsigned)(2 * ox));
+        f32x4 ta[4], tb[4];
+#pragma unroll
+        for (int k = 0; k < 4; ++k) {
+          const unsigned so = 4u * (unsigned)k * (HWu << 2);
+          ta[k] = __builtin_bit_cast(f32x4, __builtin_amdgcn_raw_buffer_load_b128(rs_res, dvoff, so, 0));
+          tb[k] = __builtin_bit_cast(f32x4, __builtin_amdgcn_raw_buffer_load_b128(rs_res, dvoff + 8u * (unsigned)p.W, so, 0));
+        }
+#pragma unroll
+        for (int k = 0; k < 4; ++k)
+          rv[k] = make_float2(0.25f * ((ta[k][0] + ta[k][1]) + (tb[k][0] + tb[k][1])), 0.25f * ((ta[k][2] + ta[k][3]) + (tb[k][2] + tb[k][3])));
+      } else {
+#pragma unroll
+        for (int k = 0; k < 4; ++k) rv[k] = __builtin_bit_cast(float2, __builtin_amdgcn_raw_buffer_load_b64(rs_res, voff, 4u * (unsigned)k * HWu, 0));
+      }
+      __syncthreads();
+      float v0[4], v1[4];
+#pragma unroll
+      for (int k = 0; k < 4; ++k) {
+        float T[3][2];
+#pragma unroll
+        for (int i = 0; i < 3; ++i) {
+          const float* d = dump + ((4 * (ehf + i)) * 16 + 4 * gq + k) * 64 + lane;
+          const float a0 = d[0 * 16 * 64], a1 = d[1 * 16 * 64], a2 = d[2 * 16 * 64], a3 = d[3 * 16 * 64];
+          T[i][0] = a0 + a1 + a2;
+          T[i][1] = a1 - a2 - a3;
+        }
+        if (ehf == 0) {
+          v0[k] = (T[0][0] + T[1][0]) + T[2][0] + rv[k].x;
+          v1[k] = (T[0][1] + T[1][1]) + T[2][1] + rv[k].y;
+        } else {
+          v0[k] = (-T[1][0] - T[2][0]) + T[0][0] + rv[k].x;
+          v1[k] = (-T[1][1] - T[2][1]) + T[0][1] + rv[k].y;
+        }
+      }
+#pragma unroll
+      for (int k = 0; k < 4; ++k)
+        __builtin_amdgcn_raw_buffer_store_b64(__builtin_bit_cast(__attribute__((ext_vector_type(2))) unsigned, make_float2(v0[k], v1[k])), rs_out, voff,
+                                              4u * (unsigned)k * HWu, 0);
+      if (p.gsum) {
+        const bool pairs = p.gsum_rc == 2;
+        float a[2], b[2];
+#pragma unroll
+        for (int e = 0; e < 2; ++e) a[e] = half_sum32((v0[2 * e] + v1[2 * e]) + (v0[2 * e + 1] + v1[2 * e + 1]));
+        const float cnt = pairs ? 128.f : 256.f;
+        const float mean0 = pairs ? a[0] * (1.0f / 128.0f) : (a[0] + a[1]) * (1.0f / 256.0f);
+        const float mean1 = pairs ? a[1] * (1.0f / 128.0f) : mean0;
+#pragma unroll
+        for (int e = 0; e < 2; ++e) {
+          const float mean = e ? mean1 : mean0;
+          float q = 0.f;
+#pragma unroll
+          for (int r = 2 * e; r < 2 * e + 2; ++r) { const float d0 = v0[r] - mean, d1 = v1[r] - mean; q = fmaf(d0, d0, q); q = fmaf(d1, d1, q); }
+          b[e] = half_sum32(q);
+        }
+        if ((lane & 31) == 0) {
+          const int quad = 2 * gq + (lane >> 5);
+          if (pairs) {
+#pragma unroll
+            for (int e = 0; e < 2; ++e) {
+              float* slot = red + (ehf * (C::MT / 2) + 2 * quad + e) * 3;
+              slot[0] = cnt; slot[1] = a[e]; slot[2] = b[e];
+            }
+          } else {
+            float* slot = red + (ehf * (C::MT / 4) + quad) * 3;
+            slot[0] = cnt; slot[1] = a[0] + a[1]; slot[2] = b[0] + b[1];
+          }
+        }
+        __syncthreads();
+        conv_stats_store<C, 2>(p, red, n, m0, tile, tiles_img, tid);
+      }
+      break;
+    }
     WINO_EP(0)
     const int y0 = (tile / tiles_x) * WPH, x0 = (tile % tiles_x) * WPW;
     const int pt = lane & 31;
@@ -682,6 +831,13 @@
   static int env = -1;
   if (env < 0) { const char* e = getenv("MCEDM_WINO_UPZ"); env = e ? atoi(e) : 1; }
   return variant_choice(KV_CONV_WINO_UPZ, g_wino_upz, env);
+}
+static int g_wino_split = -1;
+void set_conv_wino_split(int enable) { g_wino_split = enable; }
+static int wino_split_env() {
+  static int env = -1;
+  if (env < 0) { const char* e = getenv("MCEDM_WINO_SPLIT"); env = e ? atoi(e) : 1; }
+  return variant_choice(KV_CONV_WINO_SPLIT, g_wino_split, env);
 }
 static int wino_mode_env() {
   static int env = -1;
@@ -845,4 +1001,53 @@
 }
 bool conv_wino_preferred(const ConvArgs& a) { return wino_env() != 0 && (long long)a.H * a.W >= wino_min_hw_env(); }
 
-}
+bool conv_wino_small(int H, int W) { return (long long)H * W < wino_min_hw_env(); }
+bool conv_wino_split_preferred() { return wino_env() != 0 && wino_split_env() != 0; }
+bool conv_wino_split_applicable(const ConvArgs& a, int taps) {
+  const int Cin = a.Ca + a.Cb;
+  return taps == 9 && a.wino && a.resample == RS_NONE && !a.sk_wpk && a.bias_batch == 0 && conv_wino_small(a.H, a.W) && a.Cout % 32 == 0 &&
+         a.H % WPH == 0 && a.W % WPW == 0 && a.Ca > 0 && a.Cb >= 0 && Cin % WKC == 0 && a.Ca % WKC == 0 && Cin <= 1024 &&
+         (((size_t)a.xa | (size_t)a.xb | (size_t)a.wino) & 15) == 0 && (!a.res || a.res_mode == RS_NONE || a.res_mode == RS_DOWN);
+}
+
+int launch_conv_wino_split(const ConvArgs& a_in, hipStream_t stream) {
+  typedef WinoSplitCfg C;
+  ConvArgs a = a_in;
+  a.dbg = nullptr;
+  MCEDM_REQUIRE(conv_wino_split_applicable(a, 9), "conv_wino_split: shape not served by the split Winograd kernel");
+  MCEDM_REQUIRE(a.out && a.B > 0 && a.Hs == a.H && a.Ws == a.W, "conv_wino_split: bad arguments");
+  MCEDM_REQUIRE((unsigned long long)a.H * a.W * 4ull * a.Cout * (a.res && a.res_mode == RS_DOWN ? 4 : 1) < (1ull << 32),
+                "conv_wino_split: one sample of the output / residual exceeds the 4 GiB buffer range");
+  { const int rc = conv_resolve_identity(a); if (rc != MCEDM_OK) return rc; }
+  const int tiles_x = a.W / WPW, tiles_img = tiles_x * (a.H / WPH), nmb = a.Cout / C::MT;
+  const long long total = (long long)a.B * tiles_img * nmb;
+  MCEDM_REQUIRE(total > 0 && total <= 0x7fffffffLL, "conv_wino_split: grid out of range");
+  const int Cin = a.Ca + a.Cb, nch = Cin / WKC;
+  const int lds_bytes = (C::LDS_ROWS_OFF + 4 * Cin + C::XCH_FLOATS + C::RED_FLOATS) * 4;
+  MCEDM_REQUIRE(lds_bytes <= 160 * 1024, "conv_wino_split: %d input channels exceed the LDS row table", Cin);
+  static std::atomic<bool> attr_set[64];
+  int dev = 0;
+  MCEDM_HIP_TRY(hipGetDevice(&dev));
+  MCEDM_REQUIRE(dev >= 0 && dev < 64, "device index %d out of range", dev);
+  if (!attr_set[dev].load(std::memory_order_acquire)) {
+    MCEDM_HIP_TRY(hipFuncSetAttribute((const void*)conv_wino_kernel<C, false>, hipFuncAttributeMaxDynamicSharedMemorySize, 160 * 1024));
+    MCEDM_HIP_TRY(hipFuncSetAttribute((const void*)conv_wino_kernel<C, false, false>, hipFuncAttributeMaxDynamicSharedMemorySize, 160 * 1024));
+    attr_set[dev].store(true, std::memory_order_release);
+  }
+  char name[64] = "";
+  if (prof_enabled()) snprintf(name, sizeof(name), "conv_wino_kernel<WinoSplitCfg, false, %s>", a.act ? "true" : "false");
+  const double px = (double)a.B * a.H * a.W;
+  ProfScope ps(name, 2.0 * px * a.Cout * (double)Cin * 9,
+               4.0 * ((double)a.B * Cin * a.H * a.W + px * a.Cout * (a.res ? 2 : 1) + (double)a.Cout * Cin * 9), stream);
+  if (a.act)
+    hipLaunchKernelGGL((conv_wino_kernel<C, false>), dim3((unsigned)total), dim3(C::NT), lds_bytes, stream, a, tiles_x, tiles_img, nch,
+                       cout_padded(a.Cout) / 32, 1, 0);
+  else
+    hipLaunchKernelGGL((conv_wino_kernel<C, false, false>), dim3((unsigned)total), dim3(C::NT), lds_bytes, stream, a, tiles_x, tiles_img, nch,
+                       cout_padded(a.Cout) / 32, 1, 0);
+  MCEDM_LAUNCH_CHECK("conv_wino_kernel");
+  if (a.gsum_tiles) *a.gsum_tiles = SumTiles{tiles_img, tiles_x, WPH, WPW, a.gsum_rc == 2 ? 2 : 4};
+  return MCEDM_OK;
+}
+
+}
diff --git a/m-cedm_amd/csrc/conv_wino.hpp b/m-cedm_amd/csrc/conv_wino.hpp
--- a/m-cedm_amd/csrc/conv_wino.hpp
+++ b/m-cedm_amd/csrc/conv_wino.hpp
@@ -18,8 +18,17 @@
   static constexpr int XCH_FLOATS = NW * 16 * 64;
   static constexpr int RED_FLOATS = 2 * (MT / 2) * 3 + MT;
   static constexpr bool SKIP = false;
+  static constexpr bool SPLIT = false;
   static_assert(MB_ == 4 || MB_ == 2, "128 or 64 output channels per workgroup");
   static_assert(LDS_ROWS_OFF % 4 == 0, "LDS layout");
+};
+struct WinoSplitCfg : WinoCfg<4> {
+  static constexpr int MT = 32;
+  static constexpr int XCH_FLOATS = 0;
+  static constexpr int RED_FLOATS = 2 * (MT / 2) * 3 + MT;
+  static constexpr int DUMP_FLOATS = 16 * 16 * 64;
+  static constexpr bool SPLIT = true;
+  static_assert(DUMP_FLOATS <= 2 * VBUF, "the accumulator dump fits the two V buffers");
 };
 template <int MB_>
 struct WinoSkipCfg : WinoCfg<MB_> {
diff --git a/m-cedm_amd/csrc/ddpm.hip b/m-cedm_amd/csrc/ddpm.hip
--- a/m-cedm_amd/csrc/ddpm.hip
+++ b/m-cedm_amd/csrc/ddpm.hip
@@ -581,7 +581,7 @@
 }
 static void dst_of(DExec& E, ConvArgs& c, int out, const DConv& cv, const float* bias, bool stats) {
   c.wpk = E.pk + cv.wpk; c.bias = bias ? bias : E.pk + cv.bias;
-  c.wino = cv.wino != NONE ? E.pk + cv.wino : nullptr;
+  c.wino = cv.wino != NONE && !conv_wino_small(E.t[out].H, E.t[out].W) ? E.pk + cv.wino : nullptr;
   c.out = E.ptr(out); c.Cout = cv.cout; c.B = E.B;
   if (stats && E.t[out].rc) { c.gsum = E.sums(out); c.gsum_rc = E.t[out].rc; c.gsum_tiles = &E.t[out].st; }
 }
diff --git a/m-cedm_amd/csrc/ops_api.hip b/m-cedm_amd/csrc/ops_api.hip
--- a/m-cedm_amd/csrc/ops_api.hip
+++ b/m-cedm_amd/csrc/ops_api.hip
@@ -120,6 +120,33 @@
                                                   float* gsum, int Cout, int B, void* stream) {
   return op_conv_wino_sums(xa, xb, Ca, Cb, coef, coef_batch, act, resample, H, W, wino, bias, bias_batch, res, res_mode, out, gsum, Cout, B,
                            stream);
+}
+
+static int op_conv_wino_split(const char* who, const float* xa, const float* xb, int Ca, int Cb, const mcedm_coef* coef, int coef_batch, int act,
+                              int H, int W, const float* wino, const float* bias, const float* res, int res_mode, float* out, float* gsum,
+                              int Cout, int B, void* stream) {
+  MCEDM_REQUIRE(res_mode == RS_NONE || res_mode == RS_DOWN, "%s: res_mode must be 0 or 2 (2x2-mean down)", who);
+  ConvArgs a{};
+  a.xa = xa; a.xb = xb; a.Ca = Ca; a.Cb = Cb;
+  a.coef = reinterpret_cast<const Coef*>(coef); a.coef_batch = coef_batch; a.act = act;
+  a.resample = RS_NONE; a.H = H; a.W = W; a.Hs = H; a.Ws = W;
+  a.wino = wino; a.bias = bias; a.res = res; a.res_mode = res_mode;
+  SumTiles st;
+  a.out = out; a.Cout = Cout; a.B = B; a.gsum = gsum; a.gsum_tiles = gsum ? &st : nullptr;
+  MCEDM_REQUIRE(conv_wino_split_applicable(a, 9),
+                "%s: needs an image below 32 x 32 with H %% 8 == 0 and W %% 16 == 0, Cout %% 32 == 0, Ca %% 8 == 0, Cin %% 8 == 0 and 16-byte aligned inputs / weight table", who);
+  return launch_conv_wino_split(a, (hipStream_t)stream);
+}
+extern "C" int mcedm_op_conv_wino_split(const float* xa, const float* xb, int Ca, int Cb, const mcedm_coef* coef, int coef_batch, int act,
+                                        int H, int W, const float* wino, const float* bias, const float* res, int res_mode, float* out,
+                                        int Cout, int B, void* stream) {
+  return op_conv_wino_split("op_conv_wino_split", xa, xb, Ca, Cb, coef, coef_batch, act, H, W, wino, bias, res, res_mode, out, nullptr, Cout, B, stream);
+}
+extern "C" int mcedm_op_conv_wino_split_sums(const float* xa, const float* xb, int Ca, int Cb, const mcedm_coef* coef, int coef_batch, int act,
+                                             int H, int W, const float* wino, const float* bias, const float* res, int res_mode, float* out,
+                                             float* gsum, int Cout, int B, void* stream) {
+  MCEDM_REQUIRE(gsum, "op_conv_wino_split_sums: gsum is null");
+  return op_conv_wino_split("op_conv_wino_split_sums", xa, xb, Ca, Cb, coef, coef_batch, act, H, W, wino, bias, res, res_mode, out, gsum, Cout, B, stream);
 }
 
 extern "C" int mcedm_op_pack_conv_frag(const float* w, int Cout, int Cin, float* wfrag, void* stream) {
@@ -343,6 +370,11 @@
 
 extern "C" int mcedm_op_set_conv_wino_upz(int enable) {
   set_conv_wino_upz(enable);
+  return MCEDM_OK;
+}
+
+extern "C" int mcedm_op_set_conv_wino_split(int enable) {
+  set_conv_wino_split(enable);
   return MCEDM_OK;
 }
 
diff --git a/m-cedm_amd/csrc/plan.hip b/m-cedm_amd/csrc/plan.hip
--- a/m-cedm_amd/csrc/plan.hip
+++ b/m-cedm_amd/csrc/plan.hip
@@ -66,7 +66,7 @@
   c.bias = t.take((size_t)(c.cout + 31) / 32 * 32);
   if (dgrad) c.wpk_dgrad = t.take(conv_packed_floats(c.cin, c.cout, c.taps));
   if (c.taps == 9 && c.qkv_heads == 0) {
-    if (c.cout % 64 == 0 && c.cin % 8 == 0) c.wino = t.take(conv_wino_packed_floats(c.cout, c.cin));
+    if (c.cout % 32 == 0 && c.cin % 8 == 0) c.wino = t.take(conv_wino_packed_floats(c.cout, c.cin));
     if (dgrad && c.cin % 64 == 0 && c.cout % 8 == 0) c.wino_dgrad = t.take(conv_wino_packed_floats(c.cin, c.cout));
   }
 }
@@ -397,6 +397,7 @@
   MCEDM_REQUIRE(n_noise == 1 || n_noise == B, "layout: n_noise=%d must be 1 or B=%d", n_noise, B);
   Layout& L = *out;
   L = Layout();
+  L.training = training != 0;
   LayoutBuilder lb{L, Pool(), B};
   lb.pool.keep_all = training != 0;
   L.film = lb.make(P.film_rows, 1, 1, (size_t)n_noise * P.film_rows * sizeof(float));
@@ -547,7 +548,7 @@
   c.xa = xa; c.Ca = Ca; c.xb = xb; c.Cb = Cb;
   c.Hs = Hs; c.Ws = Ws; c.H = H; c.W = W;
   c.wpk = pk + cv.wpk; c.bias = pk + cv.bias;
-  c.wino = cv.wino != NONE ? pk + cv.wino : nullptr;
+  c.wino = cv.wino != NONE && !(L.training && conv_wino_small(H, W)) ? pk + cv.wino : nullptr;
   c.out = T(dst); c.Cout = cv.cout; c.B = B;
   c.gsum = SUMS(dst); c.gsum_tiles = c.gsum ? &st[dst] : nullptr;
   return c;
diff --git a/m-cedm_amd/csrc/plan.hpp b/m-cedm_amd/csrc/plan.hpp
--- a/m-cedm_amd/csrc/plan.hpp
+++ b/m-cedm_amd/csrc/plan.hpp
@@ -154,6 +154,7 @@
   int xdx = -1, xf = -1, d1 = -1, g1 = -1, d2 = -1;
   size_t sums_base = 0, sums_bytes = 0;
   size_t total_bytes = 0;
+  bool training = false;
 };
 
 }
diff --git a/m-cedm_amd/lib.py b/m-cedm_amd/lib.py
--- a/m-cedm_amd/lib.py
+++ b/m-cedm_amd/lib.py
@@ -47,7 +47,7 @@
 }
 GN_SYNC_WORDS = 130
 VARIANTS = {"conv_wino": 0, "conv_wino1": 1, "conv_resident": 2, "conv8": 3, "attn_fused": 4, "wgrad_wino": 5, "conv1x1_reg": 6,
-            "conv_wino_fold": 7, "conv_wino_upz": 8}
+            "conv_wino_fold": 7, "conv_wino_upz": 8, "conv_wino_split": 9}
 
 
 class UNetDesc(C.Structure):
@@ -1266,6 +1266,8 @@
     lib.mcedm_op_pack_conv_wino_dgrad.argtypes = [vp, i32, i32, vp, vp]
     lib.mcedm_op_conv_wino.argtypes = [vp, vp, i32, i32, vp, i32, i32, i32, i32, i32, vp, vp, vp, i32, vp, i32, i32, vp]
     lib.mcedm_op_conv_wino_sums.argtypes = [vp, vp, i32, i32, vp, i32, i32, i32, i32, i32, vp, vp, vp, i32, vp, vp, i32, i32, vp]
+    lib.mcedm_op_conv_wino_split.argtypes = [vp, vp, i32, i32, vp, i32, i32, i32, i32, vp, vp, vp, i32, vp, i32, i32, vp]
+    lib.mcedm_op_conv_wino_split_sums.argtypes = [vp, vp, i32, i32, vp, i32, i32, i32, i32, vp, vp, vp, i32, vp, vp, i32, i32, vp]
     lib.mcedm_op_conv_bias_batch.argtypes = [vp, vp, i32, i32, vp, i32, i32, i32, i32, i32, i32, i32, vp, vp, i32, vp, i32, vp, i32,
                                              i32, i32, vp]
     lib.mcedm_op_conv_wino_sums_bias_batch.argtypes = [vp, vp, i32, i32, vp, i32, i32, i32, i32, i32, vp, vp, i32, vp, i32, vp, vp, i32,
@@ -1286,7 +1288,7 @@
               "mcedm_op_gn_bwd", "mcedm_op_gn_bwd_sync", "mcedm_op_attention_bwd", "mcedm_op_pack_conv_wino", "mcedm_op_conv_wino",
               "mcedm_op_conv_wino_sums", "mcedm_op_pack_conv_wino_dgrad", "mcedm_op_ddim_cond_step", "mcedm_op_ddim_cond_step_rng", "mcedm_op_pack_conv_frag", "mcedm_op_conv_skip",
               "mcedm_op_attn_block64", "mcedm_op_conv_bias_batch", "mcedm_op_conv_wino_sums_bias_batch", "mcedm_op_conv_sums",
-              "mcedm_op_gn_coef_from_sums", "mcedm_op_conv_gn"):
+              "mcedm_op_gn_coef_from_sums", "mcedm_op_conv_gn", "mcedm_op_conv_wino_split", "mcedm_op_conv_wino_split_sums"):
         getattr(lib, n).restype = C.c_int
     _OPS_BOUND = True
     return lib
@@ -1300,7 +1302,8 @@
               "mcedm_op_set_wgrad_wino", "mcedm_op_set_conv1x1_reg", "mcedm_op_gn_bwd_sync", "mcedm_op_pack_conv_wino_dgrad",
               "mcedm_op_ddim_cond_step", "mcedm_op_ddim_cond_step_rng", "mcedm_op_set_conv_wino_fold", "mcedm_op_set_conv_wino_upz", "mcedm_op_conv_wino_sums", "mcedm_op_pack_conv_frag", "mcedm_op_conv_skip",
               "mcedm_op_attn_block64", "mcedm_op_conv_bias_batch", "mcedm_op_conv_wino_sums_bias_batch", "mcedm_op_conv_sums",
-              "mcedm_op_gn_coef_from_sums", "mcedm_op_conv_gn"]
+              "mcedm_op_gn_coef_from_sums", "mcedm_op_conv_gn", "mcedm_op_conv_wino_split", "mcedm_op_conv_wino_split_sums",
+              "mcedm_op_set_conv_wino_split"]
 
 
 def prof_enable(on: bool) -> None:
@@ -1356,6 +1359,12 @@
     lib = _bind_ops()
     lib.mcedm_op_set_conv_wino_upz.argtypes = [C.c_int]
     check(lib.mcedm_op_set_conv_wino_upz(int(enable)), "set_conv_wino_upz")
+
+
+def set_conv_wino_split(enable: int = -1) -> None:
+    lib = _bind_ops()
+    lib.mcedm_op_set_conv_wino_split.argtypes = [C.c_int]
+    check(lib.mcedm_op_set_conv_wino_split(int(enable)), "set_conv_wino_split")
 
 
 def set_wgrad_wino(enable: int = -1) -> None:
@@ -1469,6 +1478,22 @@
     return out
 
 
+def op_conv_wino_split(xa, xb, wino, bias, Cout, coef=None, coef_batch=1, act=0, res=None, res_mode=RS_NONE, out=None, want_sums=False):
+    lib = _bind_ops()
+    B, Ca, H, W = xa.shape
+    Cb = xb.shape[1] if xb is not None else 0
+    if out is None:
+        out = torch.empty((B, Cout, H, W), dtype=torch.float32, device=xa.device)
+    if want_sums:
+        gsum = torch.zeros(B * ((H + 3) // 4) * ((W + 7) // 8) * ((Cout + 3) // 4) * 2, dtype=torch.float32, device=xa.device)
+        check(lib.mcedm_op_conv_wino_split_sums(_ptr(xa), _ptr(xb), Ca, Cb, _ptr(coef), coef_batch, act, H, W, _ptr(wino), _ptr(bias),
+                                                _ptr(res), res_mode, _ptr(out), _ptr(gsum), Cout, B, _stream()), "op_conv_wino_split_sums")
+        return out, gsum
+    check(lib.mcedm_op_conv_wino_split(_ptr(xa), _ptr(xb), Ca, Cb, _ptr(coef), coef_batch, act, H, W, _ptr(wino), _ptr(bias), _ptr(res),
+                                       res_mode, _ptr(out), Cout, B, _stream()), "op_conv_wino_split")
+    return out
+
+
 def op_pack_conv_frag(w: torch.Tensor) -> torch.Tensor:
     lib = _bind_ops()
     Cout, Cin = w.shape[:2]
```
